# lbcb-sci/GNNome

Hardware: AMD Instinct MI355X
Metric: edges/sec full-graph GatedGCN fwd (higher is better)
Workload: dtype f32

## Files before the change

### gnnome_amd/_lib.py

```python
import ctypes
import os

_HERE = os.path.dirname(os.path.abspath(__file__))
LIB_PATH = os.environ.get("GNNOME_HIP_LIB") or os.path.join(_HERE, "lib", "libgnnome_hip.so")
HEADER_PATH = os.path.join(os.path.dirname(_HERE), "include", "gnnome_hip.h")

_p = ctypes.c_void_p
_i = ctypes.c_int
_l = ctypes.c_int64
_sz = ctypes.c_size_t

SIGNATURES = {
    "gnnome_abi_version": [],
    "gnnome_last_error": [],
    "gnnome_set_tuning": [_i, _i],
    "gnnome_debug_gate_profile": [_p],
    "gnnome_graph_views_workspace_bytes": [_l, _l, ctypes.POINTER(_sz)],
    "gnnome_build_graph_views": [_p, _p, _l, _l, _p, _p, _p, _p, _p, _p, _p, _p, _sz, _p],
    "gnnome_encode_f32": [_p, _l, _i, _p, _p, _p, _i, _p, _p, _i, _p, _p],
    "gnnome_linear_f32": [_p, _l, _i, _i, _p, _i, _p, _i, _p, _i, _p],
    "gnnome_linear_acc_f32": [_p, _l, _i, _i, _p, _i, _p, _i, _p, _i, _p],
    "gnnome_weight_planes_f16": [_p, _i, _i, _i, _p, _p],
    "gnnome_linear_planes_f32": [_p, _l, _i, _i, _p, _p, _i, _p, _i, _p],
    "gnnome_linear_planes_route": [_l, _i, _i, _i],
    "gnnome_edge_gate_f32": [_p, _p, _l, _i, _p, _p, _i, _p, _p, _p, _i, _i, _p, _p, _p],
    "gnnome_edge_gate_encode_f32": [_p, _p, _p, _p, _p, _p, _p, _l, _i, _p, _p, _i, _p, _p, _p, _i, _p, _p, _p],
    "gnnome_linear_ref_f32": [_p, _l, _i, _i, _p, _i, _p, _i, _p, _i, _p],
    "gnnome_edge_gate_ref_f32": [_p, _p, _l, _i, _p, _p, _i, _p, _p, _p, _i, _p, _p, _p, _p, _p, _p, _p, _p, _p, _p],
    "gnnome_node_aggregate_f32": [_p, _i, _l, _p, _p, _p, _i, _p, _p, _p, _p, _p, _p, _i, _p, _i, _p, _p, _p],
    "gnnome_build_node_records": [_p, _p, _p, _p, _p, _l, _p, _p],
    "gnnome_debug_node_records": [_p],
    "gnnome_node_aggregate_range_f32": [_p, _i, _l, _l, _l, _p, _p, _p, _i, _p, _p, _p, _p, _p, _p, _i, _p, _i, _p, _p, _p],
    "gnnome_node_aggregate_in_f32": [_p, _i, _l, _p, _p, _i, _p, _p, _p, _i, _p, _i, _p, _p, _p],
    "gnnome_node_aggregate_in_range_f32": [_p, _i, _l, _l, _l, _p, _p, _i, _p, _p, _p, _i, _p, _i, _p, _p, _p],
    "gnnome_node_aggregate_in_raw_f32": [_p, _i, _l, _p, _p, _i, _p, _p, _p, _p, _p, _p],
    "gnnome_node_aggregate_in_bwd_f32": [_p, _l, _i, _l, _p, _p, _p, _i, _p, _p, _p, _p, _p, _p, _p, _p],
    "gnnome_node_aggregate_in_raw_part_f32": [_p, _i, _l, _l, _p, _p, _i, _p, _p, _p, _p, _p, _p],
    "gnnome_node_aggregate_in_bwd_part_f32": [_p, _l, _i, _l, _l, _p, _p, _p, _i, _p, _p, _p, _p, _p, _p, _p, _p],
    "gnnome_node_neighbour_sum_f32": [_p, _i, _i, _l, _p, _p, _p, _p, _p, _p, _p, _i, _p],
    "gnnome_relu_rows_f32": [_p, _i, _l, _i, _p],
    "gnnome_node_neighbour_sum_bwd_f32": [_p, _i, _i, _l, _p, _p, _p, _p, _i, _p, _p, _p, _i, _p, _i, _p, _i, _p, _i, _p],
    "gnnome_node_neighbour_sum_part_f32": [_p, _i, _i, _l, _l, _p, _l, _p, _p, _p, _p, _p, _p, _p, _i, _p],
    "gnnome_node_neighbour_sum_bwd_part_f32": [_p, _i, _i, _l, _l, _p, _l, _p, _p, _p, _p, _i, _p, _p, _p, _i, _p, _i, _p, _i, _p, _i, _p],
    "gnnome_relu_mul_rows_f32": [_p, _i, _p, _i, _l, _i, _i, _p],
    "gnnome_node_attention_sum_f32": [_p, _i, _p, _i, _p, _i, _i, _i, _l, _p, _p, _p, _p, ctypes.c_float, _p, _p, _i, _p],
    "gnnome_node_attention_sum_stats_f32": [_p, _i, _p, _i, _p, _i, _i, _i, _l, _p, _p, _p, _p, ctypes.c_float, _p, _p, _i, _p, _i, _p],
    "gnnome_node_attention_sum_bwd_f32": [_p, _i, _p, _i, _p, _i, _p, _i, _p, _i, _p, _p, _i, _i, _i, _l, _p, _p, _p, _p, _i, ctypes.c_float,
                                          _p, _i, _p, _i, _p, _i, _p, _p],
    "gnnome_node_attention_sum_part_f32": [_p, _i, _p, _i, _p, _i, _i, _i, _l, _l, _p, _p, _p, _p, ctypes.c_float, _p, _p, _i, _p],
    "gnnome_node_attention_sum_stats_part_f32": [_p, _i, _p, _i, _p, _i, _i, _i, _l, _l, _p, _p, _p, _p, ctypes.c_float, _p, _p, _i, _p, _i, _p],
    "gnnome_node_attention_sum_bwd_dst_part_f32": [_p, _i, _p, _i, _p, _i, _p, _i, _p, _i, _p, _p, _i, _i, _i, _l, _l, _p, _p, _p, _p, _i,
                                                   ctypes.c_float, _p, _i, _p, _p],
    "gnnome_node_attention_sum_bwd_src_part_f32": [_p, _i, _p, _i, _p, _i, _p, _i, _i, _l, _l, _p, _p, _p, _p, _i, ctypes.c_float, _p, _i, _p, _i,
                                                   _p],
    "gnnome_stream_schedule_sizes": [_l, _l, _i, ctypes.POINTER(_l), ctypes.POINTER(_sz)],
    "gnnome_build_stream_schedule": [_l, _l, _p, _p, _p, _p, _p, _i, _i, _i, _p, _p, _p, _p, _p, _p, _p, _p, _sz, _p],
    "gnnome_node_aggregate_stream_f32": [_p, _i, _l, _l, _p, _p, _p, _i, _p, _p, _p, _p, _p, _p, _i, _p, _p, _p, _i, _i, _i, _p, _p, _p, _p, _p, _p,
                                         _p, _l, _p, _p],
    "gnnome_edge_score_f32": [_p, _l, _i, _i, _p, _p, _i, _p, _p, _p, _p, _i, _p, _p, _p, _p, _p, _p, _p],
    "gnnome_debug_forward_events": [_p, _p, _p, _p, _i],
    "gnnome_model_forward_workspace_bytes": [_l, _l, _i, _i, ctypes.POINTER(_sz)],
    "gnnome_model_forward_f32": [_p, _p, _p, _p, _p, _p, _sz, _p],
    "gnnome_model_forward_buffers_f32": [_p, _p, _p, _p, _p, _p, _p],
    "gnnome_edge_gate_raw_f32": [_p, _p, _l, _i, _p, _p, _i, _p, _p, _p, _i, _p],
    "gnnome_edge_gate_raw_stats_rows": [_i, ctypes.POINTER(_i)],
    "gnnome_edge_gate_raw_stats_f32": [_p, _p, _l, _i, _p, _p, _i, _p, _p, _p, _i, _p, _p, _p],
    "gnnome_edge_gate_raw_stats_x16": [_p, _p, _l, _i, _p, _p, _i, _p, _p, _p, _i, _p, _p, _p],
    "gnnome_edge_gate_bn_f32": [_p, _p, _p, _l, _i, _p, _p, _i, _p, _p, _p, _i, _p, _p, _p],
    "gnnome_edge_gate_bn_x16": [_p, _p, _p, _l, _i, _p, _p, _i, _p, _p, _p, _i, _p, _p, _p],
    "gnnome_node_aggregate_raw_f32": [_p, _i, _l, _i, _p, _p, _p, _i, _p, _p, _p, _p, _p, _p, _p, _p, _p, _p, _p],
    "gnnome_colsum_workspace_bytes": [ctypes.POINTER(_sz)],
    "gnnome_colsum2_f32": [_p, _p, _l, _i, _p, _p, _p, _p, _sz, _p],
    "gnnome_bn_relu_res_f32": [_p, _p, _p, _p, _l, _i, _p, _p],
    "gnnome_bn_relu_res_x16": [_p, _p, _p, _p, _l, _i, _p, _p],
    "gnnome_bn_bwd_stats_f32": [_p, _p, _p, _p, _p, _l, _i, _p, _p, _p, _sz, _p],
    "gnnome_bn_bwd_apply_f32": [_p, _p, _p, _p, _l, _i, _p, _p, _p, _p, _p, _p, _p],
    "gnnome_bn_bwd_apply_tables_f32": [_p, _p, _p, _p, _l, _i, _p, _p, _p, _p, _p, _p, _p, _p, _p, _p, _p, _p, _p, _p, _p, _p],
    "gnnome_ln_relu_res_f32": [_p, _p, _p, _p, _l, _i, _i, _p, _p],
    "gnnome_ln_bwd_f32": [_p, _p, _p, _p, _l, _i, _i, _p, _p, _p, _p, _sz, _p],
    "gnnome_mul23_f32": [_p, _p, _p, _l, _p, _p, _p],
    "gnnome_add_f32": [_p, _p, _l, _p, _p],
    "gnnome_relu_bwd_f32": [_p, _p, _l, _p, _p],
    "gnnome_segment_sum_f32": [_p, _i, _p, _p, _l, _p, _i, _p],
    "gnnome_segment_sum2_f32": [_p, _i, _p, _p, _p, _l, _p, _i, _p, _i, _p],
    "gnnome_segment_sum2_amax_f32": [_p, _i, _p, _p, _p, _l, _p, _i, _p, _i, _p, _p],
    "gnnome_segment_sum2_x16": [_p, _i, _p, _p, _p, _l, _p, _i, _p, _i, _p],
    "gnnome_wgrad_workspace_bytes": [_l, _i, _i, ctypes.POINTER(_sz)],
    "gnnome_wgrad_f32": [_p, _i, _i, _p, _i, _i, _l, _p, _i, _p, _sz, _p],
    "gnnome_wgrad_scaled_f32": [_p, _i, _i, _p, _i, _i, _l, _p, _p, _i, _p, _sz, _p],
    "gnnome_wgrad_x16": [_p, _i, _i, _p, _i, _i, _l, _p, _i, _p, _sz, _p],
    "gnnome_wgrad_blocks_f32": [_p, _i, _i, _i, _p, _i, _i, _l, _p, _i, _p, _p, _sz, _p],
    "gnnome_wgrad_blocks_scaled_f32": [_p, _i, _i, _i, _p, _i, _i, _l, _p, _p, _i, _p, _p, _sz, _p],
    "gnnome_linear_blocks_f32": [_p, _i, _i, _l, _i, _p, _i, _i, _p, _i, _i, _p],
    "gnnome_linear_blocks_scaled_f32": [_p, _i, _i, _l, _i, _p, _i, _i, _p, _p, _i, _i, _p],
    "gnnome_score_tail_bwd_f32": [_p, _p, _p, _l, _i, _p, _p, _p, _p, _p, _p, _p],
    "gnnome_agg_edge_bwd_f32": [_p, _l, _i, _p, _p, _p, _p, _p, _p, _i, _p, _p, _p, _p],
    "gnnome_encode_hidden_f32": [_p, _l, _i, _p, _p, _p, _i, _p, _p],
    "gnnome_gather_rows_f32": [_p, _i, _p, _l, _i, _p, _i, _p],
    "gnnome_scatter_add_rows_f32": [_p, _i, _p, _l, _i, _p, _i, _p],
    "gnnome_closure_workspace_bytes": [ctypes.POINTER(_sz)],
    "gnnome_degree_features_f32": [_p, _p, _l, _i, _p, _p, _sz, _p],
    "gnnome_edge_features_f32": [_p, _p, _l, _p, _p, _sz, _p],
    "gnnome_bn_bwd_dgrad_f32": [_p, _p, _l, _l, _i, _p, _p, _p, _p, _p, _p, _p, _p, _i, _p, _p],
    "gnnome_bn_bwd_dgrad_amax_f32": [_p, _p, _l, _l, _i, _p, _p, _p, _p, _p, _p, _p, _p, _i, _p, _p, _p],
    "gnnome_bn_bwd_dgrad_out_f32": [_p, _p, _p, _l, _l, _i, _p, _p, _p, _p, _p, _p, _p, _p, _i, _p, _p],
    "gnnome_bn_bwd_dgrad_out_amax_f32": [_p, _p, _p, _l, _l, _i, _p, _p, _p, _p, _p, _p, _p, _p, _i, _p, _p, _p],
    "gnnome_bn_bwd_dgrad_x16": [_p, _p, _l, _l, _i, _p, _p, _p, _p, _p, _p, _p, _p, _i, _p, _p],
    "gnnome_bn_bwd_dgrad_out_x16": [_p, _p, _p, _l, _l, _i, _p, _p, _p, _p, _p, _p, _p, _p, _i, _p, _p],
    "gnnome_agg_edge_bwd_stats_f32": [_p, _l, _i, _p, _p, _p, _p, _p, _p, _i, _p, _p, _p, _p, _p, _p, _p, _p, _p, _p, _sz, _p],
    "gnnome_agg_edge_bwd_stats_x16": [_p, _l, _i, _p, _p, _p, _p, _p, _p, _i, _p, _p, _p, _p, _p, _p, _p, _p, _p, _p, _sz, _p],
    "gnnome_agg_bwd_fused_f32": [_p, _l, _l, _i, _p, _p, _p, _p, _p, _p, _i, _p, _p, _p, _p, _p, _p, _p, _p, _p, _p, _p, _p, _p, _p, _p, _p, _sz, _p],
    "gnnome_agg_bwd_fused_x16": [_p, _l, _l, _i, _p, _p, _p, _p, _p, _p, _i, _p, _p, _p, _p, _p, _p, _p, _p, _p, _p, _p, _p, _p, _p, _p, _p, _sz, _p],
    "gnnome_bn_bwd_terms_f32": [_p, _p, _p, _l, _i, _p, _p, _p, _p],
    "gnnome_pack_layer_f32": [_p, _p, _p, _p, _i, _p, _p, _p, _p, _p],
    "gnnome_bn_train_finish_f32": [_p, _p, _p, _l, _i, _p, _p, _p, _p, _p, ctypes.c_float, ctypes.c_float, _i, _p, _p, _p, _p, _p],
    "gnnome_gate_center_f32": [_p, _l, _i, _p, _p, _i, _p, _p, _p, _i, _p, _p],
    "gnnome_greedy_walks_workspace_bytes": [_l, _i, ctypes.POINTER(_sz)],
    "gnnome_greedy_walks": [_p, _p, _p, _p, _p, _p, _p, _l, _p, _p, _p, _i, _p, _p, _l, _p, _p, _p, _p, _p, _p, _p, _sz, _p],
    "gnnome_greedy_walks_opts": [_p, _p, _p, _p, _p, _p, _p, _l, _p, _p, _p, _i, _p, _p, _l, _p, _p, _p, _p, _p, _p, _p, _sz, ctypes.c_float, _i, _l,
                                 _p],
    "gnnome_candidate_table": [_p, _p, _p, _p, _p, _p, _p, _i, _p, _p],
    "gnnome_mark_walk_visited": [_p, _p, _p, _l, _p, _p],
    "gnnome_overlap_workspace_bytes": [ctypes.POINTER(_sz)],
    "gnnome_overlap_edit_distance": [_p, _p, _l, _p, _i, _p, _p, _p, _l, _p, _p, _p, _sz, _p],
    "gnnome_overlap_long_workspace_bytes": [_l, ctypes.POINTER(_sz)],
    "gnnome_overlap_edit_distance_long": [_p, _p, _l, _p, _i, _p, _p, _p, _l, _l, _p, _p, _p, _sz, _p],
    "gnnome_contig_pieces_workspace_bytes": [_l, _l, ctypes.POINTER(_sz)],
    "gnnome_contig_pieces": [_p, _l, _p, _l, _p, _p, _p, _p, _l, _p, _l, _p, _p, _sz, _p],
    "gnnome_contig_spell": [_p, _l, _p, _l, _p, _p, _p, _l, _p, _i, _p, _l, _p],
    "gnnome_edge_labels_workspace_bytes": [_l, _l, ctypes.POINTER(_sz)],
    "gnnome_edge_labels": [_p, _p, _l, _l, _p, _p, _p, _p, _p, _p, _l, _p, _sz, _p],
    "gnnome_cluster_inputs_workspace_bytes": [_l, _l, ctypes.POINTER(_sz)],
    "gnnome_cluster_inputs_f32": [_p, _p, _l, _l, _p, _p, _l, _p, _l, _p, _l, _p, _p, _l, _p, _p, _l, _p, _p, _p, _p, _p, _sz, _p],
    "gnnome_adjacency_support": [_p, _p, _p, _l, _l, _p, _p],
    "gnnome_bfs_levels": [_p, _p, _l, _p, _p, _p, _p, _p, _p, _p],
    "gnnome_hem_propose": [_p, _p, _p, _p, _p, _l, _i, _p, _p],
    "gnnome_kway_gains": [_p, _p, _p, _p, _l, _p, _p, _p],
    "gnnome_greedy_growing_host": [_p, _p, _p, _p, _l, _i, _p],
    "gnnome_edge_loss_f32": [_p, _p, _p, _l, _p, ctypes.c_float, ctypes.c_float, _p, _p, _p, _p, _p, _sz, _p],
    "gnnome_gfa_tile_sizes": [ctypes.POINTER(_i), ctypes.POINTER(_i)],
    "gnnome_gfa_mark": [_p, _l, _p, _p, _p],
    "gnnome_gfa_classify": [_p, _l, _p, _p, _l, _p, _l, _p, _p, _p, _p, _p],
    "gnnome_gfa_names_insert": [_p, _l, _p, _p, _l, _p, _l, _p, _l, _p, _p],
    "gnnome_gfa_links": [_p, _l, _p, _p, _l, _p, _p, _l, _p, _l, _p, _l, _p, _p, _p, _p],
    "gnnome_gfa_pack": [_p, _l, _p, _p, _l, _p, _l, _p],
    "gnnome_reads_records_fasta": [_p, _l, _p, _p, _l, _p, _p, _l, _p, _p, _p, _p, _p, _p],
    "gnnome_reads_records_fastq": [_p, _l, _p, _p, _l, _p, _p, _l, _p, _l, _p, _p, _p, _p],
    "gnnome_reads_names_insert": [_p, _l, _p, _l, _p, _l, _p, _p, _p],
    "gnnome_reads_match": [_p, _l, _p, _i, _l, _p, _l, _p, _l, _p, _l, _p, _p],
    "gnnome_reads_annotations": [_p, _l, _p, _i, _l, _p, _p, _l, _p, _p, _p, _l, _p, _p],
    "gnnome_maf_lines": [_p, _l, _p, _p, _l, _p, _l, _p, _p, _p, _p, _p],
    "gnnome_maf_text_check": [_p, _l, _p, _p, _l, _p, _l, _p, _p],
    "gnnome_pr_curve_tile_size": [ctypes.POINTER(_i)],
    "gnnome_pr_curve_workspace_bytes": [_l, ctypes.POINTER(_sz)],
    "gnnome_pr_curve_keys": [_p, _p, _l, _i, _i, _p, _p, _p, _sz, _p],
    "gnnome_pr_curve_scan": [_p, _l, _p, _sz, _p, _p],
    "gnnome_pr_curve_emit": [_p, _l, _l, _l, _p, _p, _p, _p, _p, _p, _p, _sz, _p],
    "gnnome_pr_curve_ap": [_p, _p, _l, _p, _p, _sz, _p],
    "gnnome_walk_audit": [_p, _p, _p, _l, _l, _p, _p, _p, _p, _l, _p, _p, _p],
    "gnnome_interval_union_tile_size": [ctypes.POINTER(_i)],
    "gnnome_interval_union_workspace_bytes": [_l, ctypes.POINTER(_sz)],
    "gnnome_interval_union": [_p, _p, _p, _l, _p, _p, _p, _p, _l, _p, _p, _p, _p, _p, _sz, _p],
    "gnnome_pagerank_workspace_bytes": [_l, ctypes.POINTER(_sz)],
    "gnnome_pagerank_steps_f64": [_p, _p, _p, _l, _i, _p, _p, _p, _sz, _p],
    "gnnome_rw_return_lds_bytes": [_i, ctypes.POINTER(_sz)],
    "gnnome_rw_return_workspace_bytes": [_l, _i, ctypes.POINTER(_sz)],
    "gnnome_rw_return_f64": [_p, _p, _p, _l, _i, _i, _p, _i, _p, _p, _p, _sz, _p],
    "gnnome_sketch_tile_size": [ctypes.POINTER(_i)],
    "gnnome_sketch_workspace_bytes": [_l, ctypes.POINTER(_sz)],
    "gnnome_sketch_reads": [_p, _p, _l, _i, _i, _p, _l, _p, _p, _p, _p, _l, _p, _p, _sz, _p],
    "gnnome_seed_pairs_workspace_bytes": [_l, ctypes.POINTER(_sz)],
    "gnnome_seed_pairs": [_p, _p, _p, _p, _l, _p, _l, _i, _i, _p, _p, _l, _p, _p, _sz, _p],
    "gnnome_chain_overlaps": [_p, _p, _l, _p, _l, _p, _l, _i, _i, _i, _i, _i, _p, _p],
    "gnnome_transitive_tile_size": [ctypes.POINTER(_i)],
    "gnnome_transitive_edges": [_p, _p, _p, _p, _l, _l, _i, _p, _p],
    "gnnome_tip_nodes_workspace_bytes": [_l, ctypes.POINTER(_sz)],
    "gnnome_tip_nodes": [_p, _p, _p, _p, _p, _p, _l, _i, _p, _p, _sz, _p],
}

ABI_VERSION = 32


class LayerParams(ctypes.Structure):
    _fields_ = [(n, _p) for n in ("Wcat", "Wcat_planes", "bcat", "W3", "b3", "scale_e", "shift_e", "scale_h", "shift_h")] + [
        ("norm_kind", ctypes.c_int32), ("reference_order", ctypes.c_int32)]


class ModelParams(ctypes.Structure):
    _fields_ = ([(n, ctypes.c_int32) for n in ("hidden", "hidden_ne", "num_layers", "score_hidden", "node_features", "edge_features")]
                + [(n, _p) for n in ("node_W1", "node_b1", "node_W2", "node_b2", "edge_W1", "edge_b1", "edge_W2", "edge_b2")]
                + [("layers_host", ctypes.POINTER(LayerParams)), ("W_nodes", _p), ("W_nodes_planes", _p), ("b_nodes", _p), ("W1e", _p),
                   ("ld_w1e", ctypes.c_int32), ("reserved", ctypes.c_int32), ("W2", _p), ("b2", _p), ("W3", _p), ("b3", _p)])


class Views(ctypes.Structure):
    _fields_ = ([("num_nodes", ctypes.c_int64), ("num_edges", ctypes.c_int64)]
                + [(n, _p) for n in ("in_ptr", "srt_src", "srt_dst", "srt_eid", "out_ptr", "out_pos", "out_dst", "node_gather")]
                + [("transposed", ctypes.c_int32), ("reserved", ctypes.c_int32)])


class ForwardBuffers(ctypes.Structure):
    _fields_ = [("h", _p * 2), ("P", _p), ("e", _p * 2), ("PQ", _p)]


NORM_AFFINE = 0
NORM_LAYER = 1

_lib = None


class GnnomeHipError(RuntimeError):
    pass


def load():
    global _lib
# ... 26 lines not shown
```

### gnnome_amd/csrc/common.h

```cpp
#pragma once
#include <hip/hip_runtime.h>
#include <stdint.h>
#include <stdio.h>

#include "../../include/gnnome_hip.h"

namespace gnnome {

void set_error(const char* fmt, ...);

enum { kTuneGateVariant = 0, kTuneGateAblation = 1, kTuneLinearVariant = 2, kTuneGateTileOrder = 3, kTuneGateExperiment = 4, kTuneAggLdsKiB = 5, kTuneAggHubs = 6, kTuneAggVariant = 7, kTuneRefVariant = 8, kTuneOverlapBand = 9, kTuneArith = 10, kTuneAggAddr64 = 11, kTuneProjectSchedule = 12, kTuneCount = 16 };
int tuning(int key);

struct GateEnc {
    const float* e_raw;
    const int32_t* srt_eid;
    const float *W1, *b1, *W2, *b2;
    const float *W23, *b23;
};

struct GateBnBwd {
    const float *a, *c1, *c2, *mean, *rstd, *scale, *shift;
    float* a_out;
    int64_t n_once;
    unsigned* amax_bits = nullptr;
};

struct GateBfArgs {
    const float* e_in;
    float* e_out;
    int64_t E;
    const float* B1h;
    const float* B2h;
    int ldn;
    const int32_t* srt_src;
    const int32_t* srt_dst;
    const float* W3;
    int ldw;
    const float* scale;
    const float* shift;
    float* stats;
    int num_tiles;
    int abl;
    long long* prof;
    int xp;
    int num_cblocks, ld_out;
    GateEnc enc;
    GateBnBwd bnb;
};
int gate_bf_launch(int hidden, int mode, bool enc, const GateBfArgs& args, hipStream_t s, bool x16 = false, int extra = 0);
int gate_stream_launch(const float* e_in, float* e_out, int64_t E, const float* B1h, const float* B2h, int ldn, const int32_t* ss,
                       const int32_t* sd, const float* W3, int ldw, const float* scale, const float* shift, hipStream_t s);

int ws_linear_acc(const float* A, int64_t M, int K, const float* W, int ldw, float* C, hipStream_t s);
int stream_linear_acc_256(const float* A, int64_t M, const float* W, int ldw, float* C, hipStream_t s);
int gate_pl256_launch(int mode, const GateBfArgs& a, hipStream_t s, bool x16 = false);
int gate_f16_launch(int mode, const GateBfArgs& a, int grid, hipStream_t s, bool x16 = false);
int gate_enc256_launch(const GateBfArgs& a, hipStream_t s);
int gate_pl256_stats_rows();
void hub_cache_invalidate();
long long* gate_profile_buffer();
int linear_refm_launch(const float* A, int64_t M, int K, int lda, const float* W, int ldw, const float* bias, int Nout, float* C, int ldc,
                       hipStream_t s);
int gate_refm_launch(int hidden, bool with_enc, const float* e_in, float* e_out, int64_t E, const float* B1h, const float* B2h, int ldn,
                     const int32_t* ss, const int32_t* sd, const float* W3, int ldw, const float* b3, const float* scale, const float* shift,
                     const GateEnc& enc, hipStream_t s);

#define GN_REQUIRE(cond, ...)                 \
    do {                                      \
        if (!(cond)) {                        \
            ::gnnome::set_error(__VA_ARGS__); \
            return GNNOME_EINVAL;             \
        }                                     \
    } while (0)

#define GN_HIP(call)                                                                              \
    do {                                                                                          \
        hipError_t err__ = (call);                                                                \
        if (err__ != hipSuccess) {                                                                \
            ::gnnome::set_error("%s failed: %s (%s:%d)", #call, hipGetErrorString(err__), __FILE__, \
                                __LINE__);                                                        \
            return GNNOME_EHIP;                                                                   \
        }                                                                                         \
    } while (0)

#define GN_LAUNCH_CHECK() GN_HIP(hipGetLastError())

constexpr int kWave = 64;
constexpr int kXcds = 8;
constexpr int kNumCUs = 256;
int persistent_grid();
constexpr float kAggEps = 1e-6f;
constexpr float kNormEps = 1e-5f;

typedef float f32x4 __attribute__((ext_vector_type(4)));
typedef float f32x16 __attribute__((ext_vector_type(16)));

__device__ __forceinline__ unsigned bf16_bits(float x) {
    const unsigned u = __float_as_uint(x);
    return (u + 0x7FFFu + ((u >> 16) & 1u)) >> 16;
}
__device__ __forceinline__ uint2 pack_bf16x4(const f32x4 v) {
    return make_uint2(bf16_bits(v[0]) | (bf16_bits(v[1]) << 16), bf16_bits(v[2]) | (bf16_bits(v[3]) << 16));
}
__device__ __forceinline__ f32x4 unpack_bf16x4(const uint2 p) {
    return f32x4{__uint_as_float(p.x << 16), __uint_as_float(p.x & 0xFFFF0000u), __uint_as_float(p.y << 16),
                 __uint_as_float(p.y & 0xFFFF0000u)};
}
template <bool X16>
__device__ __forceinline__ f32x4 load4_as(const void* base, int64_t off) {
    if (X16) return unpack_bf16x4(*reinterpret_cast<const uint2*>(reinterpret_cast<const uint16_t*>(base) + off));
    return *reinterpret_cast<const f32x4*>(reinterpret_cast<const float*>(base) + off);
}
template <bool X16>
__device__ __forceinline__ void store4_as(void* base, int64_t off, const f32x4 v) {
    if (X16)
        *reinterpret_cast<uint2*>(reinterpret_cast<uint16_t*>(base) + off) = pack_bf16x4(v);
    else
        *reinterpret_cast<f32x4*>(reinterpret_cast<float*>(base) + off) = v;
}


__device__ __forceinline__ int xcd_remap(int bid, int n) {
    const int xcd = bid % kXcds, q = n / kXcds, r = n % kXcds;
    const int base = xcd < r ? xcd * (q + 1) : r * (q + 1) + (xcd - r) * q;
    return base + bid / kXcds;
}

__device__ __forceinline__ float sigmoidf_(float x) { return __builtin_amdgcn_rcpf(1.0f + __expf(-x)); }

typedef float f32x2 __attribute__((ext_vector_type(2)));
__device__ __forceinline__ f32x2 packed_(f32x2 v) {
    asm("" : "+v"(v));
    return v;
}
__device__ __forceinline__ f32x4 sigmoid4_(const f32x4 x) {
    const f32x2 t0 = packed_(packed_(f32x2{x[0], x[1]}) * -1.4426950408889634f), t1 = packed_(packed_(f32x2{x[2], x[3]}) * -1.4426950408889634f);
    const f32x2 d0 = packed_(packed_(f32x2{__builtin_amdgcn_exp2f(t0[0]), __builtin_amdgcn_exp2f(t0[1])}) + 1.0f);
    const f32x2 d1 = packed_(packed_(f32x2{__builtin_amdgcn_exp2f(t1[0]), __builtin_amdgcn_exp2f(t1[1])}) + 1.0f);
    return f32x4{__builtin_amdgcn_rcpf(d0[0]), __builtin_amdgcn_rcpf(d0[1]), __builtin_amdgcn_rcpf(d1[0]), __builtin_amdgcn_rcpf(d1[1])};
}

__device__ __forceinline__ float relu_keep_nan(float t) { return t < 0.f ? 0.f : t; }

__device__ __forceinline__ void wave_amax_to(unsigned* amax_bits, float v) {
#pragma unroll
    for (int o = 32; o > 0; o >>= 1) v = fmaxf(v, __shfl_xor(v, o));
    if ((threadIdx.x & 63) == 0) {
        const unsigned b = __float_as_uint(v);
        if (b > __hip_atomic_load(amax_bits, __ATOMIC_RELAXED, __HIP_MEMORY_SCOPE_AGENT)) atomicMax(amax_bits, b);
    }
}

__device__ __forceinline__ float half_wave_sum(float v) {
    v += __shfl_xor(v, 1);
    v += __shfl_xor(v, 2);
    v += __shfl_xor(v, 4);
    v += __shfl_xor(v, 8);
    v += __shfl_xor(v, 16);
    return v;
}

}
```

### gnnome_amd/csrc/edge_gate.hip

```cpp
#include "gemm_tile.h"
#include "lds_handover.h"

namespace gnnome {

template <int NB, int NORM>
__global__ __launch_bounds__(kGemmThreads) void k_edge_gate(const float* e_in, float* e_out, int64_t E,
                                                            const float* __restrict__ B1h,
                                                            const float* __restrict__ B2h, int ldn,
                                                            const int32_t* __restrict__ srt_src,
                                                            const int32_t* __restrict__ srt_dst,
                                                            const float* __restrict__ W3, int ldw,
                                                            const float* __restrict__ scale,
                                                            const float* __restrict__ shift, int total_tiles, int norm_width) {
    constexpr int H = 32 * NB;
    __shared__ __attribute__((aligned(16))) float lds[tile_lds_floats<NB>() + 2 * kTileM];
    float* As = lds;
    float* Ws = lds + kTileM * kLdk;
    int* s_src = reinterpret_cast<int*>(lds + tile_lds_floats<NB>());
    int* s_dst = s_src + kTileM;

    const int tid = threadIdx.x, wave = tid >> 6, lane = tid & 63;
    const int tile = xcd_remap(blockIdx.x, total_tiles);
    const int64_t row0 = (int64_t)tile * kTileM;
    const int valid = (int)min((int64_t)kTileM, E - row0);
// ... 473 lines not shown
    hipStream_t s = (hipStream_t)stream;
    const int variant = tuning(kTuneGateVariant);
    const bool rows16 = ld_node % 4 == 0 && ((uintptr_t)B1h % 16 == 0) && ((uintptr_t)B2h % 16 == 0);
    const bool persistent_ok = norm_kind == GNNOME_NORM_AFFINE && (hidden == 64 || hidden == 128);
    if (persistent_ok && variant != 1) {
        if ((variant == 0 || variant == 7 || variant == 8) && rows16) {
            GateBfArgs a = {};
            a.e_in = e_in; a.e_out = e_out; a.E = num_edges; a.B1h = B1h; a.B2h = B2h; a.ldn = ld_node; a.srt_src = srt_src;
            a.srt_dst = srt_dst; a.W3 = W3; a.ldw = ldw; a.scale = norm_scale; a.shift = norm_shift;
            return gate_bf_launch(hidden, 0, false, a, s);
        }
        if ((variant == 5 || variant == 6) && rows16) {
            if (hidden == 128)
                return launch_gate_ws<4, 1>(e_in, e_out, num_edges, B1h, B2h, ld_node, srt_src, srt_dst, W3, ldw, norm_scale, norm_shift, s);
            return launch_gate_ws<2, 2>(e_in, e_out, num_edges, B1h, B2h, ld_node, srt_src, srt_dst, W3, ldw, norm_scale, norm_shift, s);
        }
    }
    if (hidden == 256 && norm_kind == GNNOME_NORM_AFFINE && (variant == 0 || variant == 9) && e_in != e_out && ld_node % 4 == 0 &&
        ((uintptr_t)e_out % 16 == 0)) {
        if (variant == 0 && rows16) {
            GateBfArgs a = {};
            a.e_in = e_in; a.e_out = e_out; a.E = num_edges; a.B1h = B1h; a.B2h = B2h; a.ldn = ld_node; a.srt_src = srt_src;
            a.srt_dst = srt_dst; a.W3 = W3; a.ldw = ldw; a.scale = norm_scale; a.shift = norm_shift;
            return gate_pl256_launch(0, a, s);
        }
        return gate_stream_launch(e_in, e_out, num_edges, B1h, B2h, ld_node, srt_src, srt_dst, W3, ldw, norm_scale, norm_shift, s);
    }
    switch (hidden) {
        case 64: return launch_gate<2>(e_in, e_out, num_edges, B1h, B2h, ld_node, srt_src, srt_dst, W3, ldw, norm_kind, norm_scale, norm_shift, s, norm_width);
        case 128: return launch_gate<4>(e_in, e_out, num_edges, B1h, B2h, ld_node, srt_src, srt_dst, W3, ldw, norm_kind, norm_scale, norm_shift, s, norm_width);
        case 256: return launch_gate<8>(e_in, e_out, num_edges, B1h, B2h, ld_node, srt_src, srt_dst, W3, ldw, norm_kind, norm_scale, norm_shift, s, norm_width);
        default: set_error("edge_gate: hidden=%d not in {64,128,256}", hidden); return GNNOME_EINVAL;
    }
}

extern "C" int gnnome_edge_gate_raw_f32(const float* e_in, float* x_out, int64_t num_edges, int hidden, const float* B1h,
                                        const float* B2h, int ld_node, const int32_t* srt_src, const int32_t* srt_dst,
                                        const float* W3, int ldw, void* stream) {
    using namespace gnnome;
    GN_REQUIRE(num_edges >= 0, "edge_gate_raw: negative edge count");
    if (num_edges == 0) return GNNOME_OK;
    GN_REQUIRE(e_in && x_out && x_out != e_in && B1h && B2h && srt_src && srt_dst && W3, "edge_gate_raw: bad pointers");
    GN_REQUIRE(ld_node >= hidden && ldw >= hidden && ldw % 4 == 0, "edge_gate_raw: bad strides");
    GN_REQUIRE(((uintptr_t)e_in % 16 == 0) && ((uintptr_t)W3 % 16 == 0), "edge_gate_raw: e_in and W3 must be 16-byte aligned");
    hipStream_t s = (hipStream_t)stream;
    if (hidden == 256 && tuning(kTuneGateVariant) == 0 && ld_node % 4 == 0 && ((uintptr_t)B1h % 16 == 0) && ((uintptr_t)B2h % 16 == 0) &&
        ((uintptr_t)x_out % 16 == 0)) {
        GateBfArgs a = {};
        a.e_in = e_in; a.e_out = x_out; a.E = num_edges; a.B1h = B1h; a.B2h = B2h; a.ldn = ld_node; a.srt_src = srt_src;
        a.srt_dst = srt_dst; a.W3 = W3; a.ldw = ldw;
        return gate_pl256_launch(1, a, s);
    }
    switch (hidden) {
        case 64: return launch_gate<2>(e_in, x_out, num_edges, B1h, B2h, ld_node, srt_src, srt_dst, W3, ldw, 2, nullptr, nullptr, s);
        case 128: return launch_gate<4>(e_in, x_out, num_edges, B1h, B2h, ld_node, srt_src, srt_dst, W3, ldw, 2, nullptr, nullptr, s);
        case 256: return launch_gate<8>(e_in, x_out, num_edges, B1h, B2h, ld_node, srt_src, srt_dst, W3, ldw, 2, nullptr, nullptr, s);
        default: set_error("edge_gate_raw: hidden=%d not in {64,128,256}", hidden); return GNNOME_EINVAL;
    }
}

extern "C" int gnnome_edge_gate_raw_stats_rows(int hidden, int* rows_host) {
    using namespace gnnome;
    GN_REQUIRE(rows_host && (hidden == 64 || hidden == 128 || hidden == 256), "edge_gate_raw_stats_rows: hidden=%d not in {64,128,256}", hidden);
    if (hidden == 256) {
        *rows_host = gate_pl256_stats_rows();
        return GNNOME_OK;
    }
    *rows_host = (tuning(kTuneGateVariant) == 0 || tuning(kTuneGateVariant) == 8) ? kNumCUs * 8 : kNumCUs * (hidden == 128 ? 1 : 2);
    return GNNOME_OK;
}

static int raw_stats_impl(const float* e_in, void* x_out, int64_t num_edges, int hidden, const float* B1h,
                          const float* B2h, int ld_node, const int32_t* srt_src, const int32_t* srt_dst,
                          const float* W3, int ldw, const float* center, float* stats_partial, void* stream, bool x16) {
    using namespace gnnome;
    GN_REQUIRE(num_edges > 0, "edge_gate_raw_stats: needs at least one edge");
    GN_REQUIRE(e_in && x_out != (const void*)e_in && B1h && B2h && srt_src && srt_dst && W3 && center && stats_partial,
               "edge_gate_raw_stats: bad pointers");
    GN_REQUIRE(x_out || ((hidden == 128 || (hidden == 256 && tuning(kTuneArith) == 0 && !x16)) && tuning(kTuneGateVariant) == 0),
               "edge_gate_raw_stats: x_out may be NULL at hidden = 128 and, as fp16x3 with fp32 storage, 256 (default kernels)");
    GN_REQUIRE(hidden == 64 || hidden == 128 || hidden == 256, "edge_gate_raw_stats: hidden=%d not in {64,128,256}", hidden);
    GN_REQUIRE(ld_node >= hidden && ld_node % 4 == 0 && ldw >= hidden && ldw % 4 == 0, "edge_gate_raw_stats: bad strides");
    GN_REQUIRE(((uintptr_t)e_in % 16 == 0) && ((uintptr_t)W3 % 16 == 0) && ((uintptr_t)B1h % 16 == 0) && ((uintptr_t)B2h % 16 == 0),
               "edge_gate_raw_stats: 16-byte alignment required");
    GN_REQUIRE(!x16 || hidden == 256 || tuning(kTuneGateVariant) == 0 || tuning(kTuneGateVariant) == 8,
               "edge_gate_raw_stats_x16: bf16 storage is built on the default kernels (gnnome_set_tuning key 0 = 0 or 8), got %d", tuning(kTuneGateVariant));
    hipStream_t s = (hipStream_t)stream;
    if (hidden == 256) {
        GateBfArgs a = {};
        a.e_in = e_in; a.e_out = (float*)x_out; a.E = num_edges; a.B1h = B1h; a.B2h = B2h; a.ldn = ld_node; a.srt_src = srt_src;
        a.srt_dst = srt_dst; a.W3 = W3; a.ldw = ldw; a.scale = center; a.stats = stats_partial;
        return gate_pl256_launch(1, a, s, x16);
    }
    if (tuning(kTuneGateVariant) == 0 || tuning(kTuneGateVariant) == 8 || x16) {
        GateBfArgs a = {};
        a.e_in = e_in; a.e_out = (float*)x_out; a.E = num_edges; a.B1h = B1h; a.B2h = B2h; a.ldn = ld_node; a.srt_src = srt_src;
        a.srt_dst = srt_dst; a.W3 = W3; a.ldw = ldw; a.scale = center; a.stats = stats_partial;
        return gate_bf_launch(hidden, 1, false, a, s, x16, x_out == nullptr ? 1 : 0);
    }
    if (hidden == 128)
        return launch_ws_raw_stats<4, 1>(e_in, (float*)x_out, num_edges, B1h, B2h, ld_node, srt_src, srt_dst, W3, ldw, center, stats_partial, s);
    return launch_ws_raw_stats<2, 2>(e_in, (float*)x_out, num_edges, B1h, B2h, ld_node, srt_src, srt_dst, W3, ldw, center, stats_partial, s);
}

extern "C" int gnnome_edge_gate_raw_stats_f32(const float* e_in, float* x_out, int64_t num_edges, int hidden, const float* B1h,
                                              const float* B2h, int ld_node, const int32_t* srt_src, const int32_t* srt_dst,
                                              const float* W3, int ldw, const float* center, float* stats_partial, void* stream) {
    return raw_stats_impl(e_in, x_out, num_edges, hidden, B1h, B2h, ld_node, srt_src, srt_dst, W3, ldw, center, stats_partial, stream, false);
}

extern "C" int gnnome_edge_gate_raw_stats_x16(const float* e_in, uint16_t* x_out, int64_t num_edges, int hidden, const float* B1h,
                                              const float* B2h, int ld_node, const int32_t* srt_src, const int32_t* srt_dst,
                                              const float* W3, int ldw, const float* center, float* stats_partial, void* stream) {
    return raw_stats_impl(e_in, x_out, num_edges, hidden, B1h, B2h, ld_node, srt_src, srt_dst, W3, ldw, center, stats_partial, stream, true);
}

static int gate_bn_impl(const float* e_in, float* e_out, void* x_out, int64_t num_edges, int hidden, const float* B1h, const float* B2h, int ld_node,
                        const int32_t* srt_src, const int32_t* srt_dst, const float* W3, int ldw, const float* scale, const float* shift,
                        void* stream, bool x16) {
    using namespace gnnome;
    GN_REQUIRE(num_edges >= 0, "edge_gate_bn: negative edge count");
    if (num_edges == 0) return GNNOME_OK;
    GN_REQUIRE(e_in && e_out && x_out && x_out != (const void*)e_in && x_out != (void*)e_out && B1h && B2h && srt_src && srt_dst && W3 && scale && shift,
               "edge_gate_bn: bad pointers");
    GN_REQUIRE((hidden == 128 || (hidden == 256 && tuning(kTuneArith) == 0 && !x16)) && tuning(kTuneGateVariant) == 0,
               "edge_gate_bn: built at hidden = 128 and, as fp16x3 with fp32 storage, 256 (default kernels), got %d", hidden);
    GN_REQUIRE(ld_node >= hidden && ld_node % 4 == 0 && ldw >= hidden && ldw % 4 == 0, "edge_gate_bn: bad strides");
    GN_REQUIRE(((uintptr_t)e_in % 16 == 0) && ((uintptr_t)e_out % 16 == 0) && ((uintptr_t)x_out % 16 == 0) && ((uintptr_t)W3 % 16 == 0) &&
                   ((uintptr_t)B1h % 16 == 0) && ((uintptr_t)B2h % 16 == 0), "edge_gate_bn: 16-byte alignment required");
    GateBfArgs a = {};
    a.e_in = e_in; a.e_out = e_out; a.E = num_edges; a.B1h = B1h; a.B2h = B2h; a.ldn = ld_node; a.srt_src = srt_src; a.srt_dst = srt_dst;
    a.W3 = W3; a.ldw = ldw; a.scale = scale; a.shift = shift; a.bnb.a_out = (float*)x_out;
    if (hidden == 256) return gate_pl256_launch(0, a, (hipStream_t)stream, false);
    return gate_bf_launch(hidden, 0, false, a, (hipStream_t)stream, x16, 1);
}

extern "C" int gnnome_edge_gate_bn_f32(const float* e_in, float* e_out, float* x_out, int64_t num_edges, int hidden, const float* B1h,
                                       const float* B2h, int ld_node, const int32_t* srt_src, const int32_t* srt_dst, const float* W3, int ldw,
                                       const float* scale, const float* shift, void* stream) {
    return gate_bn_impl(e_in, e_out, x_out, num_edges, hidden, B1h, B2h, ld_node, srt_src, srt_dst, W3, ldw, scale, shift, stream, false);
}

extern "C" int gnnome_edge_gate_bn_x16(const float* e_in, float* e_out, uint16_t* x_out, int64_t num_edges, int hidden, const float* B1h,
                                       const float* B2h, int ld_node, const int32_t* srt_src, const int32_t* srt_dst, const float* W3, int ldw,
                                       const float* scale, const float* shift, void* stream) {
    return gate_bn_impl(e_in, e_out, x_out, num_edges, hidden, B1h, B2h, ld_node, srt_src, srt_dst, W3, ldw, scale, shift, stream, true);
}

extern "C" int gnnome_edge_gate_encode_f32(const float* e_raw, const int32_t* srt_eid, const float* encW1, const float* encb1,
                                           const float* encW2, const float* encb2, float* e_out, int64_t num_edges, int hidden,
                                           const float* B1h, const float* B2h, int ld_node, const int32_t* srt_src,
                                           const int32_t* srt_dst, const float* W3, int ldw, const float* norm_scale,
                                           const float* norm_shift, void* stream) {
    using namespace gnnome;
    GN_REQUIRE(num_edges >= 0, "edge_gate_encode: negative edge count");
    if (num_edges == 0) return GNNOME_OK;
    GN_REQUIRE(e_raw && srt_eid && encW1 && encb1 && encW2 && encb2 && e_out && B1h && B2h && srt_src && srt_dst && W3 &&
                   norm_scale && norm_shift, "edge_gate_encode: null pointer");
    GN_REQUIRE(hidden == 64 || hidden == 128 || (hidden == 256 && tuning(kTuneArith) == 0 && tuning(kTuneGateVariant) == 0),
               "edge_gate_encode: hidden=%d not in {64,128,256 (default kernels)}", hidden);
    GN_REQUIRE(ld_node % 4 == 0 && ldw % 4 == 0 && ((uintptr_t)B1h % 16 == 0) && ((uintptr_t)B2h % 16 == 0) && ((uintptr_t)W3 % 16 == 0),
               "edge_gate_encode: alignment");
    const GateEnc enc = {e_raw, srt_eid, encW1, encb1, encW2, encb2};
    hipStream_t s = (hipStream_t)stream;
    if (hidden == 256) {
        GN_REQUIRE((uintptr_t)e_out % 16 == 0, "edge_gate_encode: e_out must be 16-byte aligned");
        GateBfArgs a = {};
        a.e_out = e_out; a.E = num_edges; a.B1h = B1h; a.B2h = B2h; a.ldn = ld_node; a.srt_src = srt_src; a.srt_dst = srt_dst;
        a.W3 = W3; a.ldw = ldw; a.scale = norm_scale; a.shift = norm_shift; a.enc = enc;
        return gate_enc256_launch(a, s);
    }
    if (tuning(kTuneGateVariant) == 0 || tuning(kTuneGateVariant) == 7 || tuning(kTuneGateVariant) == 8) {
        GateBfArgs a = {};
        a.e_out = e_out; a.E = num_edges; a.B1h = B1h; a.B2h = B2h; a.ldn = ld_node; a.srt_src = srt_src; a.srt_dst = srt_dst;
        a.W3 = W3; a.ldw = ldw; a.scale = norm_scale; a.shift = norm_shift; a.enc = enc;
        return gate_bf_launch(hidden, 0, true, a, s);
    }
    if (hidden == 128)
        return launch_gate_ws<4, 1>(nullptr, e_out, num_edges, B1h, B2h, ld_node, srt_src, srt_dst, W3, ldw, norm_scale, norm_shift, s, &enc);
    return launch_gate_ws<2, 2>(nullptr, e_out, num_edges, B1h, B2h, ld_node, srt_src, srt_dst, W3, ldw, norm_scale, norm_shift, s, &enc);
}
```

### gnnome_amd/csrc/edge_gate_bf.hip

```cpp
#include "common.h"
#include "lds_handover.h"
#include "operand_planes.h"

namespace gnnome {

template <int CB, int RB>
struct GateBF {
    static_assert(CB * RB == 4, "four compute waves");
    static constexpr int H = 32 * CB, TM = 32 * RB, LDK = H + 4, RING = 4, LWAVES = 2;
    static constexpr int NT = 64 * (4 + RING * LWAVES);
    static constexpr int NP = TM * (H / 4) / (64 * LWAVES);
    static constexpr int kSlotFloats = TM * LDK;
    static constexpr int kLdsFloats = RING * 2 * kSlotFloats;
};

template <int CB, int RB, int MODE, bool ENC, bool X16 = false>
__global__ __launch_bounds__(768) void k_edge_gate_bf(GateBfArgs a) {
    using P = GateBF<CB, RB>;
    constexpr int H = P::H, TM = P::TM, NP = P::NP, LDK = P::LDK, RING = P::RING, KS = H / 16, SLOT = P::kSlotFloats;
    constexpr int kEncFloats = ENC ? 16 * H + H + 48 : (MODE == 1 ? 8 * 64 * 8 : 0);
    __shared__ __attribute__((aligned(16))) float lds[P::kLdsFloats + kEncFloats];
    __shared__ unsigned flags[2 * RING];
    float* Aring = lds;
    float* Gring = lds + RING * SLOT;
// ... 664 lines not shown
    constexpr int H = 128, TM = 32, RING = 3, LDK = H + 4, TPLD = 48, TPLANE = TM * TPLD, TILEF = TM * LDK;
    constexpr int SLOTB = 3 * TPLANE + 2 * TILEF * 4, NP = 8, RSTEP = 4;
    __shared__ __attribute__((aligned(16))) unsigned char ring[RING * SLOTB];
    __shared__ __attribute__((aligned(16))) float consts[4 * H];
    __shared__ float w1s[32], b1s[16];
    __shared__ unsigned flags[2 * RING];
    const int tid = threadIdx.x, lane = tid & 63;
    const int wave = __builtin_amdgcn_readfirstlane(tid >> 6);
    const unsigned full0 = lds_addr(&flags[0]), done0 = lds_addr(&flags[RING]);
    const int per_xcd = gridDim.x / kXcds;
    const int first = (int)(blockIdx.x % kXcds) * per_xcd + (int)(blockIdx.x / kXcds);
    const int stride = (int)gridDim.x;
    const int n = first < a.num_tiles ? (a.num_tiles - first + stride - 1) / stride : 0;
    if (n <= 0) return;
    auto tile_of = [&](int r) { return first + r * stride; };
    auto tile_valid = [&](int r) { return (int)min((int64_t)TM, a.E - (int64_t)tile_of(r) * TM); };
    if (tid < 4 * H) {
        const int q = tid / H, c = tid % H;
        consts[tid] = q == 0 ? a.scale[c] : q == 1 ? a.shift[c] : q == 2 ? a.enc.b23[c] : a.enc.b2[c];
    }
    if (tid >= 4 * H && tid < 4 * H + 32) w1s[tid - 4 * H] = a.enc.W1[tid - 4 * H];
    if (tid >= 4 * H + 32 && tid < 4 * H + 48) b1s[tid - 4 * H - 32] = a.enc.b1[tid - 4 * H - 32];
    if (tid < 2 * RING) flags[tid] = 0;
    __syncthreads();

    if (wave < 4) {
        const int cl = lane & 31, half = lane >> 5, col = 32 * wave + cl;
        uint4 u1, u2, u3, v1, v2, v3;
        {
            const float* p = a.enc.W23 + col * 16 + 8 * half;
            bf16_split8(*reinterpret_cast<const f32x4*>(p), *reinterpret_cast<const f32x4*>(p + 4), u1, u2, u3);
            const float* q = a.enc.W2 + col * 16 + 8 * half;
            bf16_split8(*reinterpret_cast<const f32x4*>(q), *reinterpret_cast<const f32x4*>(q + 4), v1, v2, v3);
        }
        auto crow = [](int r) { return (r & 3) + 8 * (r >> 2); };
        const int lane_x = 4 * half * LDK + col;
        const float bxc = consts[2 * H + col], bec = consts[3 * H + col];
        for (int i = 0; i < n; ++i) {
            const int slot = i % RING;
            const unsigned use = (unsigned)(i / RING) + 1u;
            flag_wait(full0 + 4 * slot, 2u * use, 0);
            const unsigned char* tp = ring + slot * SLOTB + cl * TPLD + 16 * half;
            const uint4 c1 = *reinterpret_cast<const uint4*>(tp), c2 = *reinterpret_cast<const uint4*>(tp + TPLANE),
                        c3 = *reinterpret_cast<const uint4*>(tp + 2 * TPLANE);
            f32x16 ax, ae;
#pragma unroll
            for (int r = 0; r < 16; ++r) ax[r] = ae[r] = 0.f;
            ax = __builtin_amdgcn_mfma_f32_32x32x16_bf16(as_bf16x8(c3), as_bf16x8(u1), ax, 0, 0, 0);
            ae = __builtin_amdgcn_mfma_f32_32x32x16_bf16(as_bf16x8(c3), as_bf16x8(v1), ae, 0, 0, 0);
            ax = __builtin_amdgcn_mfma_f32_32x32x16_bf16(as_bf16x8(c1), as_bf16x8(u3), ax, 0, 0, 0);
            ae = __builtin_amdgcn_mfma_f32_32x32x16_bf16(as_bf16x8(c1), as_bf16x8(v3), ae, 0, 0, 0);
            ax = __builtin_amdgcn_mfma_f32_32x32x16_bf16(as_bf16x8(c2), as_bf16x8(u2), ax, 0, 0, 0);
            ae = __builtin_amdgcn_mfma_f32_32x32x16_bf16(as_bf16x8(c2), as_bf16x8(v2), ae, 0, 0, 0);
            ax = __builtin_amdgcn_mfma_f32_32x32x16_bf16(as_bf16x8(c2), as_bf16x8(u1), ax, 0, 0, 0);
            ae = __builtin_amdgcn_mfma_f32_32x32x16_bf16(as_bf16x8(c2), as_bf16x8(v1), ae, 0, 0, 0);
            ax = __builtin_amdgcn_mfma_f32_32x32x16_bf16(as_bf16x8(c1), as_bf16x8(u2), ax, 0, 0, 0);
            ae = __builtin_amdgcn_mfma_f32_32x32x16_bf16(as_bf16x8(c1), as_bf16x8(v2), ae, 0, 0, 0);
            ax = __builtin_amdgcn_mfma_f32_32x32x16_bf16(as_bf16x8(c1), as_bf16x8(u1), ax, 0, 0, 0);
            ae = __builtin_amdgcn_mfma_f32_32x32x16_bf16(as_bf16x8(c1), as_bf16x8(v1), ae, 0, 0, 0);
            float* X = reinterpret_cast<float*>(ring + slot * SLOTB + 3 * TPLANE) + lane_x;
#pragma unroll
            for (int r = 0; r < 16; ++r) {
                X[crow(r) * LDK] = ax[r] + bxc;
                X[TILEF + crow(r) * LDK] = ae[r] + bec;
            }
            flag_bump(done0 + 4 * slot, lane);
        }
    } else {
        const int group = (wave - 4) / 2;
        const int gl = ((wave - 4) % 2) * 64 + lane;
        const int r0 = gl / (H / 4), c4 = gl % (H / 4);
        const int trow = gl >> 2, jq = gl & 3;
        f32x4 g1[NP], g2[NP], gk[NP];
        int si[NP], di[NP], eid = 0;
        float raw0 = 0.f, raw1 = 0.f;
        const unsigned off_row = (unsigned)(r0 * H + 4 * c4);
        auto issue_early = [&](int r) {
            const int64_t row0 = (int64_t)tile_of(r) * TM;
            const int valid = tile_valid(r);
#pragma unroll
            for (int p = 0; p < NP; ++p) {
                const int64_t row = row0 + min(r0 + p * RSTEP, valid - 1);
                si[p] = a.srt_src[row];
                di[p] = a.srt_dst[row];
            }
            eid = a.enc.srt_eid[row0 + min(trow, valid - 1)];
        };
        auto issue_late = [&]() {
            raw0 = a.enc.e_raw[2 * (int64_t)eid];
            raw1 = a.enc.e_raw[2 * (int64_t)eid + 1];
#pragma unroll
            for (int p = 0; p < NP; ++p) {
                g1[p] = *reinterpret_cast<const f32x4*>(a.B1h + (int64_t)si[p] * a.ldn + 4 * c4);
                g2[p] = *reinterpret_cast<const f32x4*>(a.B2h + (int64_t)di[p] * a.ldn + 4 * c4);
            }
        };
        if (group < n) {
            issue_early(group);
            issue_late();
            if (group + RING < n) issue_early(group + RING);
        }
        unsigned char* S = ring + group * SLOTB;
        const float* Xs = reinterpret_cast<const float*>(S + 3 * TPLANE);
        for (int r = group; r < n; r += RING) {
            const unsigned use = (unsigned)(r / RING) + 1u;
            {
                f32x4 t;
#pragma unroll
                for (int j = 0; j < 4; ++j) {
                    const int hu = 4 * jq + j;
                    t[j] = fmaxf(__builtin_fmaf(raw1, w1s[2 * hu + 1], raw0 * w1s[2 * hu]) + b1s[hu], 0.f);
                }
                uint2 p1, p2, p3;
                bf16_split4(t, p1, p2, p3);
                unsigned char* d = S + trow * TPLD + 8 * jq;
                *reinterpret_cast<uint2*>(d) = p1;
                *reinterpret_cast<uint2*>(d + TPLANE) = p2;
                *reinterpret_cast<uint2*>(d + 2 * TPLANE) = p3;
            }
#pragma unroll
            for (int p = 0; p < NP; ++p) {
                gk[p] = g1[p] + g2[p];
                asm volatile("" : "+v"(gk[p]));
            }
            flag_bump(full0 + 4 * group, lane);
            if (r + RING < n) issue_late();
            if (r + 2 * RING < n) issue_early(r + 2 * RING);
            flag_wait(done0 + 4 * group, 4u * use, a.xp & 3);
            const int valid = tile_valid(r);
            const f32x4 sc4 = *reinterpret_cast<const f32x4*>(consts + 4 * c4), sh4 = *reinterpret_cast<const f32x4*>(consts + H + 4 * c4);
            float* out = a.e_out + (int64_t)tile_of(r) * TM * H;
#pragma unroll
            for (int pb = 0; pb < NP; pb += 2) {
                f32x4 x[2], e0[2];
#pragma unroll
                for (int u = 0; u < 2; ++u) {
                    x[u] = *reinterpret_cast<const f32x4*>(Xs + (r0 + (pb + u) * RSTEP) * LDK + 4 * c4);
                    e0[u] = *reinterpret_cast<const f32x4*>(Xs + TILEF + (r0 + (pb + u) * RSTEP) * LDK + 4 * c4);
                }
                asm volatile("" : "+v"(x[0]), "+v"(x[1]));
#pragma unroll
                for (int u = 0; u < 2; ++u) {
                    const int p = pb + u, row = r0 + p * RSTEP;
                    f32x4 y;
#pragma unroll
                    for (int j = 0; j < 4; ++j) y[j] = fmaxf((x[u][j] + gk[p][j]) * sc4[j] + sh4[j], 0.f) + e0[u][j];
                    if (row < valid) *reinterpret_cast<f32x4*>(out + (off_row + (unsigned)(p * RSTEP * H))) = y;
                }
            }
        }
    }
}

struct EncFoldScratch {
    float* w23 = nullptr;
};
static EncFoldScratch g_enc_fold[16];

static int launch_enc16(const GateBfArgs& args, hipStream_t s) {
    GateBfArgs a = args;
    const int64_t tiles = (a.E + 31) / 32;
    GN_REQUIRE(tiles < (1ll << 31), "edge_gate: too many tiles");
    a.num_tiles = (int)tiles;
    a.xp = tuning(kTuneGateExperiment);
    int dev = 0;
    GN_HIP(hipGetDevice(&dev));
    GN_REQUIRE(dev >= 0 && dev < 16, "edge_gate_encode: device index %d", dev);
    if (!g_enc_fold[dev].w23) GN_HIP(hipMalloc(&g_enc_fold[dev].w23, sizeof(float) * (128 * 16 + 128)));
    float* w23 = g_enc_fold[dev].w23;
    hipLaunchKernelGGL(k_fold_encoder, dim3((128 * 17 + 3) / 4), dim3(256), 0, s, a.W3, a.ldw, a.enc.W2, a.enc.b2, 128, w23, w23 + 128 * 16);
    GN_LAUNCH_CHECK();
    a.enc.W23 = w23;
    a.enc.b23 = w23 + 128 * 16;
    hipLaunchKernelGGL(k_edge_gate_enc16, dim3(persistent_grid()), dim3(640), 0, s, a);
    GN_LAUNCH_CHECK();
    return GNNOME_OK;
}

static EncFoldScratch g_enc_fold256[16];
int gate_enc256_launch(const GateBfArgs& args, hipStream_t s) {
    GateBfArgs a = args;
    const int64_t tiles = (a.E + 31) / 32;
    GN_REQUIRE(tiles < (1ll << 31), "edge_gate: too many tiles");
    a.num_tiles = (int)tiles;
    a.prof = g_gate_prof;
    int dev = 0;
    GN_HIP(hipGetDevice(&dev));
    GN_REQUIRE(dev >= 0 && dev < 16, "edge_gate_encode: device index %d", dev);
    if (!g_enc_fold256[dev].w23) GN_HIP(hipMalloc(&g_enc_fold256[dev].w23, sizeof(float) * (256 * 16 + 256)));
    float* w23 = g_enc_fold256[dev].w23;
    hipLaunchKernelGGL(k_fold_encoder, dim3((256 * 17 + 3) / 4), dim3(256), 0, s, a.W3, a.ldw, a.enc.W2, a.enc.b2, 256, w23, w23 + 256 * 16);
    GN_LAUNCH_CHECK();
    a.enc.W23 = w23;
    a.enc.b23 = w23 + 256 * 16;
    int g = persistent_grid();
    g -= g % 16;
    return gate_f16_launch(5, a, g < 16 ? 16 : g, s);
}

template <int CB, int RB, int MODE, bool ENC, bool X16 = false>
static int launch_bf(const GateBfArgs& args, hipStream_t s) {
    using P = GateBF<CB, RB>;
    GateBfArgs a = args;
    const int64_t tiles = (a.E + P::TM - 1) / P::TM;
    GN_REQUIRE(tiles < (1ll << 31), "edge_gate: too many tiles");
    a.num_tiles = (int)tiles;
    a.abl = tuning(kTuneGateAblation);
    a.xp = tuning(kTuneGateExperiment);
    a.prof = g_gate_prof;
    if (MODE == 1) GN_HIP(hipMemsetAsync(a.stats, 0, sizeof(float) * kNumCUs * P::RING * P::LWAVES * 2 * P::H, s));
    hipLaunchKernelGGL((k_edge_gate_bf<CB, RB, MODE, ENC, X16>), dim3(persistent_grid()), dim3(P::NT), 0, s, a);
    GN_LAUNCH_CHECK();
    return GNNOME_OK;
}

int gate_bf_launch(int hidden, int mode, bool enc, const GateBfArgs& a, hipStream_t s, bool x16, int extra) {
    const bool planes = hidden == 128 && tuning(kTuneGateVariant) != 8;
    if (extra) {
        GN_REQUIRE(hidden == 128 && !enc && (mode == 0 || mode == 1), "edge-tile kernel: the two-pass training forward is built at hidden = 128");
        if (mode == 1) return x16 ? launch_pl<false, 1, true, 1>(a, s) : launch_pl<false, 1, false, 1>(a, s);
        return x16 ? launch_pl<false, 0, true, 1>(a, s) : launch_pl<false, 0, false, 1>(a, s);
    }
    if (x16) {
        if (mode == 1 && planes) return launch_pl<false, 1, true>(a, s);
        if (mode == 3 && planes) return launch_pl<false, 3, true>(a, s);
        if (mode == 1) return hidden == 128 ? launch_bf<4, 1, 1, false, true>(a, s) : launch_bf<2, 2, 1, false, true>(a, s);
        if (mode == 3) return hidden == 128 ? launch_bf<4, 1, 3, false, true>(a, s) : launch_bf<2, 2, 3, false, true>(a, s);
        set_error("edge-tile kernel: bf16 storage exists for modes 1 and 3 only");
        return GNNOME_EINVAL;
    }
    if (hidden == 128) {
        if (mode == 0 && enc && tuning(kTuneGateVariant) == 0) return launch_enc16(a, s);
        if (mode == 0 && tuning(kTuneGateVariant) != 8) return enc ? launch_pl<true>(a, s) : launch_pl<false>(a, s);
        if (mode == 1 && planes) return launch_pl<false, 1>(a, s);
        if (mode == 3 && planes) return launch_pl<false, 3>(a, s);
        if (mode == 4) return launch_pl<false, 4>(a, s);
        if (mode == 2 && planes) return launch_pl<false, 2>(a, s);
        if (mode == 0) return enc ? launch_bf<4, 1, 0, true>(a, s) : launch_bf<4, 1, 0, false>(a, s);
        if (mode == 3) return launch_bf<4, 1, 3, false>(a, s);
        return mode == 1 ? launch_bf<4, 1, 1, false>(a, s) : launch_bf<4, 1, 2, false>(a, s);
    }
    if (mode == 0) return enc ? launch_bf<2, 2, 0, true>(a, s) : launch_bf<2, 2, 0, false>(a, s);
    if (mode == 3) return launch_bf<2, 2, 3, false>(a, s);
    return mode == 1 ? launch_bf<2, 2, 1, false>(a, s) : launch_bf<2, 2, 2, false>(a, s);
}

}

extern "C" int gnnome_debug_gate_profile(void* counters) {
    gnnome::g_gate_prof = (long long*)counters;
    return GNNOME_OK;
}

static int bn_bwd_dgrad_impl(float* C, const void* X, int64_t rows, int64_t rows_once, int hidden, const float* scale, const float* shift,
                             const float* a, const float* c1, const float* c2, const float* mean, const float* rstd,
                             const float* W, int ldw, void* dxe, void* stream, bool x16, unsigned* amax_bits = nullptr) {
    using namespace gnnome;
    GN_REQUIRE(rows >= 0 && (hidden == 64 || hidden == 128), "bn_bwd_dgrad: hidden=%d not in {64,128}", hidden);
    GN_REQUIRE(rows_once >= 0 && rows_once <= rows, "bn_bwd_dgrad: rows_once=%lld outside [0, rows]", (long long)rows_once);
    if (rows == 0) return GNNOME_OK;
    GN_REQUIRE(C && X && scale && shift && a && c1 && c2 && mean && rstd && W && dxe && dxe != (void*)C && ldw >= hidden && ldw % 4 == 0,
               "bn_bwd_dgrad: bad arguments");
    GN_REQUIRE(((uintptr_t)C % 16 == 0) && ((uintptr_t)X % 16 == 0) && ((uintptr_t)dxe % 16 == 0) && ((uintptr_t)W % 16 == 0),
               "bn_bwd_dgrad: tensors must be 16-byte aligned");
    GateBfArgs g = {};
    g.e_in = (const float*)X; g.e_out = C; g.E = rows; g.B1h = C; g.ldn = hidden; g.W3 = W; g.ldw = ldw;
    g.bnb = GateBnBwd{a, c1, c2, mean, rstd, scale, shift, (float*)dxe, rows_once};
    if (amax_bits != nullptr) {
        GN_REQUIRE(hidden == 128 && tuning(kTuneGateVariant) != 8, "bn_bwd_dgrad_amax: hidden = 128 on the plane-form kernel only");
        GN_HIP(hipMemsetAsync(amax_bits, 0, sizeof(unsigned), (hipStream_t)stream));
        g.bnb.amax_bits = amax_bits;
    }
    return gate_bf_launch(hidden, 3, false, g, (hipStream_t)stream, x16);
}

extern "C" int gnnome_bn_bwd_dgrad_f32(float* C, const float* X, int64_t rows, int64_t rows_once, int hidden, const float* scale, const float* shift,
                                       const float* a, const float* c1, const float* c2, const float* mean, const float* rstd,
                                       const float* W, int ldw, float* dxe, void* stream) {
    return bn_bwd_dgrad_impl(C, X, rows, rows_once, hidden, scale, shift, a, c1, c2, mean, rstd, W, ldw, dxe, stream, false);
}

extern "C" int gnnome_bn_bwd_dgrad_amax_f32(float* C, const float* X, int64_t rows, int64_t rows_once, int hidden, const float* scale,
                                            const float* shift, const float* a, const float* c1, const float* c2, const float* mean,
                                            const float* rstd, const float* W, int ldw, float* dxe, unsigned* amax_bits, void* stream) {
    GN_REQUIRE(amax_bits != nullptr, "bn_bwd_dgrad_amax: null amax_bits");
    return bn_bwd_dgrad_impl(C, X, rows, rows_once, hidden, scale, shift, a, c1, c2, mean, rstd, W, ldw, dxe, stream, false, amax_bits);
}

extern "C" int gnnome_bn_bwd_dgrad_x16(float* C, const uint16_t* X, int64_t rows, int64_t rows_once, int hidden, const float* scale, const float* shift,
                                       const float* a, const float* c1, const float* c2, const float* mean, const float* rstd,
                                       const float* W, int ldw, uint16_t* dxe, void* stream) {
    return bn_bwd_dgrad_impl(C, X, rows, rows_once, hidden, scale, shift, a, c1, c2, mean, rstd, W, ldw, dxe, stream, true);
}

static int bn_bwd_dgrad_out_impl(const float* C_in, float* C_out, const float* X, int64_t rows, int64_t rows_once, int hidden,
                                 const float* scale, const float* shift, const float* a, const float* c1, const float* c2,
                                 const float* mean, const float* rstd, const float* W, int ldw, float* dxe, void* stream, bool x16,
                                 unsigned* amax_bits = nullptr);
extern "C" int gnnome_bn_bwd_dgrad_out_amax_f32(const float* C_in, float* C_out, const float* X, int64_t rows, int64_t rows_once, int hidden,
                                                const float* scale, const float* shift, const float* a, const float* c1, const float* c2,
                                                const float* mean, const float* rstd, const float* W, int ldw, float* dxe, unsigned* amax_bits,
                                                void* stream) {
    GN_REQUIRE(amax_bits != nullptr, "bn_bwd_dgrad_out_amax: null amax_bits");
    return bn_bwd_dgrad_out_impl(C_in, C_out, X, rows, rows_once, hidden, scale, shift, a, c1, c2, mean, rstd, W, ldw, dxe, stream, false, amax_bits);
}
extern "C" int gnnome_bn_bwd_dgrad_out_f32(const float* C_in, float* C_out, const float* X, int64_t rows, int64_t rows_once, int hidden,
                                           const float* scale, const float* shift, const float* a, const float* c1, const float* c2,
                                           const float* mean, const float* rstd, const float* W, int ldw, float* dxe, void* stream) {
    return bn_bwd_dgrad_out_impl(C_in, C_out, X, rows, rows_once, hidden, scale, shift, a, c1, c2, mean, rstd, W, ldw, dxe, stream, false);
}
extern "C" int gnnome_bn_bwd_dgrad_out_x16(const float* C_in, float* C_out, const uint16_t* X, int64_t rows, int64_t rows_once, int hidden,
                                           const float* scale, const float* shift, const float* a, const float* c1, const float* c2,
                                           const float* mean, const float* rstd, const float* W, int ldw, uint16_t* dxe, void* stream) {
    return bn_bwd_dgrad_out_impl(C_in, C_out, (const float*)X, rows, rows_once, hidden, scale, shift, a, c1, c2, mean, rstd, W, ldw, (float*)dxe, stream, true);
}
static int bn_bwd_dgrad_out_impl(const float* C_in, float* C_out, const float* X, int64_t rows, int64_t rows_once, int hidden,
                                 const float* scale, const float* shift, const float* a, const float* c1, const float* c2,
                                 const float* mean, const float* rstd, const float* W, int ldw, float* dxe, void* stream, bool x16,
                                 unsigned* amax_bits) {
    using namespace gnnome;
    GN_REQUIRE(rows >= 0 && hidden == 256, "bn_bwd_dgrad_out: hidden=%d (256 only; 64 / 128 update C in place: gnnome_bn_bwd_dgrad_f32)", hidden);
    if (amax_bits != nullptr) GN_HIP(hipMemsetAsync(amax_bits, 0, sizeof(unsigned), (hipStream_t)stream));
    GN_REQUIRE(rows_once >= 0 && rows_once <= rows, "bn_bwd_dgrad_out: rows_once=%lld outside [0, rows]", (long long)rows_once);
    if (rows == 0) return GNNOME_OK;
    GN_REQUIRE(C_in && C_out && C_out != C_in && X && scale && shift && a && c1 && c2 && mean && rstd && W && dxe && dxe != C_out && dxe != C_in &&
                   ldw >= hidden && ldw % 4 == 0, "bn_bwd_dgrad_out: bad arguments");
    GN_REQUIRE(((uintptr_t)C_in % 16 == 0) && ((uintptr_t)C_out % 16 == 0) && ((uintptr_t)X % 16 == 0) && ((uintptr_t)dxe % 16 == 0) &&
                   ((uintptr_t)W % 16 == 0), "bn_bwd_dgrad_out: tensors must be 16-byte aligned");
    (void)x16;
    GateBfArgs g = {};
    g.e_in = X; g.e_out = C_out; g.E = rows; g.B1h = C_in; g.ldn = hidden; g.W3 = W; g.ldw = ldw;
    g.bnb = GateBnBwd{a, c1, c2, mean, rstd, scale, shift, dxe, rows_once};
    g.bnb.amax_bits = amax_bits;
    return gate_pl256_launch(3, g, (hipStream_t)stream, x16);
}
```

### gnnome_amd/csrc/encode.hip

```cpp
#include "common.h"

namespace gnnome {

constexpr int kEncThreads = 256;
constexpr int kEncMaxF = 8, kEncMaxM = 64;

template <int H>
__global__ __launch_bounds__(kEncThreads) void k_encode(const float* __restrict__ in, int64_t rows, int F,
                                                        const int32_t* __restrict__ gather, const float* __restrict__ W1,
                                                        const float* __restrict__ b1, int M, const float* __restrict__ W2,
                                                        const float* __restrict__ b2, float* __restrict__ out) {
    constexpr int LPR = H / 4, RPB = kEncThreads / LPR, KMAX = (kEncMaxM + LPR - 1) / LPR;
    __shared__ __attribute__((aligned(16))) float w2t[kEncMaxM * H];
    __shared__ float w1s[kEncMaxM * kEncMaxF];
    __shared__ float b1s[kEncMaxM];
    const int tid = threadIdx.x;
    for (int i = tid; i < M * H; i += kEncThreads) w2t[i] = W2[(i % H) * M + (i / H)];
    for (int i = tid; i < M * F; i += kEncThreads) w1s[i] = W1[i];
    for (int i = tid; i < M; i += kEncThreads) b1s[i] = b1[i];
    __syncthreads();

    const int li = tid % LPR, rg = tid / LPR, c = 4 * li;
    const int lane_base = (tid & 63) - li;
    const f32x4 bias = *reinterpret_cast<const f32x4*>(b2 + c);

    for (int64_t r0 = (int64_t)blockIdx.x * RPB; r0 < rows; r0 += (int64_t)gridDim.x * RPB) {
        const int64_t r = r0 + rg;
        const bool live = r < rows;
        const int64_t rin = live ? (gather != nullptr ? (int64_t)gather[r] : r) : 0;
        float xin[kEncMaxF];
#pragma unroll
        for (int f = 0; f < kEncMaxF; ++f) xin[f] = (live && f < F) ? in[rin * F + f] : 0.f;
        float t[KMAX];
#pragma unroll
        for (int k = 0; k < KMAX; ++k) {
            const int j = li + k * LPR;
            float s = 0.f;
            if (j < M) {
#pragma unroll
                for (int f = 0; f < kEncMaxF; ++f)
                    if (f < F) s = __builtin_fmaf(xin[f], w1s[j * F + f], s);
                s = fmaxf(s + b1s[j], 0.f);
            }
            t[k] = s;
        }
        f32x4 acc = {0.f, 0.f, 0.f, 0.f};
#pragma unroll
        for (int k = 0; k < KMAX; ++k) {
            const int jn = min(LPR, M - k * LPR);
            for (int jj = 0; jj < jn; ++jj) {
                const float tj = __shfl(t[k], lane_base + jj);
                const f32x4 w = *reinterpret_cast<const f32x4*>(&w2t[(k * LPR + jj) * H + c]);
#pragma unroll
                for (int i = 0; i < 4; ++i) acc[i] = __builtin_fmaf(tj, w[i], acc[i]);
            }
        }
        if (live) *reinterpret_cast<f32x4*>(out + r * H + c) = acc + bias;
    }
}

template <int H>
__global__ __launch_bounds__(kEncThreads) void k_encode_f2m16(const float* __restrict__ in, int64_t rows,
                                                              const int32_t* __restrict__ gather,
                                                              const float* __restrict__ W1, const float* __restrict__ b1,
                                                              const float* __restrict__ W2, const float* __restrict__ b2,
                                                              float* __restrict__ out) {
    constexpr int LPR = H / 4, RPB = kEncThreads / LPR, M = 16;
    const int tid = threadIdx.x, li = tid % LPR, rg = tid / LPR, c = 4 * li;
    float w1a[M], w1b[M], bb[M];
#pragma unroll
    for (int j = 0; j < M; ++j) {
        w1a[j] = W1[2 * j];
        w1b[j] = W1[2 * j + 1];
        bb[j] = b1[j];
    }
    f32x4 w2[M];
#pragma unroll
    for (int i = 0; i < 4; ++i) {
#pragma unroll
        for (int j4 = 0; j4 < M / 4; ++j4) {
            const f32x4 v = *reinterpret_cast<const f32x4*>(W2 + (c + i) * M + 4 * j4);
#pragma unroll
            for (int jj = 0; jj < 4; ++jj) w2[4 * j4 + jj][i] = v[jj];
        }
    }
    const f32x4 bias = *reinterpret_cast<const f32x4*>(b2 + c);
    for (int64_t r = (int64_t)blockIdx.x * RPB + rg; r < rows; r += (int64_t)gridDim.x * RPB) {
        const int64_t rin = gather != nullptr ? (int64_t)gather[r] : r;
        const float x0 = in[2 * rin], x1 = in[2 * rin + 1];
        f32x4 acc = {0.f, 0.f, 0.f, 0.f};
#pragma unroll
        for (int j = 0; j < M; ++j) {
            const float t = fmaxf(__builtin_fmaf(x1, w1b[j], x0 * w1a[j]) + bb[j], 0.f);
#pragma unroll
            for (int i = 0; i < 4; ++i) acc[i] = __builtin_fmaf(t, w2[j][i], acc[i]);
        }
        *reinterpret_cast<f32x4*>(out + r * H + c) = acc + bias;
    }
}

template <int H>
static int launch_encode(const float* in, int64_t rows, int F, const int32_t* gather, const float* W1, const float* b1,
                         int M, const float* W2, const float* b2, float* out, hipStream_t s) {
    constexpr int RPB = kEncThreads / (H / 4);
    int64_t blocks = (rows + RPB - 1) / RPB;
    if (blocks > kNumCUs * 8) blocks = kNumCUs * 8;
    if (F == 2 && M == 16 && ((uintptr_t)W2 % 16 == 0)) {
        hipLaunchKernelGGL(k_encode_f2m16<H>, dim3((unsigned)blocks), dim3(kEncThreads), 0, s, in, rows, gather, W1, b1, W2, b2,
                           out);
    } else {
        hipLaunchKernelGGL(k_encode<H>, dim3((unsigned)blocks), dim3(kEncThreads), 0, s, in, rows, F, gather, W1, b1, M, W2,
                           b2, out);
    }
    GN_LAUNCH_CHECK();
    return GNNOME_OK;
}

__global__ __launch_bounds__(256) void k_gather_rows(const float* __restrict__ in, int ld_in,
                                                     const int32_t* __restrict__ idx, int64_t rows, int w4,
                                                     float* __restrict__ out, int ld_out) {
    const int64_t total = rows * w4;
    for (int64_t i = (int64_t)blockIdx.x * blockDim.x + threadIdx.x; i < total; i += (int64_t)gridDim.x * blockDim.x) {
        const int64_t r = i / w4;
        const int c = (int)(i % w4) * 4;
        *reinterpret_cast<f32x4*>(out + r * ld_out + c) = *reinterpret_cast<const f32x4*>(in + (int64_t)idx[r] * ld_in + c);
    }
}

__global__ __launch_bounds__(256) void k_scatter_add_rows(const float* __restrict__ in, int ld_in,
                                                          const int32_t* __restrict__ idx, int64_t rows, int w4,
                                                          float* __restrict__ out, int ld_out) {
    const int64_t total = rows * w4;
    for (int64_t i = (int64_t)blockIdx.x * blockDim.x + threadIdx.x; i < total; i += (int64_t)gridDim.x * blockDim.x) {
        const int64_t r = i / w4;
        const int c = (int)(i % w4) * 4;
        f32x4* dst = reinterpret_cast<f32x4*>(out + (int64_t)idx[r] * ld_out + c);
        const f32x4 a = *reinterpret_cast<const f32x4*>(in + r * ld_in + c);
        f32x4 b = *dst;
        b[0] += a[0]; b[1] += a[1]; b[2] += a[2]; b[3] += a[3];
        *dst = b;
    }
}

}

extern "C" int gnnome_encode_f32(const float* in, int64_t rows, int in_features, const int32_t* gather, const float* W1,
                                 const float* b1, int hidden_ne, const float* W2, const float* b2, int hidden, float* out,
                                 void* stream) {
    using namespace gnnome;
    GN_REQUIRE(rows >= 0, "encode: negative row count");
    if (rows == 0) return GNNOME_OK;
    GN_REQUIRE(in && W1 && b1 && W2 && b2 && out, "encode: null pointer");
    GN_REQUIRE(in_features >= 1 && in_features <= kEncMaxF, "encode: in_features=%d not in [1,%d]", in_features, kEncMaxF);
    GN_REQUIRE(hidden_ne >= 1 && hidden_ne <= kEncMaxM, "encode: hidden_ne=%d not in [1,%d]", hidden_ne, kEncMaxM);
    GN_REQUIRE(((uintptr_t)out % 16 == 0) && ((uintptr_t)b2 % 16 == 0), "encode: out and b2 must be 16-byte aligned");
    hipStream_t s = (hipStream_t)stream;
    switch (hidden) {
        case 64: return launch_encode<64>(in, rows, in_features, gather, W1, b1, hidden_ne, W2, b2, out, s);
        case 128: return launch_encode<128>(in, rows, in_features, gather, W1, b1, hidden_ne, W2, b2, out, s);
        case 256: return launch_encode<256>(in, rows, in_features, gather, W1, b1, hidden_ne, W2, b2, out, s);
        default: set_error("encode: hidden=%d not in {64,128,256}", hidden); return GNNOME_EINVAL;
    }
}

extern "C" int gnnome_gather_rows_f32(const float* in, int ld_in, const int32_t* idx, int64_t rows, int width, float* out,
                                      int ld_out, void* stream) {
    using namespace gnnome;
    GN_REQUIRE(rows >= 0, "gather_rows: negative row count");
    if (rows == 0) return GNNOME_OK;
    GN_REQUIRE(in && idx && out, "gather_rows: null pointer");
    GN_REQUIRE(width > 0 && width % 4 == 0 && ld_in % 4 == 0 && ld_out % 4 == 0 && ld_in >= width && ld_out >= width,
               "gather_rows: width and strides must be multiples of 4");
    GN_REQUIRE(((uintptr_t)in % 16 == 0) && ((uintptr_t)out % 16 == 0), "gather_rows: 16-byte alignment required");
    const int w4 = width / 4;
    int64_t blocks = (rows * w4 + 255) / 256;
    if (blocks > kNumCUs * 8) blocks = kNumCUs * 8;
    hipLaunchKernelGGL(k_gather_rows, dim3((unsigned)blocks), dim3(256), 0, (hipStream_t)stream, in, ld_in, idx, rows, w4,
                       out, ld_out);
    GN_LAUNCH_CHECK();
    return GNNOME_OK;
}

extern "C" int gnnome_scatter_add_rows_f32(const float* in, int ld_in, const int32_t* idx, int64_t rows, int width,
                                           float* out, int ld_out, void* stream) {
    using namespace gnnome;
    GN_REQUIRE(rows >= 0, "scatter_add_rows: negative row count");
    if (rows == 0) return GNNOME_OK;
    GN_REQUIRE(in && idx && out, "scatter_add_rows: null pointer");
    GN_REQUIRE(width > 0 && width % 4 == 0 && ld_in % 4 == 0 && ld_out % 4 == 0 && ld_in >= width && ld_out >= width,
               "scatter_add_rows: width and strides must be multiples of 4");
    GN_REQUIRE(((uintptr_t)in % 16 == 0) && ((uintptr_t)out % 16 == 0), "scatter_add_rows: 16-byte alignment required");
    const int w4 = width / 4;
    int64_t blocks = (rows * w4 + 255) / 256;
    if (blocks > kNumCUs * 8) blocks = kNumCUs * 8;
    hipLaunchKernelGGL(k_scatter_add_rows, dim3((unsigned)blocks), dim3(256), 0, (hipStream_t)stream, in, ld_in, idx, rows,
                       w4, out, ld_out);
    GN_LAUNCH_CHECK();
    return GNNOME_OK;
}
```

### gnnome_amd/csrc/model_forward.cpp

```cpp
#include "common.h"

namespace gnnome {
namespace {

constexpr size_t kAlign = 256;
size_t rounded(size_t bytes) { return (bytes + kAlign - 1) / kAlign * kAlign; }

struct Workspace {
    size_t h[2], P, e[2], PQ, total;
};
Workspace layout(int64_t n, int64_t e, int hidden, int hs) {
    Workspace w;
    size_t off = 0;
    auto take = [&](size_t bytes) {
        const size_t at = off;
        off += rounded(bytes);
        return at;
    };
    w.h[0] = take(sizeof(float) * n * hidden);
    w.h[1] = take(sizeof(float) * n * hidden);
    w.P = take(sizeof(float) * n * 5 * hidden);
    w.e[0] = take(sizeof(float) * e * hidden);
    w.e[1] = hidden == 256 ? take(sizeof(float) * e * hidden) : w.e[0];
    w.PQ = take(sizeof(float) * n * 2 * hs);
    w.total = off;
    return w;
}

struct ForwardEvents {
    hipEvent_t ev[4] = {nullptr, nullptr, nullptr, nullptr};
    int layer = -1;
};
thread_local ForwardEvents g_events;
int mark(int which, int layer, void* stream) {
    if (layer != g_events.layer || g_events.ev[which] == nullptr) return GNNOME_OK;
    GN_HIP(hipEventRecord(g_events.ev[which], (hipStream_t)stream));
    return GNNOME_OK;
}

int project(const float* A, int64_t M, int K, const float* W, const void* planes, const float* bias, int Nout, float* C, void* stream) {
    if (planes != nullptr && gnnome_linear_planes_route(M, K, Nout, 1)) return gnnome_linear_planes_f32(A, M, K, K, planes, bias, Nout, C, Nout, stream);
    return gnnome_linear_f32(A, M, K, K, W, K, bias, Nout, C, Nout, stream);
}

}
}

extern "C" int gnnome_debug_forward_events(void* gate_start, void* gate_stop, void* aggregate_start, void* aggregate_stop, int layer) {
    using namespace gnnome;
    g_events.ev[0] = (hipEvent_t)gate_start;
    g_events.ev[1] = (hipEvent_t)gate_stop;
    g_events.ev[2] = (hipEvent_t)aggregate_start;
    g_events.ev[3] = (hipEvent_t)aggregate_stop;
    g_events.layer = layer;
    return GNNOME_OK;
}

extern "C" int gnnome_model_forward_workspace_bytes(int64_t num_nodes, int64_t num_edges, int hidden, int score_hidden, size_t* bytes_host) {
    using namespace gnnome;
    GN_REQUIRE(bytes_host && num_nodes >= 0 && num_edges >= 0 && hidden > 0 && score_hidden > 0, "model_forward_workspace_bytes: bad argument");
    *bytes_host = layout(num_nodes, num_edges, hidden, score_hidden).total;
    return GNNOME_OK;
}

#define GN_TRY(call)                       \
    do {                                   \
        const int rc__ = (call);           \
        if (rc__ != GNNOME_OK) return rc__; \
    } while (0)

namespace gnnome {
namespace {
int forward_on(const gnnome_model_params* m, const gnnome_views* g, const float* x, const float* e_raw, float* logits, float* const h[2], float* P,
               float* const eb[2], float* PQ, void* stream);
}
}

static int check_model(const gnnome_model_params* m, const gnnome_views* g) {
    using namespace gnnome;
    GN_REQUIRE(m && g, "model_forward: null parameter block");
    const int H = m->hidden, hs = m->score_hidden, L = m->num_layers;
    GN_REQUIRE(g->num_nodes >= 0 && g->num_edges >= 0 && L >= 0 && (L == 0 || m->layers_host != nullptr), "model_forward: bad sizes");
    GN_REQUIRE(H == 64 || H == 128 || H == 256, "model_forward: hidden=%d (the kernels are built for 64 / 128 / 256; pad narrower models)", H);
    GN_REQUIRE(hs == 32 || hs == 64 || hs == 128, "model_forward: score_hidden=%d (built for 32 / 64 / 128)", hs);
    return GNNOME_OK;
}

extern "C" int gnnome_model_forward_f32(const gnnome_model_params* m, const gnnome_views* g, const float* x, const float* e_raw, float* logits,
                                        void* workspace, size_t workspace_bytes, void* stream) {
    using namespace gnnome;
    GN_TRY(check_model(m, g));
    const int64_t N = g->num_nodes, E = g->num_edges;
    const Workspace ws = layout(N, E, m->hidden, m->score_hidden);
    if (workspace_bytes < ws.total) {
        set_error("model_forward: workspace of %zu bytes, %zu needed", workspace_bytes, ws.total);
        return GNNOME_EWORKSPACE;
    }
    GN_REQUIRE((N == 0 && E == 0) || (workspace != nullptr && (uintptr_t)workspace % kAlign == 0), "model_forward: workspace must be 256-byte aligned");
    GN_REQUIRE(E == 0 || logits != nullptr, "model_forward: null logits");
    char* base = static_cast<char*>(workspace);
    float* h[2] = {reinterpret_cast<float*>(base + ws.h[0]), reinterpret_cast<float*>(base + ws.h[1])};
    float* eb[2] = {reinterpret_cast<float*>(base + ws.e[0]), reinterpret_cast<float*>(base + ws.e[1])};
    return forward_on(m, g, x, e_raw, logits, h, reinterpret_cast<float*>(base + ws.P), eb, reinterpret_cast<float*>(base + ws.PQ), stream);
}

extern "C" int gnnome_model_forward_buffers_f32(const gnnome_model_params* m, const gnnome_views* g, const float* x, const float* e_raw, float* logits,
                                                const gnnome_forward_buffers* b, void* stream) {
    using namespace gnnome;
    GN_TRY(check_model(m, g));
    GN_REQUIRE(b != nullptr, "model_forward_buffers: null buffer block");
    const int64_t N = g->num_nodes, E = g->num_edges;
    GN_REQUIRE(E == 0 || logits != nullptr, "model_forward_buffers: null logits");
    GN_REQUIRE(N == 0 || (b->h[0] && b->h[1] && b->P && b->PQ && b->h[0] != b->h[1]), "model_forward_buffers: node buffers h[0], h[1], P, PQ");
    GN_REQUIRE(E == 0 || (b->e[0] && (m->hidden != 256 || (b->e[1] && b->e[1] != b->e[0]))), "model_forward_buffers: edge buffers e[0] (and e[1] at hidden = 256)");
    for (const void* p : {(const void*)b->h[0], (const void*)b->h[1], (const void*)b->P, (const void*)b->e[0], (const void*)b->e[1], (const void*)b->PQ})
        GN_REQUIRE((uintptr_t)p % 16 == 0, "model_forward_buffers: buffers must be 16-byte aligned");
    float* h[2] = {b->h[0], b->h[1]};
    float* eb[2] = {b->e[0], m->hidden == 256 ? b->e[1] : b->e[0]};
    return forward_on(m, g, x, e_raw, logits, h, b->P, eb, b->PQ, stream);
}

namespace gnnome {
namespace {
int forward_on(const gnnome_model_params* m, const gnnome_views* g, const float* x, const float* e_raw, float* logits, float* const h[2], float* P,
               float* const eb[2], float* PQ, void* stream) {
    const int64_t N = g->num_nodes, E = g->num_edges;
    const int H = m->hidden, hs = m->score_hidden, L = m->num_layers;

    GN_TRY(gnnome_encode_f32(x, N, m->node_features, g->node_gather, m->node_W1, m->node_b1, m->hidden_ne, m->node_W2, m->node_b2, H, h[0], stream));
    const bool wide_ok = tuning(kTuneArith) == 0 && tuning(kTuneGateVariant) == 0;
    const bool fold = L > 0 && m->edge_features == 2 && m->hidden_ne == 16 && (H == 64 || H == 128 || (H == 256 && wide_ok)) &&
                      m->layers_host[0].norm_kind == GNNOME_NORM_AFFINE && E > 0;
    float* e = nullptr;
    if (!fold) {
        e = eb[0];
        GN_TRY(gnnome_encode_f32(e_raw, E, m->edge_features, g->srt_eid, m->edge_W1, m->edge_b1, m->hidden_ne, m->edge_W2, m->edge_b2, H, e, stream));
    }
    int cur = 0;
    for (int i = 0; i < L; ++i) {
        const gnnome_layer_params& lw = m->layers_host[i];
        if (lw.reference_order) GN_TRY(gnnome_linear_ref_f32(h[cur], N, H, H, lw.Wcat, H, lw.bcat, 5 * H, P, 5 * H, stream));
        else GN_TRY(project(h[cur], N, H, lw.Wcat, lw.Wcat_planes, lw.bcat, 5 * H, P, stream));
        const float *A1 = P, *A2 = P + H, *A3 = P + 2 * H, *B1 = P + 3 * H, *B2 = P + 4 * H;
        if (g->transposed) {
            const float* t = A2; A2 = A3; A3 = t;
            t = B1; B1 = B2; B2 = t;
        }
        GN_TRY(mark(0, i, stream));
        if (lw.reference_order) {
            float* out = e ? e : eb[0];
            GN_TRY(gnnome_edge_gate_ref_f32(e, out, E, H, B1, B2, 5 * H, g->srt_src, g->srt_dst, lw.W3, H, lw.b3, lw.scale_e, lw.shift_e,
                                            e ? nullptr : e_raw, e ? nullptr : g->srt_eid, e ? nullptr : m->edge_W1, e ? nullptr : m->edge_b1,
                                            e ? nullptr : m->edge_W2, e ? nullptr : m->edge_b2, stream));
            e = out;
        } else if (e == nullptr) {
            GN_TRY(gnnome_edge_gate_encode_f32(e_raw, g->srt_eid, m->edge_W1, m->edge_b1, m->edge_W2, m->edge_b2, eb[0], E, H, B1, B2, 5 * H, g->srt_src,
                                               g->srt_dst, lw.W3, H, lw.scale_e, lw.shift_e, stream));
            e = eb[0];
        } else if (H == 256 && lw.norm_kind == GNNOME_NORM_AFFINE) {
            float* out = e == eb[0] ? eb[1] : eb[0];
            GN_TRY(gnnome_edge_gate_f32(e, out, E, H, B1, B2, 5 * H, g->srt_src, g->srt_dst, lw.W3, H, lw.norm_kind, lw.scale_e, lw.shift_e, stream));
            e = out;
        } else {
            GN_TRY(gnnome_edge_gate_f32(e, e, E, H, B1, B2, 5 * H, g->srt_src, g->srt_dst, lw.W3, H, lw.norm_kind, lw.scale_e, lw.shift_e, stream));
        }
        GN_TRY(mark(1, i, stream));
        GN_TRY(mark(2, i, stream));
        GN_TRY(gnnome_node_aggregate_f32(e, H, N, A1, A2, A3, 5 * H, g->in_ptr, g->srt_src, g->out_ptr, g->out_pos, g->out_dst, h[cur], H, h[cur ^ 1],
                                         lw.norm_kind, lw.scale_h, lw.shift_h, stream));
        GN_TRY(mark(3, i, stream));
        cur ^= 1;
    }
    GN_TRY(project(h[cur], N, H, m->W_nodes, m->W_nodes_planes, m->b_nodes, 2 * hs, PQ, stream));
    const float *Ps = PQ, *Qd = PQ + hs;
    if (g->transposed) {
        const float* t = Ps; Ps = Qd; Qd = t;
    }
    return gnnome_edge_score_f32(e, E, H, hs, Ps, Qd, 2 * hs, g->srt_src, g->srt_dst, g->srt_eid, m->W1e, m->ld_w1e, m->W2, m->b2, m->W3, m->b3, logits,
                                 nullptr, stream);
}
}
}
```

### gnnome_amd/engine.py

```python
import torch
import torch.nn.functional as F

from . import ops as hip_ops
from ._lib import NORM_AFFINE, NORM_LAYER
from .graph import views_for


class LayerWeights:
    __slots__ = ("Wcat", "bcat", "W3", "b3", "norm", "scale_e", "shift_e", "scale_h", "shift_h", "ref", "gain_e", "planes")


REFERENCE_ORDER_GAIN = 16.0
ARITHMETIC_MODES = ("auto", "reference", "fast")

BUILT_HIDDEN = (64, 128, 256)
BUILT_SCORE_HIDDEN = (32, 64, 128)


def padded_width(width, built=BUILT_HIDDEN, what="hidden_features"):
    for b in built:
        if width <= b:
            return b
    raise ValueError(f"{what}={width}: the HIP kernels are built for widths up to {built[-1]}")


def _pad(t, *shape):
    if tuple(t.shape) == tuple(shape):
        return t
    out = t.new_zeros(shape)
    out[tuple(slice(0, n) for n in t.shape)] = t
    return out


class Prepared:

    def __init__(self, model, device):
        def dev(t):
            return t.detach().to(device=device, dtype=torch.float32).contiguous()

        arithmetic = getattr(model, "arithmetic", "auto")
        self.device = device
        self.model_hidden = model.linear2_node.out_features
        self.hidden = H = padded_width(self.model_hidden)
        ne = model.linear2_node.in_features
        self.enc_node = tuple(dev(t) for t in (model.linear1_node.weight, model.linear1_node.bias,
                                               _pad(model.linear2_node.weight.detach(), H, ne), _pad(model.linear2_node.bias.detach(), H)))
        self.enc_edge = tuple(dev(t) for t in (model.linear1_edge.weight, model.linear1_edge.bias,
                                               _pad(model.linear2_edge.weight.detach(), H, ne), _pad(model.linear2_edge.bias.detach(), H)))
        self.layers = [prepare_layer(conv, device, arithmetic) for conv in model.gnn.convs]
        self.predictor = prepare_predictor(model.predictor, device)
        weights = [t for lw in self.layers for t in (lw.Wcat, lw.W3)] + [self.predictor["_W1"], self.predictor["W2"]]
        amax = max((float(t.abs().max()) if t.numel() else 0.0) for t in weights) if weights else 0.0
        self.force_bf16x6 = not (amax < hip_ops_fp16_max())
        self.range_verified = self.range_failed = None
        self.block = None


def hip_ops_fp16_max():
    return getattr(hip_ops, "FP16_MAX", 65504.0)


def _inputs_key(views, x, e):
    import weakref
    return (weakref.ref(x), x._version, weakref.ref(e), e._version, weakref.ref(views))


def _same_inputs(key, views, x, e):
    return key is not None and key[0]() is x and key[1] == x._version and key[2]() is e and key[3] == e._version and key[4]() is views


def forward_in_range(ops, prep, views, x, e, xd, ed, check=True):
    bf = getattr(ops, "bf16x6_arithmetic", None)
    if bf is None or getattr(ops, "_TUNING", {}).get(10, 0) == 1:
        return run_stack(ops, prep, views, xd, ed)
    if prep.force_bf16x6 or _same_inputs(prep.range_failed, views, x, e):
        with bf():
            return run_stack(ops, prep, views, xd, ed)
    logits = run_stack(ops, prep, views, xd, ed)
    if not check or _same_inputs(prep.range_verified, views, x, e):
        return logits
    if bool(torch.isfinite(logits).all()):
        prep.range_verified = _inputs_key(views, x, e)
        return logits
    prep.range_failed = _inputs_key(views, x, e)
    with bf():
        return run_stack(ops, prep, views, xd, ed)


def _norm_affine(norm_module, device):
    def dev(t):
        return t.detach().to(device=device, dtype=torch.float32).contiguous()

    if isinstance(norm_module, torch.nn.BatchNorm1d):
        var = norm_module.running_var.detach().float().cpu()
        mean = norm_module.running_mean.detach().float().cpu()
        gamma = norm_module.weight.detach().float().cpu()
        beta = norm_module.bias.detach().float().cpu()
        scale = gamma * (1.0 / torch.sqrt(var + norm_module.eps))
        shift = (beta.double() - mean.double() * scale.double()).float()
        width = padded_width(scale.numel())
        return NORM_AFFINE, dev(_pad(scale, width)), dev(_pad(shift, width))
    if isinstance(norm_module, torch.nn.LayerNorm):
        if abs(norm_module.eps - 1e-5) > 1e-12:
            raise ValueError("LayerNorm eps other than 1e-5 is not supported by the HIP kernels")
        own = int(norm_module.weight.numel())
        width = padded_width(own)
        kind = NORM_LAYER if width == own else (NORM_LAYER | (own << 8))
        return kind, dev(_pad(norm_module.weight.detach(), width)), dev(_pad(norm_module.bias.detach(), width))
    raise TypeError(type(norm_module))


def prepare_layer(conv, device, arithmetic=None):
    def dev(t):
        return t.detach().to(device=device, dtype=torch.float32).contiguous()

    arithmetic = getattr(conv, "arithmetic", "auto") if arithmetic is None else arithmetic
    if arithmetic not in ARITHMETIC_MODES:
        raise ValueError(f"arithmetic must be one of {ARITHMETIC_MODES}, got {arithmetic!r}")
    lw = LayerWeights()
    width = conv.B_3.weight.shape[0]
    hidden = padded_width(width)
    W = lambda lin: _pad(lin.weight.detach(), hidden, hidden)
    b = lambda lin: _pad(lin.bias.detach(), hidden)
    lw.Wcat = dev(torch.cat([W(conv.A_1), W(conv.A_2), W(conv.A_3), W(conv.B_1), W(conv.B_2)], 0))
    lw.W3 = dev(W(conv.B_3))
    lw.b3 = dev(b(conv.B_3))
    lw.norm, lw.scale_e, lw.shift_e = _norm_affine(conv.bn_e, device)
    kind_h, lw.scale_h, lw.shift_h = _norm_affine(conv.bn_h, device)
    assert kind_h == lw.norm
    lw.gain_e = float(lw.scale_e.abs().max()) if lw.norm == NORM_AFFINE and lw.scale_e.numel() else 0.0
    can = hip_ops.reference_order_supported(hidden, lw.norm)
    lw.ref = can and (arithmetic == "reference" or (arithmetic == "auto" and lw.gain_e > REFERENCE_ORDER_GAIN))
    planes_ok = getattr(hip_ops, "planes_supported", None)
    lw.planes = hip_ops.weight_planes(lw.Wcat) if (not lw.ref and planes_ok is not None and planes_ok(hidden, 5 * hidden)
                                                   and lw.Wcat.is_cuda) else None
    if lw.ref:
        lw.bcat = dev(torch.cat([b(conv.A_1), b(conv.A_2), b(conv.A_3), b(conv.B_1), b(conv.B_2)], 0))
    else:
        lw.bcat = dev(torch.cat([b(conv.A_1), b(conv.A_2), b(conv.A_3), b(conv.B_1), b(conv.B_2) + b(conv.B_3)], 0))
    return lw


def prepare_predictor(pred, device):
    def dev(t):
        return t.detach().to(device=device, dtype=torch.float32).contiguous()

    hs_model, h3 = pred.W1.weight.shape
    width = h3 // 3
    if pred.W2.out_features != 32 or pred.W3.in_features != 32 or pred.W3.out_features != 1:
        raise ValueError("ScorePredictor tail must be hs -> 32 -> 1 (score_predictor.py:9-10)")
    hidden, hs = padded_width(width), padded_width(hs_model, BUILT_SCORE_HIDDEN, "hidden_edge_scores")
    W1 = dev(torch.cat([_pad(pred.W1.weight.detach()[:, i * width:(i + 1) * width], hs, hidden) for i in range(3)], 1))
    b1 = _pad(pred.W1.bias.detach(), hs)
    W_nodes = torch.cat([W1[:, :hidden], W1[:, hidden:2 * hidden]], 0).contiguous()
    b_nodes = torch.cat([torch.zeros_like(b1), b1])
    planes_ok = getattr(hip_ops, "planes_supported", None)
    planes = (hip_ops.weight_planes(W_nodes) if planes_ok is not None and W_nodes.is_cuda and planes_ok(hidden, 2 * hs) and 2 * hs >= 128 else None)
    return {
        "planes": planes,
        "hidden": hidden, "hs": hs, "model_hidden": width, "W_nodes": W_nodes, "b_nodes": dev(b_nodes), "W1_e": W1[:, 2 * hidden:],
        "W2": dev(_pad(pred.W2.weight.detach(), 32, hs)), "b2": dev(pred.W2.bias),
        "W3": dev(pred.W3.weight.reshape(-1)), "b3": dev(pred.W3.bias.reshape(-1)), "_W1": W1,
    }


def tail_weights(pw):
    return pw["W1_e"], pw["W2"], pw["b2"], pw["W3"], pw["b3"]


class _StateProbe:

    __slots__ = ("device", "arithmetic", "slots", "modules")

    def __init__(self, module, device):
        self.device, self.arithmetic = str(device), getattr(module, "arithmetic", "auto")
        self.slots, self.modules = [], []
        for sub in module.modules():
            self.modules.append((sub._modules, len(sub._modules)))
            for table in (sub._parameters, sub._buffers):
                for name, t in table.items():
                    if t is not None:
                        self.slots.append((table, name, t, t._version, t.data_ptr()))

    def unchanged(self, module, device):
        if str(device) != self.device or getattr(module, "arithmetic", "auto") != self.arithmetic:
            return False
        for table, count in self.modules:
            if len(table) != count:
                return False
        for table, name, t, version, ptr in self.slots:
            if table.get(name) is not t or t._version != version or t.data_ptr() != ptr:
                return False
        return True


def prepared_for(module, device, build):
    cached = module.__dict__.get("_gnnome_prepared")
    if cached is None or not cached[0].unchanged(module, device):
        probe = _StateProbe(module, device)
        cached = (probe, build(module, device))
        module.__dict__["_gnnome_prepared"] = cached
    return cached[1]


def compute_device(*tensors):
    for t in tensors:
        if t.is_cuda:
            return t.device
    if not torch.cuda.is_available():
        raise RuntimeError("gnnome_amd runs on an MI355X only: no HIP device is visible and there is no CPU fallback")
    return torch.device("cuda", torch.cuda.current_device())


def _refuse_training(module):
    if module.training and (torch.is_grad_enabled() or any(isinstance(m, torch.nn.BatchNorm1d) for m in module.modules())):
        raise NotImplementedError("train mode is supported through SymGatedGCNModel.forward only; call .eval() for the "
                                  "layer-level API")
    if torch.is_grad_enabled() and any(p.requires_grad for p in module.parameters()):
        raise NotImplementedError("gnnome_amd layer-level forward is inference-only: its outputs carry no autograd history - wrap the "
                                  "call in torch.no_grad() (or freeze the parameters), or train through SymGatedGCNModel.forward")



def gate_update(ops, lw, views, e, B1, B2, scratch=None):
    if scratch is not None and e.shape[1] == 256 and lw.norm == 0 and getattr(ops, "edge_gate_out_of_place_at_256", False):
        spare = scratch.get("e_spare")
        if spare is None or spare.shape != e.shape or spare.device != e.device:
            spare = torch.empty_like(e)
        ops.edge_gate(e, B1, B2, views, lw.W3, lw.norm, lw.scale_e, lw.shift_e, out=spare)
        scratch["e_spare"] = e
        return spare
    ops.edge_gate(e, B1, B2, views, lw.W3, lw.norm, lw.scale_e, lw.shift_e)
    return e


def project(ops, lw, h, out=None):
    if lw.ref:
        return ops.linear_ref(h, lw.Wcat, lw.bcat, out=out)
    return ops.linear(h, lw.Wcat, lw.bcat, out=out, planes=lw.planes)


def gate(ops, lw, views, e, B1, B2, raw_edges=None, scratch=None):
    if lw.ref:
        return ops.edge_gate_ref(e, B1, B2, views, lw.W3, lw.b3, lw.scale_e, lw.shift_e, raw_edges=raw_edges)
    if e is None:
        return ops.edge_gate_encode(raw_edges[0], raw_edges[1], B1, B2, views, lw.W3, lw.scale_e, lw.shift_e)
    return gate_update(ops, lw, views, e, B1, B2, scratch)


def aggregate_then_project(ops, lw, views, e, A1, A2, A3, h, then):
    n = h.shape[0]
    side = ops.side_stream(h.device)
    main = torch.cuda.current_stream(h.device)
    h_out = torch.empty_like(h)
    P_next = torch.empty((n, then.width), dtype=torch.float32, device=h.device)
    bounds = [n * i // PIPELINE_CHUNKS // 32 * 32 for i in range(PIPELINE_CHUNKS)] + [n]
    for lo, hi in zip(bounds[:-1], bounds[1:]):
        ops.node_aggregate(e, A1, A2, A3, views, h, lw.norm, lw.scale_h, lw.shift_h, node_range=(lo, hi), out=h_out)
        done = torch.cuda.Event()
        done.record(main)
        with torch.cuda.stream(side):
            side.wait_event(done)
            then(h_out[lo:hi], out=P_next[lo:hi])
    main.wait_stream(side)
    return h_out, P_next


import os as _os
ONE_CALL_FORWARD = _os.environ.get("GNNOME_ONE_CALL_FORWARD", "1") != "0"
PIPELINE_CHUNKS = 1
PIPELINE_MIN_NODES = 1 << 15


class _Projection:

    def __init__(self, fn, W, b):
        self.fn, self.W, self.b, self.width = fn, W, b, W.shape[0]

    def __call__(self, rows, out=None):
        return self.fn(rows, self.W, self.b, out=out)


def layer_projection(ops, lw):
    if lw.ref:
        return _Projection(ops.linear_ref, lw.Wcat, lw.bcat)
    return _Projection(lambda rows, W, b, out=None: ops.linear(rows, W, b, out=out, planes=lw.planes), lw.Wcat, lw.bcat)


def layer_step(ops, lw, views, h, e, n_out=None, raw_edges=None, scratch=None, P=None, then=None):
    H = h.shape[1]
    if P is None:
        P = project(ops, lw, h)
    A1, A2, A3, B1, B2 = (P[:, i * H:(i + 1) * H] for i in range(5))
    if views.transposed:
        A2, A3, B1, B2 = A3, A2, B2, B1
    e = gate(ops, lw, views, e, B1, B2, raw_edges, scratch)
    if then is not None:
        h_new, P_next = aggregate_then_project(ops, lw, views, e, A1, A2, A3, h, then)
        return h_new, e, P_next
    return ops.node_aggregate(e, A1, A2, A3, views, h, lw.norm, lw.scale_h, lw.shift_h, num_nodes_out=n_out), e, None


def encode_nodes(ops, views, x, enc):
    gather = getattr(views, "node_gather", None)
    if gather is None:
        return ops.encode(x, *enc)
    return ops.encode(x, *enc, gather=gather, rows=views.num_nodes)


def encode_edges(ops, prep, views, e_raw):
    fuse = getattr(ops, "can_fuse_edge_encoder", None)
    if prep.layers and fuse is not None and fuse(e_raw, prep.enc_edge, prep.hidden, prep.layers[0].norm, prep.layers[0].Wcat):
        return None
    return ops.encode(e_raw, *prep.enc_edge, gather=views.srt_eid, rows=views.num_edges)


def predictor_projection(ops, pw):
    return _Projection(lambda rows, W, b, out=None: ops.linear(rows, W, b, out=out, planes=pw.get("planes")), pw["W_nodes"], pw["b_nodes"])


def score_step(ops, pw, views, h, e, logits, n_edges=None, PQ=None):
    hs = pw["hs"]
    if PQ is None:
        PQ = ops.linear(h, pw["W_nodes"], pw["b_nodes"], planes=pw.get("planes"))
    Ps, Qd = PQ[:, :hs], PQ[:, hs:]
    if views.transposed:
        Ps, Qd = Qd, Ps
    return ops.edge_score(e, Ps, Qd, views, pw["W1_e"], pw["W2"], pw["b2"], pw["W3"], pw["b3"], logits, num_edges=n_edges)


def run_stack(ops, prep, views, x, e_raw, logits=None):
    pipelined = getattr(ops, "side_stream", None) is not None and PIPELINE_CHUNKS > 1 and views.num_nodes >= PIPELINE_MIN_NODES
    one_call = getattr(ops, "model_forward", None)
    if (ONE_CALL_FORWARD and one_call is not None and not pipelined
            and not getattr(ops, "STREAM_AGGREGATE", False) and isinstance(views, ops.GraphViews) and x.is_cuda and x.is_contiguous()
            and e_raw.is_contiguous()):
        block = getattr(prep, "block", None)
        if block is None:
            block = prep.block = ops.ModelBlock(prep)
        with ops.node_records_for(views, prep.hidden):
            return one_call(block, views, x, e_raw, logits)
    h = encode_nodes(ops, views, x, prep.enc_node)
    e = encode_edges(ops, prep, views, e_raw)
    scratch = {}
    P = None
    for i, lw in enumerate(prep.layers):
        then = None
        if pipelined:
            then = layer_projection(ops, prep.layers[i + 1]) if i + 1 < len(prep.layers) else predictor_projection(ops, prep.predictor)
        h, e, P = layer_step(ops, lw, views, h, e, raw_edges=(e_raw, prep.enc_edge), scratch=scratch, P=P, then=then)
    if logits is None:
        logits = torch.empty(views.num_edges, dtype=torch.float32, device=h.device)
    score_step(ops, prep.predictor, views, h, e, logits, PQ=P)
    return logits



def project_rows(product, h, n_own, finish, width):
    P = torch.empty((h.shape[0], width), dtype=torch.float32, device=h.device)
    if n_own > 0:
        product(h[:n_own], out=P[:n_own])
    finish()
    if h.shape[0] > n_own:
        product(h[n_own:], out=P[n_own:])
    return P


def scored_rows(ops, e, rows, count):
    if rows is None:
        return e
    return ops.gather_rows(e, rows) if count > 0 else e[:0]


def score_tail(ops, e, Ps, Qd, w_tail, score_views, count, total, z1_out=None, pad=None, assemble=None):
    kw = {} if z1_out is None else dict(z1_out=z1_out)
    if assemble is None:
        logits = torch.empty(total, dtype=torch.float32, device=e.device)
        ops.edge_score(e, Ps, Qd, score_views, *w_tail, logits, num_edges=count, **kw)
        return logits
    piece = torch.empty(pad, dtype=torch.float32, device=e.device)
    if count > 0:
        ops.edge_score(e, Ps, Qd, score_views, *w_tail, piece, num_edges=count, scatter_to_edge_id=False, **kw)
    return assemble(piece)



def model_forward(model, graph, x, e):
    if model.training:
        from .train import train_forward
        return train_forward(model, graph, x, e).to(x.device)
    out_device = x.device
    device = compute_device(x, e)
    prep = prepared_for(model, device, Prepared)
    views = views_for(graph, device, node_order=getattr(model, "node_order", "input"))
    if x.shape[0] != views.num_nodes or e.shape[0] != views.num_edges:
        raise ValueError(f"x has {x.shape[0]} rows for {views.num_nodes} nodes, e has {e.shape[0]} rows for {views.num_edges} edges")
    with torch.no_grad():
        xd = x.detach().to(device=device, dtype=torch.float32).contiguous()
        ed = e.detach().to(device=device, dtype=torch.float32).contiguous()
# ... 51 lines not shown
```

### gnnome_amd/ops.py

```python
import ctypes

import torch

from . import _lib
from ._lib import NORM_AFFINE, NORM_LAYER


def _ptr(t):
    return ctypes.c_void_p(t.data_ptr() if t is not None and t.numel() > 0 else None)


def _stream(device):
    return ctypes.c_void_p(torch.cuda.current_stream(device).cuda_stream)


_SIDE_STREAMS = {}


def side_stream(device):
    s = _SIDE_STREAMS.get(device.index)
    if s is None:
        s = _SIDE_STREAMS[device.index] = torch.cuda.Stream(device=device, priority=-1)
    return s

# ... 135 lines not shown
STREAM_SLOTS = 62


class StreamSchedule:

    __slots__ = ("chunks", "chunk_node", "chunk_steps", "steps", "edge_meta", "node_pend", "pend_nodes", "counters", "num_pending",
                 "num_far", "num_overflow", "max_live", "max_steps", "total_steps", "far_fraction", "usable", "why")

    def __init__(self, views, chunks=None, slots=None):
        lib = _lib.load()
        dev, n, e = views.device, views.num_nodes, views.num_edges
        self.usable, self.why = False, ""
        if e == 0 or n == 0:
            self.why = "empty graph"
            return
        cus = torch.cuda.get_device_properties(dev).multi_processor_count
        self.chunks = int(chunks) if chunks else max(2 * cus, -(-e // STREAM_ROWS_PER_CHUNK))
        slots = STREAM_SLOTS if slots is None else int(slots)
        cap, scratch = ctypes.c_int64(0), ctypes.c_size_t(0)
        _lib.check(lib.gnnome_stream_schedule_sizes(n, e, STREAM_ROWS_PER_STEP, ctypes.byref(cap), ctypes.byref(scratch)), "stream_schedule_sizes")
        mk = lambda k: torch.empty(k, dtype=torch.int32, device=dev)
        self.chunk_node, self.chunk_steps = mk(self.chunks + 1), mk(self.chunks)
        self.steps = torch.empty((int(cap.value), 4), dtype=torch.int32, device=dev)
        self.edge_meta = torch.empty(e, dtype=torch.uint8, device=dev)
        self.node_pend, self.pend_nodes, self.counters = mk(n), mk(n), mk(8)
        ws = torch.empty(int(scratch.value), dtype=torch.uint8, device=dev)
        with _on(dev):
            _lib.check(lib.gnnome_build_stream_schedule(n, e, _ptr(views.in_ptr), _ptr(views.srt_src), _ptr(views.out_ptr), _ptr(views.out_pos),
                                                        _ptr(views.out_dst), self.chunks, STREAM_ROWS_PER_STEP, slots, _ptr(self.chunk_node),
                                                        _ptr(self.chunk_steps), _ptr(self.steps), _ptr(self.edge_meta), _ptr(self.node_pend),
                                                        _ptr(self.pend_nodes), _ptr(self.counters), _ptr(ws), ws.numel(), _stream(dev)),
                       "build_stream_schedule")
            ws.record_stream(torch.cuda.current_stream(dev))
        c = self.counters.tolist()
        self.num_pending, self.num_far, self.num_overflow, self.max_live, self.max_steps = c[0], c[1], c[2], c[3], c[4]
        self.total_steps = int(self.chunk_steps.sum())
        self.far_fraction = self.num_far / e
        if self.far_fraction > STREAM_MAX_FAR:
            self.why = f"{self.far_fraction:.0%} of the rows are far: the numbering has no locality (or the graph is too small for its chunks)"
        elif self.max_steps > 4 * (self.total_steps // self.chunks + 16):
            self.why = f"a chunk of {self.max_steps} steps against {self.total_steps // self.chunks} on average: a hub"
        else:
            self.usable = True


def stream_schedule_for(views, e_rows, num_nodes_out, node_range, norm_kind):
    if (not STREAM_AGGREGATE or norm_kind != NORM_AFFINE or node_range is not None or views.num_edges < STREAM_MIN_EDGES
            or e_rows != views.num_edges or (num_nodes_out is not None and num_nodes_out != views.num_nodes) or not hasattr(views, "stream_schedule")):
        return None
    sched = views.stream_schedule()
    return sched if sched.usable else None


edge_gate_out_of_place_at_256 = True


_TUNING = {}


def set_tuning(key, value):
    _lib.check(_lib.load().gnnome_set_tuning(int(key), int(value)), "set_tuning")
    _TUNING[int(key)] = int(value)


FP16_MAX = 65504.0


class bf16x6_arithmetic:

    def __enter__(self):
        self.prev = _TUNING.get(10, 0)
        if self.prev != 1:
            set_tuning(10, 1)
        return self

    def __exit__(self, *exc):
        if self.prev != 1:
            set_tuning(10, self.prev)


def encode(x, W1, b1, W2, b2, gather=None, rows=None):
    lib = _lib.load()
    x, _ = _rows(x.contiguous(), "encode.in")
    hidden, hidden_ne = W2.shape[0], W1.shape[0]
    rows = int(x.shape[0] if rows is None else rows)
    out = torch.empty((rows, hidden), dtype=torch.float32, device=x.device)
    with _on(x.device):
        _lib.check(lib.gnnome_encode_f32(_ptr(x), rows, x.shape[1], _ptr(gather), _ptr(W1), _ptr(b1), hidden_ne, _ptr(W2),
                                         _ptr(b2), hidden, _ptr(out), _stream(x.device)), "encode_f32")
    return out


def planes_supported(K, Nout):
    return K in (64, 128, 256) and Nout % (32 if K == 256 else 64) == 0 and 0 < Nout <= 1536


def weight_planes(W):
    lib = _lib.load()
    W, ldw = _rows(W, "weight_planes.W")
    Nout, K = W.shape
    planes = torch.empty(Nout * K * 2, dtype=torch.float16, device=W.device)
    with _on(W.device):
        _lib.check(lib.gnnome_weight_planes_f16(_ptr(W), ldw, Nout, K, _ptr(planes), _stream(W.device)), "weight_planes_f16")
    return planes


def _planes_route(A, lda, W, ldw, out, ldc, accumulate, given):
    return (not accumulate and lda % 4 == 0 and ldw % 4 == 0 and ldc % 4 == 0 and A.data_ptr() % 16 == 0 and W.data_ptr() % 16 == 0
            and out.data_ptr() % 16 == 0 and A.data_ptr() != out.data_ptr()
            and _lib.load().gnnome_linear_planes_route(A.shape[0], A.shape[1], W.shape[0], 1 if given else 0) == 1)


def linear(A, W, bias, out=None, accumulate=False, planes=None):
    lib = _lib.load()
    A, lda = _rows(A, "linear.A")
    W, ldw = _rows(W, "linear.W")
    M, K = A.shape
    Nout = W.shape[0]
    if out is None:
        out = torch.empty((M, Nout), dtype=torch.float32, device=A.device)
    out, ldc = _rows(out, "linear.out")
    if _planes_route(A, lda, W, ldw, out, ldc, accumulate, planes is not None):
        if planes is None:
            planes = weight_planes(W)
        with _on(A.device):
            _lib.check(lib.gnnome_linear_planes_f32(_ptr(A), M, K, lda, _ptr(planes), _ptr(bias), Nout, _ptr(out), ldc, _stream(A.device)),
                       "linear_planes_f32")
        return out
    with _on(A.device):
        fn = lib.gnnome_linear_acc_f32 if accumulate else lib.gnnome_linear_f32
        _lib.check(fn(_ptr(A), M, K, lda, _ptr(W), ldw, _ptr(bias), Nout, _ptr(out), ldc, _stream(A.device)), "linear_f32")
    return out


def _dptr(t):
    return t.data_ptr() if t is not None and t.numel() > 0 else None


class ModelBlock:

    def __init__(self, prep):
        pw = prep.predictor
        self.keep = [prep.enc_node, prep.enc_edge, prep.layers, pw]
        n = len(prep.layers)
        self.layers = (_lib.LayerParams * max(n, 1))()
        for lp, lw in zip(self.layers, prep.layers):
            for name in ("Wcat", "bcat", "W3", "b3", "scale_e", "shift_e", "scale_h", "shift_h"):
                t = getattr(lw, name)
                if not (t.is_cuda and t.dtype == torch.float32 and t.is_contiguous()):
                    raise TypeError(f"model_forward: layer tensor {name} must be a contiguous CUDA float32 tensor")
                setattr(lp, name, _dptr(t))
            lp.Wcat_planes = _dptr(lw.planes)
            lp.norm_kind, lp.reference_order = int(lw.norm), int(bool(lw.ref))
        m = self.params = _lib.ModelParams()
        m.hidden, m.num_layers, m.score_hidden = prep.hidden, n, pw["hs"]
        (W1, b1, W2, b2), (V1, c1, V2, c2) = prep.enc_node, prep.enc_edge
        m.hidden_ne, m.node_features, m.edge_features = W1.shape[0], W1.shape[1], V1.shape[1]
        if V1.shape[0] != W1.shape[0]:
            raise ValueError("model_forward: the two encoders share hidden_ne (models/full_graph.py:13-16)")
        m.node_W1, m.node_b1, m.node_W2, m.node_b2 = (_dptr(t) for t in (W1, b1, W2, b2))
        m.edge_W1, m.edge_b1, m.edge_W2, m.edge_b2 = (_dptr(t) for t in (V1, c1, V2, c2))
        m.layers_host = ctypes.cast(self.layers, ctypes.POINTER(_lib.LayerParams))
        W1e = pw["W1_e"]
        if W1e.stride(1) != 1:
            raise ValueError("model_forward: predictor W1's edge block must have contiguous rows")
        m.W_nodes, m.W_nodes_planes, m.b_nodes = _dptr(pw["W_nodes"]), _dptr(pw.get("planes")), _dptr(pw["b_nodes"])
        m.W1e, m.ld_w1e = _dptr(W1e), W1e.stride(0)
        m.W2, m.b2, m.W3, m.b3 = (_dptr(pw[k]) for k in ("W2", "b2", "W3", "b3"))


def _views_block(views):
    blk = getattr(views, "_c_block", None)
    if blk is None:
        blk = _lib.Views()
        blk.num_nodes, blk.num_edges = views.num_nodes, views.num_edges
        for name in ("in_ptr", "srt_src", "srt_dst", "srt_eid", "out_ptr", "out_pos", "out_dst"):
            setattr(blk, name, _dptr(getattr(views, name)))
        blk.node_gather = _dptr(getattr(views, "node_gather", None))
        blk.transposed = int(bool(views.transposed))
        try:
            views._c_block = blk
        except AttributeError:
            pass
    return blk


_WS_BYTES = {}


FORWARD_BUFFERS = _os.environ.get("GNNOME_FORWARD_BUFFERS", "separate")


NODE_RECORDS_MAX_HIDDEN = int(_os.environ.get("GNNOME_NODE_RECORDS", "64"))


class node_records_for:

    def __init__(self, views, hidden):
        self.on = (0 < hidden <= NODE_RECORDS_MAX_HIDDEN and isinstance(views, GraphViews) and views.num_nodes > 0 and views.num_edges > 0
                   and not torch.cuda.is_current_stream_capturing())
        self.views = views

    def __enter__(self):
        if self.on:
            _lib.check(_lib.load().gnnome_debug_node_records(_ptr(self.views.node_records())), "debug_node_records")
        return self

    def __exit__(self, *exc):
        if self.on:
            _lib.load().gnnome_debug_node_records(None)


def model_forward(block, views, x, e_raw, logits=None):
    lib = _lib.load()
    dev = x.device
    m = block.params
    n, e, H, hs = views.num_nodes, views.num_edges, m.hidden, m.score_hidden
    if logits is None:
        logits = torch.empty(e, dtype=torch.float32, device=dev)
    if FORWARD_BUFFERS == "block":
        key = (n, e, H, hs)
        need = _WS_BYTES.get(key)
        if need is None:
            nb = ctypes.c_size_t(0)
            _lib.check(lib.gnnome_model_forward_workspace_bytes(n, e, H, hs, ctypes.byref(nb)), "model_forward_workspace_bytes")
            need = _WS_BYTES[key] = nb.value
        ws = torch.empty(max(need, 256), dtype=torch.uint8, device=dev)
        with _on(dev):
            _lib.check(lib.gnnome_model_forward_f32(ctypes.byref(m), ctypes.byref(_views_block(views)), _ptr(x), _ptr(e_raw), _ptr(logits), _ptr(ws), need,
                                                    _stream(dev)), "model_forward_f32")
        return logits
    shapes = {"h0": (n, H), "h1": (n, H), "P": (n, 5 * H), "PQ": (n, 2 * hs), "e0": (e, H)}
    if H == 256:
        shapes["e1"] = (e, H)
    vb = _views_block(views)

    def run(t):
        bufs = _lib.ForwardBuffers()
        bufs.h[0], bufs.h[1], bufs.P, bufs.PQ = t["h0"].data_ptr(), t["h1"].data_ptr(), t["P"].data_ptr(), t["PQ"].data_ptr()
        bufs.e[0], bufs.e[1] = t["e0"].data_ptr(), (t["e1"].data_ptr() if "e1" in t else None)
        _lib.check(lib.gnnome_model_forward_buffers_f32(ctypes.byref(m), ctypes.byref(vb), _ptr(x), _ptr(e_raw), _ptr(logits), ctypes.byref(bufs),
                                                        _stream(dev)), "model_forward_buffers_f32")

    with _on(dev):
        run(_placed_buffers(dev, shapes, run))
    return logits


TUNE_PLACEMENT = _os.environ.get("GNNOME_TUNE_PLACEMENT", "1") != "0"
PLACEMENT_AFTER_USES = 3
PLACEMENT_CANDIDATES = 4
PLACEMENT_MIN_TOTAL, PLACEMENT_MAX_BUFFER = 64 << 20, 1 << 30
PLACEMENT_KEPT = 3


class _Placed:
    __slots__ = ("uses", "tried", "bufs", "log")

    def __init__(self):
        self.uses, self.tried, self.bufs, self.log = 0, False, None, None


_PLACED = {}


def _placed_buffers(dev, shapes, run):
    mk = lambda name: torch.empty((max(shapes[name][0], 1), shapes[name][1]), dtype=torch.float32, device=dev)
    sizes = [max(r, 1) * c * 4 for r, c in shapes.values()]
    if not TUNE_PLACEMENT or sum(sizes) < PLACEMENT_MIN_TOTAL or max(sizes) >= PLACEMENT_MAX_BUFFER or torch.cuda.is_current_stream_capturing():
        return {name: mk(name) for name in shapes}
    stream = torch.cuda.current_stream(dev)
    key = (dev.index, stream.cuda_stream) + tuple(sorted(shapes.items()))
    st = _PLACED.get(key)
    if st is None:
        st = _PLACED[key] = _Placed()
    if st.bufs is not None:
        return st.bufs
    st.uses += 1
    cur = {name: mk(name) for name in shapes}
    free = torch.cuda.mem_get_info(dev)[0]
    if st.tried or st.uses < PLACEMENT_AFTER_USES or free < 2 * (PLACEMENT_CANDIDATES + 1) * sum(sizes):
        return cur
    st.tried = True

    def time_of(t):
        run(t)
        t0, t1 = torch.cuda.Event(enable_timing=True), torch.cuda.Event(enable_timing=True)
        t0.record(stream)
        run(t)
        run(t)
        t1.record(stream)
        t1.synchronize()
        return t0.elapsed_time(t1) / 2

    for _ in range(3):
        run(cur)
    best, log, rejected = time_of(cur), [], []
    log.append(("start", best))
    for group in (tuple(k for k in ("e0", "e1") if k in shapes), ("P",), ("h0", "h1", "PQ")):
        for _ in range(PLACEMENT_CANDIDATES):
            cand = dict(cur)
            for name in group:
                cand[name] = mk(name)
            t = time_of(cand)
            log.append((group, t))
            if t < best * 0.997:
                rejected.extend(cur[name] for name in group)
                cur, best = cand, t
            else:
                rejected.extend(cand[name] for name in group)
    st.bufs, st.log = cur, log
    del rejected, cand
    try:
        torch.cuda.empty_cache()
    except RuntimeError:
        pass
    kept = [k for k, v in _PLACED.items() if v.bufs is not None]
    for k in kept[:-PLACEMENT_KEPT]:
        _PLACED[k].bufs = None
    return cur


def edge_gate(e, B1h, B2h, views, W3, norm_kind, scale, shift, out=None, num_edges=None):
    lib = _lib.load()
    e, _ = _rows(e, "edge_gate.e")
    B1h, ldn = _rows(B1h, "edge_gate.B1h")
    B2h, ldn2 = _rows(B2h, "edge_gate.B2h")
    assert ldn == ldn2 and e.is_contiguous()
    W3, ldw = _rows(W3, "edge_gate.W3")
    out = e if out is None else out
    E = int(e.shape[0] if num_edges is None else num_edges)
    with _on(e.device):
        _lib.check(lib.gnnome_edge_gate_f32(_ptr(e), _ptr(out), E, e.shape[1], _ptr(B1h), _ptr(B2h), ldn,
                                            _ptr(views.srt_src), _ptr(views.srt_dst), _ptr(W3), ldw, norm_kind, _ptr(scale),
                                            _ptr(shift), _stream(e.device)), "edge_gate_f32")
    return out


def can_fuse_edge_encoder(e_raw, enc, hidden, norm_kind, B1h):
    widths = (64, 128, 256) if _TUNING.get(10, 0) == 0 and _TUNING.get(0, 0) == 0 else (64, 128)
    return (e_raw.dim() == 2 and e_raw.shape[1] == 2 and enc[0].shape == (16, 2) and hidden in widths
            and norm_kind == NORM_AFFINE and e_raw.shape[0] > 0 and B1h.stride(0) % 4 == 0 and B1h.data_ptr() % 16 == 0)


def edge_gate_encode(e_raw, enc, B1h, B2h, views, W3, scale, shift):
    lib = _lib.load()
    e_raw = _dense(e_raw, "edge_gate_encode.e_raw")
    B1h, ldn = _rows(B1h, "edge_gate_encode.B1h")
    B2h, _ = _rows(B2h, "edge_gate_encode.B2h")
    W3, ldw = _rows(W3, "edge_gate_encode.W3")
    E, H = views.num_edges, W3.shape[0]
    out = torch.empty((E, H), dtype=torch.float32, device=e_raw.device)
    W1, b1, W2, b2 = enc
    with _on(e_raw.device):
        _lib.check(lib.gnnome_edge_gate_encode_f32(_ptr(e_raw), _ptr(views.srt_eid), _ptr(W1), _ptr(b1), _ptr(W2), _ptr(b2),
                                                   _ptr(out), E, H, _ptr(B1h), _ptr(B2h), ldn, _ptr(views.srt_src),
                                                   _ptr(views.srt_dst), _ptr(W3), ldw, _ptr(scale), _ptr(shift),
                                                   _stream(e_raw.device)), "edge_gate_encode_f32")
    return out


def linear_ref(A, W, bias, out=None):
    lib = _lib.load()
    A, lda = _rows(A, "linear_ref.A")
    W, ldw = _rows(W, "linear_ref.W")
    M, K = A.shape
    Nout = W.shape[0]
    if out is None:
        out = torch.empty((M, Nout), dtype=torch.float32, device=A.device)
    out, ldc = _rows(out, "linear_ref.out")
    with _on(A.device):
        _lib.check(lib.gnnome_linear_ref_f32(_ptr(A), M, K, lda, _ptr(W), ldw, _ptr(bias), Nout, _ptr(out), ldc, _stream(A.device)),
                   "linear_ref_f32")
    return out


def reference_order_supported(hidden, norm_kind, B1h=None):
    return hidden in (64, 128, 256) and norm_kind == NORM_AFFINE


def edge_gate_ref(e, B1h, B2h, views, W3, b3, scale, shift, raw_edges=None, num_edges=None):
    lib = _lib.load()
    B1h, ldn = _rows(B1h, "edge_gate_ref.B1h")
    B2h, ldn2 = _rows(B2h, "edge_gate_ref.B2h")
    W3, ldw = _rows(W3, "edge_gate_ref.W3")
    assert ldn == ldn2
    H = W3.shape[0]
    if e is None:
        e_raw, (W1, b1, W2, b2) = raw_edges
        e_raw = _dense(e_raw, "edge_gate_ref.e_raw")
        E = views.num_edges if num_edges is None else int(num_edges)
        out = torch.empty((views.num_edges, H), dtype=torch.float32, device=e_raw.device)
        enc = (_ptr(e_raw), _ptr(views.srt_eid), _ptr(W1), _ptr(b1), _ptr(W2), _ptr(b2))
        e_in = _ptr(None)
    else:
        e = _dense(e, "edge_gate_ref.e")
        E = int(e.shape[0] if num_edges is None else num_edges)
        out, e_in = e, _ptr(e)
        enc = (_ptr(None),) * 6
    with _on(out.device):
        _lib.check(lib.gnnome_edge_gate_ref_f32(e_in, _ptr(out), E, H, _ptr(B1h), _ptr(B2h), ldn, _ptr(views.srt_src),
                                                _ptr(views.srt_dst), _ptr(W3), ldw, _ptr(b3), _ptr(scale), _ptr(shift), *enc,
                                                _stream(out.device)), "edge_gate_ref_f32")
    return out


def node_aggregate(e, A1h, A2h, A3h, views, h_in, norm_kind, scale, shift, num_nodes_out=None, node_range=None, out=None):
    lib = _lib.load()
    A1h, ldn = _rows(A1h, "node_aggregate.A1h")
    A2h, l2 = _rows(A2h, "node_aggregate.A2h")
    A3h, l3 = _rows(A3h, "node_aggregate.A3h")
    h_in, ldh = _rows(h_in, "node_aggregate.h_in")
    assert ldn == l2 == l3
    hidden = h_in.shape[1]
    n_out = int(h_in.shape[0] if num_nodes_out is None else num_nodes_out)
    h_out = torch.empty((h_in.shape[0], hidden), dtype=torch.float32, device=h_in.device) if out is None else out
    assert h_out.is_contiguous() and h_out.shape == (h_in.shape[0], hidden) and h_out.dtype == torch.float32
    sched = None
    if STREAM_AGGREGATE and getattr(views, "num_nodes", None) == h_in.shape[0]:
        sched = stream_schedule_for(views, e.shape[0], num_nodes_out, node_range, norm_kind)
    with _on(h_in.device):
        if sched is not None:
            pend = torch.empty((max(sched.num_pending, 1), 3, hidden), dtype=torch.float32, device=h_in.device)
            _lib.check(lib.gnnome_node_aggregate_stream_f32(_ptr(e), hidden, n_out, views.num_edges, _ptr(A1h), _ptr(A2h), _ptr(A3h), ldn, _ptr(views.in_ptr),
                                                            _ptr(views.srt_src), _ptr(views.out_ptr), _ptr(views.out_pos), _ptr(views.out_dst),
                                                            _ptr(h_in), ldh, _ptr(h_out), _ptr(scale), _ptr(shift), sched.chunks,
                                                            STREAM_ROWS_PER_STEP, STREAM_SLOTS, _ptr(sched.chunk_node), _ptr(sched.chunk_steps),
                                                            _ptr(sched.steps), _ptr(sched.edge_meta), _ptr(sched.node_pend), _ptr(sched.pend_nodes),
                                                            _ptr(sched.counters), sched.num_pending, _ptr(pend), _stream(h_in.device)),
                       "node_aggregate_stream_f32")
        elif node_range is None:
            _lib.check(lib.gnnome_node_aggregate_f32(_ptr(e), hidden, n_out, _ptr(A1h), _ptr(A2h), _ptr(A3h), ldn,
                                                     _ptr(views.in_ptr), _ptr(views.srt_src), _ptr(views.out_ptr),
                                                     _ptr(views.out_pos), _ptr(views.out_dst), _ptr(h_in), ldh, _ptr(h_out),
                                                     norm_kind, _ptr(scale), _ptr(shift), _stream(h_in.device)),
                       "node_aggregate_f32")
        else:
            assert out is not None, "node_aggregate(node_range=...) writes rows of a caller-owned `out`"
            _lib.check(lib.gnnome_node_aggregate_range_f32(_ptr(e), hidden, n_out, int(node_range[0]), int(node_range[1]), _ptr(A1h),
                                                           _ptr(A2h), _ptr(A3h), ldn, _ptr(views.in_ptr), _ptr(views.srt_src),
                                                           _ptr(views.out_ptr), _ptr(views.out_pos), _ptr(views.out_dst), _ptr(h_in),
                                                           ldh, _ptr(h_out), norm_kind, _ptr(scale), _ptr(shift),
                                                           _stream(h_in.device)), "node_aggregate_range_f32")
    return h_out


def node_aggregate_in(e, A1h, A2h, views, h_in, norm_kind, scale, shift, num_nodes_out=None, node_range=None, out=None):
    lib = _lib.load()
    A1h, ldn = _rows(A1h, "node_aggregate_in.A1h")
    A2h, l2 = _rows(A2h, "node_aggregate_in.A2h")
    h_in, ldh = _rows(h_in, "node_aggregate_in.h_in")
    assert ldn == l2
    hidden = h_in.shape[1]
    n_out = int(h_in.shape[0] if num_nodes_out is None else num_nodes_out)
    h_out = torch.empty((h_in.shape[0], hidden), dtype=torch.float32, device=h_in.device) if out is None else out
    assert h_out.is_contiguous() and h_out.shape == (h_in.shape[0], hidden) and h_out.dtype == torch.float32
    with _on(h_in.device):
        if node_range is None:
            _lib.check(lib.gnnome_node_aggregate_in_f32(_ptr(e), hidden, n_out, _ptr(A1h), _ptr(A2h), ldn, _ptr(views.in_ptr),
                                                        _ptr(views.srt_src), _ptr(h_in), ldh, _ptr(h_out), norm_kind, _ptr(scale),
                                                        _ptr(shift), _stream(h_in.device)), "node_aggregate_in_f32")
        else:
            assert out is not None, "node_aggregate_in(node_range=...) writes rows of a caller-owned `out`"
            _lib.check(lib.gnnome_node_aggregate_in_range_f32(_ptr(e), hidden, n_out, int(node_range[0]), int(node_range[1]), _ptr(A1h),
                                                              _ptr(A2h), ldn, _ptr(views.in_ptr), _ptr(views.srt_src), _ptr(h_in), ldh,
                                                              _ptr(h_out), norm_kind, _ptr(scale), _ptr(shift), _stream(h_in.device)),
                       "node_aggregate_in_range_f32")
    return h_out


def node_neighbour_sum(h, views, sscale=None, dscale=None, both=False, out=None):
    lib = _lib.load()
    h, ldh = _rows(h, "node_neighbour_sum.h")
    n, hidden = h.shape
    if n != views.num_nodes:
        raise ValueError(f"node_neighbour_sum: h has {n} rows for {views.num_nodes} nodes")
    if out is None:
        out = torch.empty((n, hidden), dtype=torch.float32, device=h.device)
    out, ldo = _rows(out, "node_neighbour_sum.out")
    if out.shape != h.shape or out.device != h.device:
        raise ValueError(f"node_neighbour_sum: out is {tuple(out.shape)} on {out.device}, h is {tuple(h.shape)} on {h.device}")
    for name, t in (("sscale", sscale), ("dscale", dscale)):
        if t is not None and (_f32(t, "node_neighbour_sum." + name).shape != (n,) or not t.is_contiguous()):
            raise ValueError(f"node_neighbour_sum: {name} is one contiguous float per node")
    lists = [(views.in_ptr, views.srt_src), (views.out_ptr, views.out_dst)]
    if views.transposed:
        lists.reverse()
    (ptr_a, idx_a), (ptr_b, idx_b) = lists
    with _on(h.device):
        _lib.check(lib.gnnome_node_neighbour_sum_f32(_ptr(h), ldh, hidden, n, _ptr(ptr_a), _ptr(idx_a), _ptr(ptr_b) if both else None,
                                                     _ptr(idx_b) if both else None, _ptr(sscale), _ptr(dscale), _ptr(out), ldo,
                                                     _stream(h.device)), "node_neighbour_sum_f32")
    return out


def node_attention_sum(feat, views, el, er, bias=None, negative_slope=0.2, both=False, out=None):
    lib = _lib.load()
    feat, ldf = _rows(feat, "node_attention_sum.feat")
    el, ld_el = _rows(el, "node_attention_sum.el")
    er, ld_er = _rows(er, "node_attention_sum.er")
    n, width = feat.shape
    heads = 3
    if n != views.num_nodes:
        raise ValueError(f"node_attention_sum: feat has {n} rows for {views.num_nodes} nodes")
    if width % heads or el.shape != (n, 4) or er.shape != (n, 4) or el.device != feat.device or er.device != feat.device:
        raise ValueError(f"node_attention_sum: feat is [N, 3H], el and er are [N, 4] (three heads and a pad) on feat's device; got "
                         f"{tuple(feat.shape)}, {tuple(el.shape)}, {tuple(er.shape)}")
    if out is None:
        out = torch.empty((n, width), dtype=torch.float32, device=feat.device)
    out, ldo = _rows(out, "node_attention_sum.out")
    if out.shape != feat.shape or out.device != feat.device:
# ... 1077 lines not shown
```

### include/gnnome_hip.h

```cpp
#ifndef GNNOME_HIP_H
#define GNNOME_HIP_H

#include <stddef.h>
#include <stdint.h>

#ifdef __cplusplus
extern "C" {
#endif

#define GNNOME_ABI_VERSION 32

#define GNNOME_OK 0
#define GNNOME_EINVAL (-1)
#define GNNOME_EHIP (-2)
#define GNNOME_EWORKSPACE (-3)

#define GNNOME_NORM_AFFINE 0
#define GNNOME_NORM_LAYER 1
#define GNNOME_NORM_LAYER_OVER(w) (GNNOME_NORM_LAYER | ((w) << 8))

int gnnome_abi_version(void);
const char* gnnome_last_error(void);

int gnnome_set_tuning(int key, int value);

int gnnome_debug_gate_profile(void* counters);

int gnnome_graph_views_workspace_bytes(int64_t num_nodes, int64_t num_edges, size_t* bytes_host);
int gnnome_build_graph_views(const int32_t* src, const int32_t* dst, int64_t num_nodes, int64_t num_edges,
                             int32_t* in_ptr, int32_t* srt_src, int32_t* srt_dst, int32_t* srt_eid,
                             int32_t* out_ptr, int32_t* out_pos, int32_t* out_dst, void* workspace,
                             size_t workspace_bytes, void* stream);

int gnnome_encode_f32(const float* in, int64_t rows, int in_features, const int32_t* gather,
                      const float* W1, const float* b1, int hidden_ne, const float* W2, const float* b2,
                      int hidden, float* out, void* stream);

int gnnome_linear_f32(const float* A, int64_t M, int K, int lda, const float* W, int ldw, const float* bias,
                      int Nout, float* C, int ldc, void* stream);
int gnnome_linear_acc_f32(const float* A, int64_t M, int K, int lda, const float* W, int ldw, const float* bias,
                          int Nout, float* C, int ldc, void* stream);

int gnnome_weight_planes_f16(const float* W, int ldw, int Nout, int K, void* planes, void* stream);
int gnnome_linear_planes_f32(const float* A, int64_t M, int K, int lda, const void* planes, const float* bias, int Nout, float* C,
                             int ldc, void* stream);
int gnnome_linear_planes_route(int64_t M, int K, int Nout, int given_planes);

int gnnome_edge_gate_f32(const float* e_in, float* e_out, int64_t num_edges, int hidden,
                         const float* B1h, const float* B2h, int ld_node, const int32_t* srt_src,
                         const int32_t* srt_dst, const float* W3, int ldw, int norm_kind,
                         const float* norm_scale, const float* norm_shift, void* stream);

int gnnome_edge_gate_encode_f32(const float* e_raw, const int32_t* srt_eid, const float* encW1, const float* encb1,
                                const float* encW2, const float* encb2, float* e_out, int64_t num_edges, int hidden,
                                const float* B1h, const float* B2h, int ld_node, const int32_t* srt_src,
                                const int32_t* srt_dst, const float* W3, int ldw, const float* norm_scale,
                                const float* norm_shift, void* stream);

int gnnome_linear_ref_f32(const float* A, int64_t M, int K, int lda, const float* W, int ldw, const float* bias, int Nout,
                          float* C, int ldc, void* stream);
int gnnome_edge_gate_ref_f32(const float* e_in, float* e_out, int64_t num_edges, int hidden, const float* B1h,
                             const float* B2h, int ld_node, const int32_t* srt_src, const int32_t* srt_dst, const float* W3,
                             int ldw, const float* b3, const float* norm_scale, const float* norm_shift, const float* e_raw,
                             const int32_t* srt_eid, const float* encW1, const float* encb1, const float* encW2,
                             const float* encb2, void* stream);

int gnnome_node_aggregate_f32(const float* e, int hidden, int64_t num_nodes_out, const float* A1h,
                              const float* A2h, const float* A3h, int ld_node, const int32_t* in_ptr,
                              const int32_t* srt_src, const int32_t* out_ptr, const int32_t* out_pos,
                              const int32_t* out_dst, const float* h_in, int ld_h, float* h_out, int norm_kind,
                              const float* norm_scale, const float* norm_shift, void* stream);

int gnnome_build_node_records(const int32_t* in_ptr, const int32_t* srt_src, const int32_t* out_ptr, const int32_t* out_pos,
                              const int32_t* out_dst, int64_t num_nodes, int32_t* records, void* stream);
int gnnome_debug_node_records(const int32_t* records);

int gnnome_node_aggregate_range_f32(const float* e, int hidden, int64_t num_nodes_out, int64_t node_begin, int64_t node_end,
                                    const float* A1h, const float* A2h, const float* A3h, int ld_node, const int32_t* in_ptr,
                                    const int32_t* srt_src, const int32_t* out_ptr, const int32_t* out_pos,
                                    const int32_t* out_dst, const float* h_in, int ld_h, float* h_out, int norm_kind,
                                    const float* norm_scale, const float* norm_shift, void* stream);

int gnnome_node_aggregate_in_f32(const float* e, int hidden, int64_t num_nodes_out, const float* A1h, const float* A2h, int ld_node,
                                 const int32_t* in_ptr, const int32_t* srt_src, const float* h_in, int ld_h, float* h_out,
                                 int norm_kind, const float* norm_scale, const float* norm_shift, void* stream);

int gnnome_node_aggregate_in_range_f32(const float* e, int hidden, int64_t num_nodes_out, int64_t node_begin, int64_t node_end,
                                       const float* A1h, const float* A2h, int ld_node, const int32_t* in_ptr, const int32_t* srt_src,
                                       const float* h_in, int ld_h, float* h_out, int norm_kind, const float* norm_scale,
                                       const float* norm_shift, void* stream);

int gnnome_node_aggregate_in_raw_f32(const float* e, int hidden, int64_t num_nodes, const float* A1h, const float* A2h, int ld_node,
                                     const int32_t* in_ptr, const int32_t* srt_src, float* v_out, float* aux0, float* aux1,
                                     void* stream);

int gnnome_node_aggregate_in_bwd_f32(const float* e, int64_t num_edges, int hidden, int64_t num_nodes, const float* Tf, const float* Uf,
                                     const float* A2h, int ld_node, const int32_t* in_ptr, const int32_t* srt_src,
                                     const int32_t* out_ptr, const int32_t* out_pos, const int32_t* out_dst, float* de, float* dA2h,
                                     void* stream);

int gnnome_node_aggregate_in_raw_part_f32(const float* e, int hidden, int64_t num_nodes_out, int64_t num_nodes_local, const float* A1h,
                                          const float* A2h, int ld_node, const int32_t* in_ptr, const int32_t* srt_src, float* v_out,
                                          float* aux0, float* aux1, void* stream);
int gnnome_node_aggregate_in_bwd_part_f32(const float* e, int64_t num_edges, int hidden, int64_t num_nodes_out, int64_t num_nodes_local,
                                          const float* Tf, const float* Uf, const float* A2h, int ld_node, const int32_t* in_ptr,
                                          const int32_t* srt_src, const int32_t* out_ptr, const int32_t* out_pos, const int32_t* out_dst,
                                          float* de, float* dA2h, void* stream);

int gnnome_node_neighbour_sum_f32(const float* h, int ld_h, int hidden, int64_t num_nodes, const int32_t* in_ptr, const int32_t* srt_src,
                                  const int32_t* out_ptr, const int32_t* out_dst, const float* sscale, const float* dscale, float* out,
                                  int ld_out, void* stream);

int gnnome_relu_rows_f32(float* x, int ld, int64_t rows, int hidden, void* stream);

int gnnome_node_neighbour_sum_bwd_f32(const float* g, int ld_g, int hidden, int64_t num_nodes, const int32_t* out_ptr, const int32_t* out_dst,
                                      const int32_t* in_ptr, const int32_t* srt_src, int both, const float* rscale, const float* oscale,
                                      const float* add, int ld_add, const float* mult, int ld_mult, const float* y, int ld_y, float* out,
                                      int ld_out, void* stream);

int gnnome_node_neighbour_sum_part_f32(const float* h, int ld_h, int hidden, int64_t num_nodes_out, int64_t num_nodes_local,
                                       const int32_t* rows, int64_t num_rows, const int32_t* in_ptr, const int32_t* srt_src,
                                       const int32_t* out_ptr, const int32_t* out_dst, const float* sscale, const float* dscale, float* out,
                                       int ld_out, void* stream);
int gnnome_node_neighbour_sum_bwd_part_f32(const float* g, int ld_g, int hidden, int64_t num_nodes_out, int64_t num_nodes_local,
                                           const int32_t* rows, int64_t num_rows, const int32_t* out_ptr, const int32_t* out_dst,
                                           const int32_t* in_ptr, const int32_t* srt_src, int both, const float* rscale, const float* oscale,
                                           const float* add, int ld_add, const float* mult, int ld_mult, const float* y, int ld_y,
                                           float* out, int ld_out, void* stream);

int gnnome_relu_mul_rows_f32(float* x, int ld, const float* mult, int ld_mult, int64_t rows, int hidden, int relu, void* stream);

int gnnome_node_attention_sum_f32(const float* feat, int ld_feat, const float* el, int ld_el, const float* er, int ld_er, int hidden,
                                  int heads, int64_t num_nodes, const int32_t* in_ptr, const int32_t* srt_src, const int32_t* out_ptr,
                                  const int32_t* out_dst, float negative_slope, const float* bias, float* out, int ld_out, void* stream);

int gnnome_node_attention_sum_stats_f32(const float* feat, int ld_feat, const float* el, int ld_el, const float* er, int ld_er, int hidden,
                                        int heads, int64_t num_nodes, const int32_t* in_ptr, const int32_t* srt_src, const int32_t* out_ptr,
                                        const int32_t* out_dst, float negative_slope, const float* bias, float* out, int ld_out, float* stats,
                                        int ld_stats, void* stream);

int gnnome_node_attention_sum_bwd_f32(const float* g, int ld_g, const float* feat, int ld_feat, const float* el, int ld_el, const float* er,
                                      int ld_er, const float* out, int ld_out, const float* bias, const float* stats, int ld_stats, int hidden,
                                      int heads, int64_t num_nodes, const int32_t* in_ptr, const int32_t* srt_src, const int32_t* out_ptr,
                                      const int32_t* out_dst, int both, float negative_slope, float* dfeat, int ld_dfeat, float* del, int ld_del,
                                      float* der, int ld_der, float* work, void* stream);

int gnnome_node_attention_sum_part_f32(const float* feat, int ld_feat, const float* el, int ld_el, const float* er, int ld_er, int hidden,
                                       int heads, int64_t num_nodes_out, int64_t num_nodes_local, const int32_t* in_ptr,
                                       const int32_t* srt_src, const int32_t* out_ptr, const int32_t* out_dst, float negative_slope,
                                       const float* bias, float* out, int ld_out, void* stream);
int gnnome_node_attention_sum_stats_part_f32(const float* feat, int ld_feat, const float* el, int ld_el, const float* er, int ld_er,
                                             int hidden, int heads, int64_t num_nodes_out, int64_t num_nodes_local, const int32_t* in_ptr,
                                             const int32_t* srt_src, const int32_t* out_ptr, const int32_t* out_dst, float negative_slope,
                                             const float* bias, float* out, int ld_out, float* stats, int ld_stats, void* stream);
int gnnome_node_attention_sum_bwd_dst_part_f32(const float* g, int ld_g, const float* feat, int ld_feat, const float* el, int ld_el,
                                               const float* er, int ld_er, const float* out, int ld_out, const float* bias,
                                               const float* stats, int ld_stats, int hidden, int heads, int64_t num_nodes_out,
                                               int64_t num_nodes_local, const int32_t* in_ptr, const int32_t* srt_src,
                                               const int32_t* out_ptr, const int32_t* out_dst, int both, float negative_slope, float* der,
                                               int ld_der, float* work, void* stream);
int gnnome_node_attention_sum_bwd_src_part_f32(const float* g, int ld_g, const float* feat, int ld_feat, const float* el, int ld_el,
                                               const float* work, int hidden, int heads, int64_t num_nodes_out, int64_t num_nodes_local,
                                               const int32_t* out_ptr, const int32_t* out_dst, const int32_t* in_ptr,
                                               const int32_t* srt_src, int both, float negative_slope, float* dfeat, int ld_dfeat,
                                               float* del, int ld_del, void* stream);

int gnnome_stream_schedule_sizes(int64_t num_nodes, int64_t num_edges, int rows_per_step, int64_t* steps_capacity_host,
                                 size_t* scratch_bytes_host);
int gnnome_build_stream_schedule(int64_t num_nodes, int64_t num_edges, const int32_t* in_ptr, const int32_t* srt_src,
                                 const int32_t* out_ptr, const int32_t* out_pos, const int32_t* out_dst, int num_chunks,
                                 int rows_per_step, int num_slots, int32_t* chunk_node, int32_t* chunk_steps, int32_t* steps,
                                 uint8_t* edge_meta, int32_t* node_pend, int32_t* pend_nodes, int32_t* counters, void* scratch,
                                 size_t scratch_bytes, void* stream);
int gnnome_node_aggregate_stream_f32(const float* e, int hidden, int64_t num_nodes, int64_t num_edges, const float* A1h, const float* A2h,
                                     const float* A3h, int ld_node, const int32_t* in_ptr, const int32_t* srt_src,
                                     const int32_t* out_ptr, const int32_t* out_pos, const int32_t* out_dst, const float* h_in,
                                     int ld_h, float* h_out, const float* norm_scale, const float* norm_shift, int num_chunks,
                                     int rows_per_step, int num_slots, const int32_t* chunk_node, const int32_t* chunk_steps,
                                     const int32_t* steps, const uint8_t* edge_meta, const int32_t* node_pend,
                                     const int32_t* pend_nodes, const int32_t* counters, int64_t num_pending, float* pend_rows,
                                     void* stream);

int gnnome_edge_score_f32(const float* e, int64_t num_edges, int hidden, int hidden_edge_scores,
                          const float* Ps, const float* Qd, int ld_node, const int32_t* srt_src,
                          const int32_t* srt_dst, const int32_t* srt_eid, const float* W1e, int ldw1,
                          const float* W2, const float* b2, const float* W3, const float* b3, float* logits,
                          float* z1_out , void* stream);

typedef struct gnnome_layer_params {
    const float* Wcat;
    const void* Wcat_planes;
    const float* bcat;
    const float* W3;
    const float* b3;
    const float* scale_e;
    const float* shift_e;
    const float* scale_h;
    const float* shift_h;
    int32_t norm_kind;
    int32_t reference_order;
} gnnome_layer_params;

typedef struct gnnome_model_params {
    int32_t hidden, hidden_ne, num_layers, score_hidden, node_features, edge_features;
    const float *node_W1, *node_b1, *node_W2, *node_b2;
    const float *edge_W1, *edge_b1, *edge_W2, *edge_b2;
    const gnnome_layer_params* layers_host;
    const float* W_nodes;
    const void* W_nodes_planes;
    const float* b_nodes;
    const float* W1e;
    int32_t ld_w1e, reserved;
    const float *W2, *b2, *W3, *b3;
} gnnome_model_params;

typedef struct gnnome_views {
    int64_t num_nodes, num_edges;
    const int32_t *in_ptr, *srt_src, *srt_dst, *srt_eid, *out_ptr, *out_pos, *out_dst;
    const int32_t* node_gather;
    int32_t transposed, reserved;
} gnnome_views;

int gnnome_debug_forward_events(void* gate_start, void* gate_stop, void* aggregate_start, void* aggregate_stop, int layer);
int gnnome_model_forward_workspace_bytes(int64_t num_nodes, int64_t num_edges, int hidden, int score_hidden, size_t* bytes_host);
int gnnome_model_forward_f32(const gnnome_model_params* params_host, const gnnome_views* views_host, const float* x, const float* e_raw,
                             float* logits, void* workspace, size_t workspace_bytes, void* stream);
typedef struct gnnome_forward_buffers {
    float* h[2];
    float* P;
    float* e[2];
    float* PQ;
} gnnome_forward_buffers;
int gnnome_model_forward_buffers_f32(const gnnome_model_params* params_host, const gnnome_views* views_host, const float* x, const float* e_raw,
                                     float* logits, const gnnome_forward_buffers* buffers_host, void* stream);


int gnnome_edge_gate_raw_f32(const float* e_in, float* x_out, int64_t num_edges, int hidden, const float* B1h,
                             const float* B2h, int ld_node, const int32_t* srt_src, const int32_t* srt_dst,
                             const float* W3, int ldw, void* stream);

int gnnome_edge_gate_raw_stats_rows(int hidden, int* rows_host);
int gnnome_edge_gate_raw_stats_f32(const float* e_in, float* x_out, int64_t num_edges, int hidden, const float* B1h,
                                   const float* B2h, int ld_node, const int32_t* srt_src, const int32_t* srt_dst,
                                   const float* W3, int ldw, const float* center, float* stats_partial, void* stream);
int gnnome_edge_gate_bn_f32(const float* e_in, float* e_out, float* x_out, int64_t num_edges, int hidden, const float* B1h,
                            const float* B2h, int ld_node, const int32_t* srt_src, const int32_t* srt_dst, const float* W3, int ldw,
                            const float* scale, const float* shift, void* stream);

int gnnome_node_aggregate_raw_f32(const float* e, int hidden, int64_t num_nodes, int mode, const float* A1h,
                                  const float* A2h, const float* A3h, int ld_node, const int32_t* in_ptr,
                                  const int32_t* srt_src, const int32_t* out_ptr, const int32_t* out_pos,
                                  const int32_t* out_dst, float* v_out, float* aux0, float* aux1, float* aux2,
                                  float* aux3, void* stream);

int gnnome_colsum_workspace_bytes(size_t* bytes_host);
int gnnome_colsum2_f32(const float* x, const float* y, int64_t rows, int hidden, const float* center, float* s1,
                       float* s2, void* workspace, size_t workspace_bytes, void* stream);

int gnnome_bn_relu_res_f32(const float* x, const float* scale, const float* shift, const float* res, int64_t rows,
                           int hidden, float* out, void* stream);

int gnnome_bn_bwd_stats_f32(const float* dy, const float* x, const float* scale, const float* shift,
                            const float* mean, int64_t rows, int hidden, float* s1, float* s2, void* workspace,
                            size_t workspace_bytes, void* stream);
int gnnome_bn_bwd_apply_f32(const float* dy, const float* x, const float* scale, const float* shift, int64_t rows,
                            int hidden, const float* a, const float* c1, const float* c2, const float* mean,
                            const float* rstd, float* dx, void* stream);

int gnnome_bn_bwd_apply_tables_f32(const float* dy, const float* x, const float* scale, const float* shift, int64_t rows, int hidden,
                                   const float* a, const float* c1, const float* c2, const float* mean, const float* rstd,
                                   const float* rdf, const float* hf, const float* rdb, const float* hb, float* dx, float* Tf, float* Uf,
                                   float* Tb, float* Ub, unsigned* amax_bits, void* stream);

int gnnome_ln_relu_res_f32(const float* x, const float* gamma, const float* beta, const float* res, int64_t rows, int hidden,
                           int norm_width, float* out, void* stream);
int gnnome_ln_bwd_f32(const float* dy, const float* x, const float* gamma, const float* beta, int64_t rows, int hidden, int norm_width,
                      float* dx, float* dbeta, float* dgamma, void* workspace, size_t workspace_bytes, void* stream);

int gnnome_mul23_f32(const float* a, const float* b, const float* c, int64_t count, float* o1, float* o2, void* stream);
int gnnome_add_f32(const float* a, const float* b, int64_t count, float* out, void* stream);
int gnnome_relu_bwd_f32(const float* dy, const float* y, int64_t count, float* dx, void* stream);

int gnnome_segment_sum_f32(const float* X, int width, const int32_t* ptr, const int32_t* pos, int64_t num_nodes,
                           float* out, int ld_out, void* stream);

int gnnome_segment_sum2_f32(const float* X, int width, const int32_t* in_ptr, const int32_t* out_ptr, const int32_t* out_pos,
                            int64_t num_nodes, float* out_in, int ld_in, float* out_out, int ld_out, void* stream);

int gnnome_wgrad_workspace_bytes(int64_t rows, int Ka, int Kb, size_t* bytes_host);
int gnnome_wgrad_f32(const float* A, int lda, int Ka, const float* B, int ldb, int Kb, int64_t rows, float* C, int ldc,
                     void* workspace, size_t workspace_bytes, void* stream);
int gnnome_wgrad_scaled_f32(const float* A, int lda, int Ka, const float* B, int ldb, int Kb, int64_t rows, const unsigned* amax_bits,
                            float* C, int ldc, void* workspace, size_t workspace_bytes, void* stream);
int gnnome_wgrad_blocks_scaled_f32(const float* const* A_blocks, int num_blocks, int block_width, int lda, const float* B, int ldb, int Kb,
                                   int64_t rows, const unsigned* amax_bits, float* C, int ldc, float* colsum, void* workspace,
                                   size_t workspace_bytes, void* stream);
int gnnome_linear_blocks_scaled_f32(const float* const* A_blocks, int num_blocks, int block_width, int64_t M, int lda, const float* W, int ldw,
                                    int Nout, const unsigned* amax_bits, float* C, int ldc, int accumulate, void* stream);
int gnnome_segment_sum2_amax_f32(const float* X, int width, const int32_t* in_ptr, const int32_t* out_ptr, const int32_t* out_pos,
                                 int64_t num_nodes, float* out_in, int ld_in, float* out_out, int ld_out, unsigned* amax_bits, void* stream);

int gnnome_wgrad_blocks_f32(const float* const* A_blocks, int num_blocks, int block_width, int lda, const float* B, int ldb,
                            int Kb, int64_t rows, float* C, int ldc, float* colsum, void* workspace, size_t workspace_bytes,
                            void* stream);

int gnnome_linear_blocks_f32(const float* const* A_blocks, int num_blocks, int block_width, int64_t M, int lda, const float* W,
                             int ldw, int Nout, float* C, int ldc, int accumulate, void* stream);

int gnnome_score_tail_bwd_f32(const float* z1, const float* dscore, const int32_t* srt_eid, int64_t num_edges,
                              int hidden_edge_scores, const float* W2, const float* b2, const float* W3, float* dz1,
                              float* dz2, float* u, void* stream);

int gnnome_agg_edge_bwd_f32(const float* e, int64_t num_edges, int hidden, const float* Tf, const float* Uf,
                            const float* Tb, const float* Ub, const float* A2h, const float* A3h, int ld_node,
                            const int32_t* srt_src, const int32_t* srt_dst, float* de, void* stream);

int gnnome_encode_hidden_f32(const float* in, int64_t rows, int in_features, const int32_t* gather, const float* W1,
                             const float* b1, int hidden_ne, float* t, void* stream);

int gnnome_gather_rows_f32(const float* in, int ld_in, const int32_t* idx, int64_t rows, int width, float* out,
                           int ld_out, void* stream);

int gnnome_scatter_add_rows_f32(const float* in, int ld_in, const int32_t* idx, int64_t rows, int width, float* out,
                                int ld_out, void* stream);

int gnnome_closure_workspace_bytes(size_t* bytes_host);

int gnnome_degree_features_f32(const int32_t* in_ptr, const int32_t* out_ptr, int64_t num_nodes, int reverse, float* x,
                               void* workspace, size_t workspace_bytes, void* stream);

int gnnome_edge_features_f32(const float* overlap_length, const float* overlap_similarity, int64_t num_edges, float* e,
                             void* workspace, size_t workspace_bytes, void* stream);

int gnnome_edge_loss_f32(const float* logits, const float* logits_rev, const float* labels, int64_t num_edges,
                         const float* pos_weight, float alpha, float grad_scale, float* loss, float* dlogits,
                         float* dlogits_rev, int64_t* tfpn, void* workspace, size_t workspace_bytes, void* stream);

int gnnome_bn_bwd_dgrad_f32(float* C, const float* X, int64_t rows, int64_t rows_once, int hidden, const float* scale, const float* shift,
                            const float* a, const float* c1, const float* c2, const float* mean, const float* rstd,
                            const float* W, int ldw, float* dxe, void* stream);
int gnnome_bn_bwd_dgrad_amax_f32(float* C, const float* X, int64_t rows, int64_t rows_once, int hidden, const float* scale, const float* shift,
                                 const float* a, const float* c1, const float* c2, const float* mean, const float* rstd,
                                 const float* W, int ldw, float* dxe, unsigned* amax_bits, void* stream);
int gnnome_bn_bwd_dgrad_out_f32(const float* C_in, float* C_out, const float* X, int64_t rows, int64_t rows_once, int hidden,
                                const float* scale, const float* shift, const float* a, const float* c1, const float* c2,
                                const float* mean, const float* rstd, const float* W, int ldw, float* dxe, void* stream);
int gnnome_bn_bwd_dgrad_out_amax_f32(const float* C_in, float* C_out, const float* X, int64_t rows, int64_t rows_once, int hidden,
                                     const float* scale, const float* shift, const float* a, const float* c1, const float* c2,
                                     const float* mean, const float* rstd, const float* W, int ldw, float* dxe, unsigned* amax_bits, void* stream);

int gnnome_agg_edge_bwd_stats_f32(const float* e, int64_t num_edges, int hidden, const float* Tf, const float* Uf,
                                  const float* Tb, const float* Ub, const float* A2h, const float* A3h, int ld_node,
                                  const int32_t* srt_src, const int32_t* srt_dst, float* de, const float* xe, const float* scale,
                                  const float* shift, const float* mean, float* s1, float* s2, void* workspace,
                                  size_t workspace_bytes, void* stream);

int gnnome_agg_bwd_fused_f32(const float* e, int64_t num_nodes, int64_t num_edges, int hidden, const float* Tf, const float* Uf,
                             const float* Tb, const float* Ub, const float* A2h, const float* A3h, int ld_node, const int32_t* in_ptr,
                             const int32_t* srt_src, const int32_t* out_ptr, const int32_t* out_pos, const int32_t* out_dst, float* de,
                             const float* xe, const float* scale, const float* shift, const float* mean, float* sum_in, float* sum_out,
                             float* s1, float* s2, unsigned* amax_bits, void* workspace, size_t workspace_bytes, void* stream);

int gnnome_bn_train_finish_f32(const float* d1, const float* d2, const float* center, int64_t rows, int hidden, const float* gamma,
                               const float* beta, float* running_mean, float* running_var, int64_t* num_batches_tracked,
                               float momentum, float eps, int updates, float* mean, float* rstd, float* scale, float* shift,
                               void* stream);
int gnnome_bn_bwd_terms_f32(const float* s1, const float* s2, const float* rstd, int64_t rows, int hidden, float* s2h, float* c1,
                            float* c2, void* stream);
int gnnome_pack_layer_f32(const float* const* weights5, const float* const* biases5, const float* B3_weight, const float* B3_bias,
                          int hidden, float* Wcat, float* bcat, float* WcatT, float* W3T, void* stream);
int gnnome_gate_center_f32(const float* e, int64_t num_edges, int hidden, const float* B1h, const float* B2h, int ld_node,
                           const int32_t* srt_src, const int32_t* srt_dst, const float* W3, int ldw, float* center, void* stream);

int gnnome_greedy_walks_workspace_bytes(int64_t num_nodes, int num_candidates, size_t* bytes_host);
int gnnome_greedy_walks(const int32_t* succ_ptr, const int32_t* succ_nbr, const int32_t* succ_eid, const float* logp,
                        const int32_t* prefix_len, const int32_t* read_len, const uint8_t* visited, int64_t num_nodes,
                        const int32_t* cand_src, const int32_t* cand_dst, const int32_t* cand_eid, int num_candidates,
                        int32_t* walks_f, int32_t* walks_b, int64_t capacity, int32_t* len_f, int32_t* len_b, float* sum_f,
                        float* sum_b, int64_t* contig_len, int32_t* status, void* workspace, size_t workspace_bytes, void* stream);
int gnnome_greedy_walks_opts(const int32_t* succ_ptr, const int32_t* succ_nbr, const int32_t* succ_eid, const float* logp,
                             const int32_t* prefix_len, const int32_t* read_len, const uint8_t* visited, int64_t num_nodes,
                             const int32_t* cand_src, const int32_t* cand_dst, const int32_t* cand_eid, int num_candidates,
                             int32_t* walks_f, int32_t* walks_b, int64_t capacity, int32_t* len_f, int32_t* len_b, float* sum_f,
                             float* sum_b, int64_t* contig_len, int32_t* status, void* workspace, size_t workspace_bytes,
                             float stop_logp, int choice_mode, int64_t seed, void* stream);
int gnnome_candidate_table(const int32_t* cand_src, const int32_t* cand_dst, const int32_t* len_f, const int32_t* len_b,
                           const float* sum_f, const float* sum_b, const int64_t* contig_len, int num_candidates, double* table,
// ... 169 lines not shown
```

Baseline: 253.6 million.

## Precompute layer-0 encoder fold once and add persistent range encoder kernel

The W3·encW2 encoder fold for the first layer's edge gate is now computed once at model preparation and passed through a new folded forward entry point, so each forward skips the fold kernel launch. The node/edge encoder for the F=2, M=16 case gets a new persistent 1024-thread kernel that walks a contiguous row range per block with software-prefetched inputs. Module change detection also now compares child identity. The cached fold becomes stale if weights change without re-preparation; the change detection update is meant to cover that.

```diff
diff --git a/gnnome_amd/_lib.py b/gnnome_amd/_lib.py
--- a/gnnome_amd/_lib.py
+++ b/gnnome_amd/_lib.py
@@ -25,6 +25,8 @@
     "gnnome_linear_planes_route": [_l, _i, _i, _i],
     "gnnome_edge_gate_f32": [_p, _p, _l, _i, _p, _p, _i, _p, _p, _p, _i, _i, _p, _p, _p],
     "gnnome_edge_gate_encode_f32": [_p, _p, _p, _p, _p, _p, _p, _l, _i, _p, _p, _i, _p, _p, _p, _i, _p, _p, _p],
+    "gnnome_encoder_fold_f32": [_p, _i, _p, _p, _i, _p, _p],
+    "gnnome_edge_gate_encode_folded_f32": [_p, _p, _p, _p, _p, _p, _p, _l, _i, _p, _p, _i, _p, _p, _p, _i, _p, _p, _p, _p],
     "gnnome_linear_ref_f32": [_p, _l, _i, _i, _p, _i, _p, _i, _p, _i, _p],
     "gnnome_edge_gate_ref_f32": [_p, _p, _l, _i, _p, _p, _i, _p, _p, _p, _i, _p, _p, _p, _p, _p, _p, _p, _p, _p, _p],
     "gnnome_node_aggregate_f32": [_p, _i, _l, _p, _p, _p, _i, _p, _p, _p, _p, _p, _p, _i, _p, _i, _p, _p, _p],
@@ -62,6 +64,7 @@
     "gnnome_model_forward_workspace_bytes": [_l, _l, _i, _i, ctypes.POINTER(_sz)],
     "gnnome_model_forward_f32": [_p, _p, _p, _p, _p, _p, _sz, _p],
     "gnnome_model_forward_buffers_f32": [_p, _p, _p, _p, _p, _p, _p],
+    "gnnome_model_forward_buffers_folded_f32": [_p, _p, _p, _p, _p, _p, _p, _p],
     "gnnome_edge_gate_raw_f32": [_p, _p, _l, _i, _p, _p, _i, _p, _p, _p, _i, _p],
     "gnnome_edge_gate_raw_stats_rows": [_i, ctypes.POINTER(_i)],
     "gnnome_edge_gate_raw_stats_f32": [_p, _p, _l, _i, _p, _p, _i, _p, _p, _p, _i, _p, _p, _p],
diff --git a/gnnome_amd/csrc/common.h b/gnnome_amd/csrc/common.h
--- a/gnnome_amd/csrc/common.h
+++ b/gnnome_amd/csrc/common.h
@@ -9,7 +9,7 @@
 
 void set_error(const char* fmt, ...);
 
-enum { kTuneGateVariant = 0, kTuneGateAblation = 1, kTuneLinearVariant = 2, kTuneGateTileOrder = 3, kTuneGateExperiment = 4, kTuneAggLdsKiB = 5, kTuneAggHubs = 6, kTuneAggVariant = 7, kTuneRefVariant = 8, kTuneOverlapBand = 9, kTuneArith = 10, kTuneAggAddr64 = 11, kTuneProjectSchedule = 12, kTuneCount = 16 };
+enum { kTuneGateVariant = 0, kTuneGateAblation = 1, kTuneLinearVariant = 2, kTuneGateTileOrder = 3, kTuneGateExperiment = 4, kTuneAggLdsKiB = 5, kTuneAggHubs = 6, kTuneAggVariant = 7, kTuneRefVariant = 8, kTuneOverlapBand = 9, kTuneArith = 10, kTuneAggAddr64 = 11, kTuneProjectSchedule = 12, kTuneForwardEnds = 13, kTuneCount = 16 };
 int tuning(int key);
 
 struct GateEnc {
diff --git a/gnnome_amd/csrc/edge_gate.hip b/gnnome_amd/csrc/edge_gate.hip
--- a/gnnome_amd/csrc/edge_gate.hip
+++ b/gnnome_amd/csrc/edge_gate.hip
@@ -649,6 +649,15 @@
                                            const float* B1h, const float* B2h, int ld_node, const int32_t* srt_src,
                                            const int32_t* srt_dst, const float* W3, int ldw, const float* norm_scale,
                                            const float* norm_shift, void* stream) {
+    return gnnome_edge_gate_encode_folded_f32(e_raw, srt_eid, encW1, encb1, encW2, encb2, e_out, num_edges, hidden, B1h, B2h, ld_node, srt_src,
+                                              srt_dst, W3, ldw, norm_scale, norm_shift, nullptr, stream);
+}
+
+extern "C" int gnnome_edge_gate_encode_folded_f32(const float* e_raw, const int32_t* srt_eid, const float* encW1, const float* encb1,
+                                                  const float* encW2, const float* encb2, float* e_out, int64_t num_edges, int hidden,
+                                                  const float* B1h, const float* B2h, int ld_node, const int32_t* srt_src,
+                                                  const int32_t* srt_dst, const float* W3, int ldw, const float* norm_scale,
+                                                  const float* norm_shift, const float* fold, void* stream) {
     using namespace gnnome;
     GN_REQUIRE(num_edges >= 0, "edge_gate_encode: negative edge count");
     if (num_edges == 0) return GNNOME_OK;
@@ -658,7 +667,9 @@
                "edge_gate_encode: hidden=%d not in {64,128,256 (default kernels)}", hidden);
     GN_REQUIRE(ld_node % 4 == 0 && ldw % 4 == 0 && ((uintptr_t)B1h % 16 == 0) && ((uintptr_t)B2h % 16 == 0) && ((uintptr_t)W3 % 16 == 0),
                "edge_gate_encode: alignment");
-    const GateEnc enc = {e_raw, srt_eid, encW1, encb1, encW2, encb2};
+    GN_REQUIRE((uintptr_t)fold % 16 == 0, "edge_gate_encode: fold must be 16-byte aligned");
+    const bool folded = fold != nullptr && (hidden == 128 || hidden == 256);
+    const GateEnc enc = {e_raw, srt_eid, encW1, encb1, encW2, encb2, folded ? fold : nullptr, folded ? fold + (size_t)hidden * 16 : nullptr};
     hipStream_t s = (hipStream_t)stream;
     if (hidden == 256) {
         GN_REQUIRE((uintptr_t)e_out % 16 == 0, "edge_gate_encode: e_out must be 16-byte aligned");
diff --git a/gnnome_amd/csrc/edge_gate_bf.hip b/gnnome_amd/csrc/edge_gate_bf.hip
--- a/gnnome_amd/csrc/edge_gate_bf.hip
+++ b/gnnome_amd/csrc/edge_gate_bf.hip
@@ -840,6 +840,18 @@
     }
 }
 
+static int launch_fold(const float* W3, int ldw, const float* W2, const float* b2, int H, float* fold, hipStream_t s) {
+    hipLaunchKernelGGL(k_fold_encoder, dim3((H * 17 + 3) / 4), dim3(256), 0, s, W3, ldw, W2, b2, H, fold, fold + H * 16);
+    GN_LAUNCH_CHECK();
+    return GNNOME_OK;
+}
+#define GN_TRY_RC(call)                     \
+    do {                                    \
+        const int rc__ = (call);            \
+        if (rc__ != GNNOME_OK) return rc__; \
+    } while (0)
+static bool prepared_fold(const GateBfArgs& a) { return a.enc.W23 != nullptr && a.enc.b23 != nullptr && tuning(kTuneForwardEnds) == 0; }
+
 struct EncFoldScratch {
     float* w23 = nullptr;
 };
@@ -854,12 +866,13 @@
     int dev = 0;
     GN_HIP(hipGetDevice(&dev));
     GN_REQUIRE(dev >= 0 && dev < 16, "edge_gate_encode: device index %d", dev);
-    if (!g_enc_fold[dev].w23) GN_HIP(hipMalloc(&g_enc_fold[dev].w23, sizeof(float) * (128 * 16 + 128)));
-    float* w23 = g_enc_fold[dev].w23;
-    hipLaunchKernelGGL(k_fold_encoder, dim3((128 * 17 + 3) / 4), dim3(256), 0, s, a.W3, a.ldw, a.enc.W2, a.enc.b2, 128, w23, w23 + 128 * 16);
-    GN_LAUNCH_CHECK();
-    a.enc.W23 = w23;
-    a.enc.b23 = w23 + 128 * 16;
+    if (!prepared_fold(a)) {
+        if (!g_enc_fold[dev].w23) GN_HIP(hipMalloc(&g_enc_fold[dev].w23, sizeof(float) * (128 * 16 + 128)));
+        float* w23 = g_enc_fold[dev].w23;
+        GN_TRY_RC(launch_fold(a.W3, a.ldw, a.enc.W2, a.enc.b2, 128, w23, s));
+        a.enc.W23 = w23;
+        a.enc.b23 = w23 + 128 * 16;
+    }
     hipLaunchKernelGGL(k_edge_gate_enc16, dim3(persistent_grid()), dim3(640), 0, s, a);
     GN_LAUNCH_CHECK();
     return GNNOME_OK;
@@ -875,12 +888,13 @@
     int dev = 0;
     GN_HIP(hipGetDevice(&dev));
     GN_REQUIRE(dev >= 0 && dev < 16, "edge_gate_encode: device index %d", dev);
-    if (!g_enc_fold256[dev].w23) GN_HIP(hipMalloc(&g_enc_fold256[dev].w23, sizeof(float) * (256 * 16 + 256)));
-    float* w23 = g_enc_fold256[dev].w23;
-    hipLaunchKernelGGL(k_fold_encoder, dim3((256 * 17 + 3) / 4), dim3(256), 0, s, a.W3, a.ldw, a.enc.W2, a.enc.b2, 256, w23, w23 + 256 * 16);
-    GN_LAUNCH_CHECK();
-    a.enc.W23 = w23;
-    a.enc.b23 = w23 + 256 * 16;
+    if (!prepared_fold(a)) {
+        if (!g_enc_fold256[dev].w23) GN_HIP(hipMalloc(&g_enc_fold256[dev].w23, sizeof(float) * (256 * 16 + 256)));
+        float* w23 = g_enc_fold256[dev].w23;
+        GN_TRY_RC(launch_fold(a.W3, a.ldw, a.enc.W2, a.enc.b2, 256, w23, s));
+        a.enc.W23 = w23;
+        a.enc.b23 = w23 + 256 * 16;
+    }
     int g = persistent_grid();
     g -= g % 16;
     return gate_f16_launch(5, a, g < 16 ? 16 : g, s);
@@ -933,6 +947,14 @@
     return mode == 1 ? launch_bf<2, 2, 1, false>(a, s) : launch_bf<2, 2, 2, false>(a, s);
 }
 
+}
+
+extern "C" int gnnome_encoder_fold_f32(const float* W3, int ldw, const float* encW2, const float* encb2, int hidden, float* fold, void* stream) {
+    using namespace gnnome;
+    GN_REQUIRE(hidden == 128 || hidden == 256, "encoder_fold: hidden=%d (the folded layer-0 gates are built at 128 and 256)", hidden);
+    GN_REQUIRE(W3 && encW2 && encb2 && fold && ldw >= hidden, "encoder_fold: bad arguments");
+    GN_REQUIRE((uintptr_t)fold % 16 == 0, "encoder_fold: fold must be 16-byte aligned");
+    return launch_fold(W3, ldw, encW2, encb2, hidden, fold, (hipStream_t)stream);
 }
 
 extern "C" int gnnome_debug_gate_profile(void* counters) {
diff --git a/gnnome_amd/csrc/encode.hip b/gnnome_amd/csrc/encode.hip
--- a/gnnome_amd/csrc/encode.hip
+++ b/gnnome_amd/csrc/encode.hip
@@ -1,4 +1,6 @@
 #include "common.h"
+
+#include <type_traits>
 
 namespace gnnome {
 
@@ -99,13 +101,82 @@
     }
 }
 
+constexpr int kEncRangeThreads = 1024;
+
+template <int H, bool GATHER>
+__global__ __launch_bounds__(kEncRangeThreads) void k_encode_f2m16_range(const float* __restrict__ in, int64_t rows, int64_t per,
+                                                                         const int32_t* __restrict__ gather,
+                                                                         const float* __restrict__ W1, const float* __restrict__ b1,
+                                                                         const float* __restrict__ W2, const float* __restrict__ b2,
+                                                                         float* __restrict__ out) {
+    constexpr int LPR = H / 4, RPB = kEncRangeThreads / LPR, M = 16;
+    const int64_t begin = (int64_t)xcd_remap((int)blockIdx.x, (int)gridDim.x) * per;
+    const int64_t end = begin + per < rows ? begin + per : rows;
+    if (begin >= end) return;
+    const int tid = threadIdx.x, li = tid % LPR, rg = tid / LPR, c = 4 * li;
+    float w1a[M], w1b[M], bb[M];
+#pragma unroll
+    for (int j = 0; j < M; ++j) {
+        w1a[j] = W1[2 * j];
+        w1b[j] = W1[2 * j + 1];
+        bb[j] = b1[j];
+    }
+    f32x4 w2[M];
+#pragma unroll
+    for (int i = 0; i < 4; ++i) {
+#pragma unroll
+        for (int j4 = 0; j4 < M / 4; ++j4) {
+            const f32x4 v = *reinterpret_cast<const f32x4*>(W2 + (c + i) * M + 4 * j4);
+#pragma unroll
+            for (int jj = 0; jj < 4; ++jj) w2[4 * j4 + jj][i] = v[jj];
+        }
+    }
+    const f32x4 bias = *reinterpret_cast<const f32x4*>(b2 + c);
+    using idx_t = typename std::conditional<GATHER, int32_t, int64_t>::type;
+    auto row_in = [&](int64_t r) -> idx_t {
+        const int64_t rr = r < end ? r : end - 1;
+        if constexpr (GATHER) return gather[rr];
+        else return rr;
+    };
+    idx_t nin = row_in(begin + rg);
+    float n0 = in[2 * (int64_t)nin], n1 = in[2 * (int64_t)nin + 1];
+    nin = row_in(begin + rg + RPB);
+    asm volatile("" : "+v"(n0), "+v"(n1), "+v"(nin));
+    for (int64_t r = begin + rg; r < end; r += RPB) {
+        const float x0 = n0, x1 = n1;
+        n0 = in[2 * (int64_t)nin];
+        n1 = in[2 * (int64_t)nin + 1];
+        nin = row_in(r + 2 * RPB);
+        __builtin_amdgcn_sched_barrier(0);
+        f32x4 acc = {0.f, 0.f, 0.f, 0.f};
+#pragma unroll
+        for (int j = 0; j < M; ++j) {
+            const float t = fmaxf(__builtin_fmaf(x1, w1b[j], x0 * w1a[j]) + bb[j], 0.f);
+#pragma unroll
+            for (int i = 0; i < 4; ++i) acc[i] = __builtin_fmaf(t, w2[j][i], acc[i]);
+        }
+        *reinterpret_cast<f32x4*>(out + r * H + c) = acc + bias;
+        __builtin_amdgcn_sched_barrier(0);
+    }
+}
+
 template <int H>
 static int launch_encode(const float* in, int64_t rows, int F, const int32_t* gather, const float* W1, const float* b1,
                          int M, const float* W2, const float* b2, float* out, hipStream_t s) {
     constexpr int RPB = kEncThreads / (H / 4);
     int64_t blocks = (rows + RPB - 1) / RPB;
     if (blocks > kNumCUs * 8) blocks = kNumCUs * 8;
-    if (F == 2 && M == 16 && ((uintptr_t)W2 % 16 == 0)) {
+    if (F == 2 && M == 16 && ((uintptr_t)W2 % 16 == 0) && tuning(kTuneForwardEnds) == 0) {
+        constexpr int64_t RPW = kEncRangeThreads / (H / 4);
+        const int grid = persistent_grid();
+        const int64_t per = ((rows + grid - 1) / grid + RPW - 1) / RPW * RPW;
+        if (gather != nullptr)
+            hipLaunchKernelGGL((k_encode_f2m16_range<H, true>), dim3((unsigned)grid), dim3(kEncRangeThreads), 0, s, in, rows, per, gather, W1, b1,
+                               W2, b2, out);
+        else
+            hipLaunchKernelGGL((k_encode_f2m16_range<H, false>), dim3((unsigned)grid), dim3(kEncRangeThreads), 0, s, in, rows, per, gather, W1, b1,
+                               W2, b2, out);
+    } else if (F == 2 && M == 16 && ((uintptr_t)W2 % 16 == 0)) {
         hipLaunchKernelGGL(k_encode_f2m16<H>, dim3((unsigned)blocks), dim3(kEncThreads), 0, s, in, rows, gather, W1, b1, W2, b2,
                            out);
     } else {
diff --git a/gnnome_amd/csrc/model_forward.cpp b/gnnome_amd/csrc/model_forward.cpp
--- a/gnnome_amd/csrc/model_forward.cpp
+++ b/gnnome_amd/csrc/model_forward.cpp
@@ -72,7 +72,7 @@
 namespace gnnome {
 namespace {
 int forward_on(const gnnome_model_params* m, const gnnome_views* g, const float* x, const float* e_raw, float* logits, float* const h[2], float* P,
-               float* const eb[2], float* PQ, void* stream);
+               float* const eb[2], float* PQ, const float* enc_fold, void* stream);
 }
 }
 
@@ -101,11 +101,16 @@
     char* base = static_cast<char*>(workspace);
     float* h[2] = {reinterpret_cast<float*>(base + ws.h[0]), reinterpret_cast<float*>(base + ws.h[1])};
     float* eb[2] = {reinterpret_cast<float*>(base + ws.e[0]), reinterpret_cast<float*>(base + ws.e[1])};
-    return forward_on(m, g, x, e_raw, logits, h, reinterpret_cast<float*>(base + ws.P), eb, reinterpret_cast<float*>(base + ws.PQ), stream);
+    return forward_on(m, g, x, e_raw, logits, h, reinterpret_cast<float*>(base + ws.P), eb, reinterpret_cast<float*>(base + ws.PQ), nullptr, stream);
 }
 
 extern "C" int gnnome_model_forward_buffers_f32(const gnnome_model_params* m, const gnnome_views* g, const float* x, const float* e_raw, float* logits,
                                                 const gnnome_forward_buffers* b, void* stream) {
+    return gnnome_model_forward_buffers_folded_f32(m, g, x, e_raw, logits, b, nullptr, stream);
+}
+
+extern "C" int gnnome_model_forward_buffers_folded_f32(const gnnome_model_params* m, const gnnome_views* g, const float* x, const float* e_raw,
+                                                       float* logits, const gnnome_forward_buffers* b, const float* enc_fold, void* stream) {
     using namespace gnnome;
     GN_TRY(check_model(m, g));
     GN_REQUIRE(b != nullptr, "model_forward_buffers: null buffer block");
@@ -117,13 +122,13 @@
         GN_REQUIRE((uintptr_t)p % 16 == 0, "model_forward_buffers: buffers must be 16-byte aligned");
     float* h[2] = {b->h[0], b->h[1]};
     float* eb[2] = {b->e[0], m->hidden == 256 ? b->e[1] : b->e[0]};
-    return forward_on(m, g, x, e_raw, logits, h, b->P, eb, b->PQ, stream);
+    return forward_on(m, g, x, e_raw, logits, h, b->P, eb, b->PQ, enc_fold, stream);
 }
 
 namespace gnnome {
 namespace {
 int forward_on(const gnnome_model_params* m, const gnnome_views* g, const float* x, const float* e_raw, float* logits, float* const h[2], float* P,
-               float* const eb[2], float* PQ, void* stream) {
+               float* const eb[2], float* PQ, const float* enc_fold, void* stream) {
     const int64_t N = g->num_nodes, E = g->num_edges;
     const int H = m->hidden, hs = m->score_hidden, L = m->num_layers;
 
@@ -154,8 +159,8 @@
                                             e ? nullptr : m->edge_W2, e ? nullptr : m->edge_b2, stream));
             e = out;
         } else if (e == nullptr) {
-            GN_TRY(gnnome_edge_gate_encode_f32(e_raw, g->srt_eid, m->edge_W1, m->edge_b1, m->edge_W2, m->edge_b2, eb[0], E, H, B1, B2, 5 * H, g->srt_src,
-                                               g->srt_dst, lw.W3, H, lw.scale_e, lw.shift_e, stream));
+            GN_TRY(gnnome_edge_gate_encode_folded_f32(e_raw, g->srt_eid, m->edge_W1, m->edge_b1, m->edge_W2, m->edge_b2, eb[0], E, H, B1, B2, 5 * H,
+                                                      g->srt_src, g->srt_dst, lw.W3, H, lw.scale_e, lw.shift_e, enc_fold, stream));
             e = eb[0];
         } else if (H == 256 && lw.norm_kind == GNNOME_NORM_AFFINE) {
             float* out = e == eb[0] ? eb[1] : eb[0];
diff --git a/gnnome_amd/engine.py b/gnnome_amd/engine.py
--- a/gnnome_amd/engine.py
+++ b/gnnome_amd/engine.py
@@ -7,7 +7,7 @@
 
 
 class LayerWeights:
-    __slots__ = ("Wcat", "bcat", "W3", "b3", "norm", "scale_e", "shift_e", "scale_h", "shift_h", "ref", "gain_e", "planes")
+    __slots__ = ("Wcat", "bcat", "W3", "b3", "norm", "scale_e", "shift_e", "scale_h", "shift_h", "ref", "gain_e", "planes", "enc_fold")
 
 
 REFERENCE_ORDER_GAIN = 16.0
@@ -48,6 +48,10 @@
         self.enc_edge = tuple(dev(t) for t in (model.linear1_edge.weight, model.linear1_edge.bias,
                                                _pad(model.linear2_edge.weight.detach(), H, ne), _pad(model.linear2_edge.bias.detach(), H)))
         self.layers = [prepare_layer(conv, device, arithmetic) for conv in model.gnn.convs]
+        fold = getattr(hip_ops, "encoder_fold", None)
+        if (fold is not None and self.layers and H in hip_ops.ENCODER_FOLD_HIDDEN and not self.layers[0].ref and self.layers[0].norm == NORM_AFFINE
+                and self.layers[0].W3.is_cuda and tuple(self.enc_edge[0].shape) == (16, 2)):
+            self.layers[0].enc_fold = fold(self.layers[0].W3, self.enc_edge[2], self.enc_edge[3])
         self.predictor = prepare_predictor(model.predictor, device)
         weights = [t for lw in self.layers for t in (lw.Wcat, lw.W3)] + [self.predictor["_W1"], self.predictor["W2"]]
         amax = max((float(t.abs().max()) if t.numel() else 0.0) for t in weights) if weights else 0.0
@@ -124,6 +128,7 @@
     b = lambda lin: _pad(lin.bias.detach(), hidden)
     lw.Wcat = dev(torch.cat([W(conv.A_1), W(conv.A_2), W(conv.A_3), W(conv.B_1), W(conv.B_2)], 0))
     lw.W3 = dev(W(conv.B_3))
+    lw.enc_fold = None
     lw.b3 = dev(b(conv.B_3))
     lw.norm, lw.scale_e, lw.shift_e = _norm_affine(conv.bn_e, device)
     kind_h, lw.scale_h, lw.shift_h = _norm_affine(conv.bn_h, device)
@@ -176,7 +181,7 @@
         self.device, self.arithmetic = str(device), getattr(module, "arithmetic", "auto")
         self.slots, self.modules = [], []
         for sub in module.modules():
-            self.modules.append((sub._modules, len(sub._modules)))
+            self.modules.append((sub._modules, tuple(sub._modules.values())))
             for table in (sub._parameters, sub._buffers):
                 for name, t in table.items():
                     if t is not None:
@@ -185,8 +190,8 @@
     def unchanged(self, module, device):
         if str(device) != self.device or getattr(module, "arithmetic", "auto") != self.arithmetic:
             return False
-        for table, count in self.modules:
-            if len(table) != count:
+        for table, children in self.modules:
+            if len(table) != len(children) or any(a is not b for a, b in zip(table.values(), children)):
                 return False
         for table, name, t, version, ptr in self.slots:
             if table.get(name) is not t or t._version != version or t.data_ptr() != ptr:
@@ -244,7 +249,9 @@
     if lw.ref:
         return ops.edge_gate_ref(e, B1, B2, views, lw.W3, lw.b3, lw.scale_e, lw.shift_e, raw_edges=raw_edges)
     if e is None:
-        return ops.edge_gate_encode(raw_edges[0], raw_edges[1], B1, B2, views, lw.W3, lw.scale_e, lw.shift_e)
+        fold = getattr(lw, "enc_fold", None)
+        kw = {} if fold is None else dict(fold=fold)
+        return ops.edge_gate_encode(raw_edges[0], raw_edges[1], B1, B2, views, lw.W3, lw.scale_e, lw.shift_e, **kw)
     return gate_update(ops, lw, views, e, B1, B2, scratch)
 
 
diff --git a/gnnome_amd/ops.py b/gnnome_amd/ops.py
--- a/gnnome_amd/ops.py
+++ b/gnnome_amd/ops.py
@@ -311,6 +311,7 @@
                 setattr(lp, name, _dptr(t))
             lp.Wcat_planes = _dptr(lw.planes)
             lp.norm_kind, lp.reference_order = int(lw.norm), int(bool(lw.ref))
+        self.enc_fold = getattr(prep.layers[0], "enc_fold", None) if n else None
         m = self.params = _lib.ModelParams()
         m.hidden, m.num_layers, m.score_hidden = prep.hidden, n, pw["hs"]
         (W1, b1, W2, b2), (V1, c1, V2, c2) = prep.enc_node, prep.enc_edge
@@ -398,8 +399,8 @@
         bufs = _lib.ForwardBuffers()
         bufs.h[0], bufs.h[1], bufs.P, bufs.PQ = t["h0"].data_ptr(), t["h1"].data_ptr(), t["P"].data_ptr(), t["PQ"].data_ptr()
         bufs.e[0], bufs.e[1] = t["e0"].data_ptr(), (t["e1"].data_ptr() if "e1" in t else None)
-        _lib.check(lib.gnnome_model_forward_buffers_f32(ctypes.byref(m), ctypes.byref(vb), _ptr(x), _ptr(e_raw), _ptr(logits), ctypes.byref(bufs),
-                                                        _stream(dev)), "model_forward_buffers_f32")
+        _lib.check(lib.gnnome_model_forward_buffers_folded_f32(ctypes.byref(m), ctypes.byref(vb), _ptr(x), _ptr(e_raw), _ptr(logits), ctypes.byref(bufs),
+                                                               _ptr(getattr(block, "enc_fold", None)), _stream(dev)), "model_forward_buffers_f32")
 
     with _on(dev):
         run(_placed_buffers(dev, shapes, run))
@@ -502,7 +503,23 @@
             and norm_kind == NORM_AFFINE and e_raw.shape[0] > 0 and B1h.stride(0) % 4 == 0 and B1h.data_ptr() % 16 == 0)
 
 
-def edge_gate_encode(e_raw, enc, B1h, B2h, views, W3, scale, shift):
+ENCODER_FOLD_HIDDEN = (128, 256)
+
+
+def encoder_fold(W3, W2, b2):
+    lib = _lib.load()
+    W3, ldw = _rows(W3, "encoder_fold.W3")
+    H = W3.shape[0]
+    if H not in ENCODER_FOLD_HIDDEN or tuple(W2.shape) != (H, 16) or tuple(b2.shape) != (H,):
+        raise ValueError(f"encoder_fold: W3 [{H}, {H}] with W2 {tuple(W2.shape)}, b2 {tuple(b2.shape)}: hidden in {ENCODER_FOLD_HIDDEN}, hidden_ne = 16")
+    fold = torch.empty(H * 17, dtype=torch.float32, device=W3.device)
+    with _on(W3.device):
+        _lib.check(lib.gnnome_encoder_fold_f32(_ptr(W3), ldw, _ptr(_dense(W2, "encoder_fold.W2")), _ptr(_dense(b2, "encoder_fold.b2")), H, _ptr(fold),
+                                               _stream(W3.device)), "encoder_fold_f32")
+    return fold
+
+
+def edge_gate_encode(e_raw, enc, B1h, B2h, views, W3, scale, shift, fold=None):
     lib = _lib.load()
     e_raw = _dense(e_raw, "edge_gate_encode.e_raw")
     B1h, ldn = _rows(B1h, "edge_gate_encode.B1h")
@@ -512,10 +529,10 @@
     out = torch.empty((E, H), dtype=torch.float32, device=e_raw.device)
     W1, b1, W2, b2 = enc
     with _on(e_raw.device):
-        _lib.check(lib.gnnome_edge_gate_encode_f32(_ptr(e_raw), _ptr(views.srt_eid), _ptr(W1), _ptr(b1), _ptr(W2), _ptr(b2),
-                                                   _ptr(out), E, H, _ptr(B1h), _ptr(B2h), ldn, _ptr(views.srt_src),
-                                                   _ptr(views.srt_dst), _ptr(W3), ldw, _ptr(scale), _ptr(shift),
-                                                   _stream(e_raw.device)), "edge_gate_encode_f32")
+        _lib.check(lib.gnnome_edge_gate_encode_folded_f32(_ptr(e_raw), _ptr(views.srt_eid), _ptr(W1), _ptr(b1), _ptr(W2), _ptr(b2),
+                                                          _ptr(out), E, H, _ptr(B1h), _ptr(B2h), ldn, _ptr(views.srt_src),
+                                                          _ptr(views.srt_dst), _ptr(W3), ldw, _ptr(scale), _ptr(shift), _ptr(fold),
+                                                          _stream(e_raw.device)), "edge_gate_encode_f32")
     return out
 
 
diff --git a/include/gnnome_hip.h b/include/gnnome_hip.h
--- a/include/gnnome_hip.h
+++ b/include/gnnome_hip.h
@@ -56,6 +56,12 @@
                                 const float* B1h, const float* B2h, int ld_node, const int32_t* srt_src,
                                 const int32_t* srt_dst, const float* W3, int ldw, const float* norm_scale,
                                 const float* norm_shift, void* stream);
+int gnnome_encoder_fold_f32(const float* W3, int ldw, const float* encW2, const float* encb2, int hidden, float* fold, void* stream);
+int gnnome_edge_gate_encode_folded_f32(const float* e_raw, const int32_t* srt_eid, const float* encW1, const float* encb1,
+                                       const float* encW2, const float* encb2, float* e_out, int64_t num_edges, int hidden,
+                                       const float* B1h, const float* B2h, int ld_node, const int32_t* srt_src,
+                                       const int32_t* srt_dst, const float* W3, int ldw, const float* norm_scale,
+                                       const float* norm_shift, const float* fold, void* stream);
 
 int gnnome_linear_ref_f32(const float* A, int64_t M, int K, int lda, const float* W, int ldw, const float* bias, int Nout,
                           float* C, int ldc, void* stream);
@@ -233,6 +239,9 @@
 } gnnome_forward_buffers;
 int gnnome_model_forward_buffers_f32(const gnnome_model_params* params_host, const gnnome_views* views_host, const float* x, const float* e_raw,
                                      float* logits, const gnnome_forward_buffers* buffers_host, void* stream);
+int gnnome_model_forward_buffers_folded_f32(const gnnome_model_params* params_host, const gnnome_views* views_host, const float* x,
+                                            const float* e_raw, float* logits, const gnnome_forward_buffers* buffers_host, const float* enc_fold,
+                                            void* stream);
 
 
 int gnnome_edge_gate_raw_f32(const float* e_in, float* x_out, int64_t num_edges, int hidden, const float* B1h,
```

Result: no change. 254.3 million (median of 6 runs) (+0.3%).
